# Amanda-Zheng/MR-GNAS

Hardware: AMD Instinct MI355X
Metric: million edges/sec per supernet fwd+bwd step (FB15k-237, dim=200) (higher is better)
Workload: dtype f32

## Files before the change

include/mrgnas.h:

```cpp
#ifndef MRGNAS_H
#define MRGNAS_H

#include <stdint.h>

#ifdef __cplusplus
extern "C" {
#endif

#define MRG_ABI_VERSION 19

#define MRG_OK            0
#define MRG_E_NULLPTR    -1
#define MRG_E_SHAPE      -2
#define MRG_E_ENUM       -3
#define MRG_E_WORKSPACE  -4

#define MRG_COMPOSE_MULT 0
#define MRG_COMPOSE_SUB  1
#define MRG_COMPOSE_ADD  2
#define MRG_REDUCE_SUM   0
#define MRG_REDUCE_MEAN  1
#define MRG_REDUCE_MAX   2
#define MRG_GCS_SUB      0
#define MRG_GCS_MUL      1
#define MRG_GCS_COPY     2
#define MRG_GCS_NEGS     3
#define MRG_GCS_CCORR    4
#define MRG_GCS_CCONV    5
#define MRG_ACT_NONE     0
#define MRG_ACT_RELU     1
#define MRG_ACT_SIGMOID  2

int mrg_abi_version(void);
const char *mrg_error_string(int code);
const char *mrg_target_arch(void);

int mrg_compose_fwd(int op, const float *s, const float *hr, float *out,
                    int64_t rows, int D, void *stream);
int mrg_compose_bwd(int op, const float *gout, const float *s, const float *hr,
                    float *gs, float *ghr, int64_t rows, int D, void *stream);

int mrg_gather_compose_fwd(int op, const float *ent, const float *rel,
                           const int32_t *ent_idx, const int32_t *rel_idx,
                           float *out, int64_t rows, int D, void *stream);

#define MRG_GATE_LD(D) (2 * (D) + 4)

int mrg_gate_collapse3(const float *const *W_host, const float *const *b_host, const float *const *a_host, float *uvc,
                       int D, int in_dim, int fold, void *stream);
int mrg_gate_param_grad3(const float *const *W_host, const float *const *b_host, const float *const *a_host,
                         const float *d_uvc, float *const *gW_host, float *const *gb_host, float *const *ga_host,
                         int D, int in_dim, int fold, void *stream);
int mrg_fold_halves3(const float *const *W_host, float *Wt, int D, void *stream);
int mrg_unfold_halves3(const float *const *gWt_host, float *const *gW_host, int D, void *stream);

int mrg_gate_fwd(const float *s, const float *s_in, const float *norm, const float *uvc,
                 float *out, int64_t b0, int64_t b1, int64_t M, int D, float scale, void *stream);
int64_t mrg_gate_bwd_workspace_bytes(int64_t M, int D);
int mrg_gate_bwd(const float *gout, const float *s, const float *s_in, const float *norm,
                 const float *uvc, float *gs, float *gs_in, float *d_uvc, void *ws,
                 int64_t b0, int64_t b1, int64_t M, int D, float scale, void *stream);
int mrg_gate_row_fwd(const float *s, const float *s_in, const float *norm, const float *uvc, float *fvec, float *hvec,
                     int64_t b0, int64_t b1, int64_t M, int D, float scale, void *stream);
int mrg_gate_row_bwd(const float *q, const float *hvec, const float *s, const float *s_in, const float *uvc, float *gs_in, float *d_uvc,
                     void *ws, int64_t b0, int64_t b1, int64_t M, int D, void *stream);

int64_t mrg_seg_reduce_workspace_bytes(int64_t n_slots, int D);
int mrg_seg_reduce_fwd(int mode, const float *msg, const float *self_rows,
                       const int32_t *eid,
                       const int32_t *chunk_node, const int32_t *chunk_start, const int32_t *chunk_end,
                       const int32_t *chunk_slot, int64_t n_chunks,
                       const int32_t *hub_node, const int32_t *hub_first, const int32_t *hub_count, int64_t n_hubs,
                       int64_t n_slots, const int32_t *in_degree,
                       float *out, int32_t *arg, void *ws,
                       int64_t N, int D, void *stream);
int mrg_seg_reduce_bwd(int mode, const float *gout, const int32_t *dst, const int32_t *in_degree,
                       const int32_t *arg, float *gmsg, float *gself, const float *relu_src,
                       int64_t E, int64_t N, int D, void *stream);
int mrg_seg_reduce_bwd_ordered(int mode, const float *gout, const int32_t *dst, const int32_t *in_degree, const int32_t *arg,
                               float *gmsg, float *gself, const float *relu_src, const unsigned *relu_bits, const int32_t *order,
                               int64_t E, int64_t N, int D, void *stream);
int mrg_segmax_bwd_input_ok(int D, int Kin);
int mrg_segmax_bwd_input(const float *gout, const float *mx, const int32_t *dst, const int32_t *arg, const float *W, float *gmsg,
                         float *gx, const int32_t *order, int64_t E, int64_t N, int D, int Kin, void *stream);

int64_t mrg_seg_std_workspace_bytes(int64_t n_slots, int D);
int mrg_seg_std_fwd(const float *msg, const int32_t *eid, const int32_t *chunk_node, const int32_t *chunk_start,
                    const int32_t *chunk_end, const int32_t *chunk_slot, int64_t n_chunks, const int32_t *hub_node,
                    const int32_t *hub_first, const int32_t *hub_count, int64_t n_hubs, int64_t n_slots,
                    const int32_t *in_degree, float *out, float *mean, float *coef, void *ws, int64_t N, int D, void *stream);
int mrg_seg_std_bwd(const float *gout, const float *msg, const int32_t *dst, const float *mean, const float *coef,
                    const int32_t *order, float *gmsg, int64_t E, int64_t N, int D, void *stream);

int mrg_fused_gcs(int mode, const float *X, const int32_t *xi, const float *Y, const int32_t *yi,
                  const float *scal, const int32_t *eid,
                  const int32_t *chunk_node, const int32_t *chunk_start, const int32_t *chunk_end,
                  const int32_t *chunk_slot, int64_t n_chunks,
                  const int32_t *hub_node, const int32_t *hub_first, const int32_t *hub_count, int64_t n_hubs,
                  int64_t n_slots, const int32_t *seg_len,
                  float *out, void *ws, int64_t nseg, int D, void *stream);

int mrg_span_gcs(int mode, const float *X, const float *Y, const void *meta, const float *ext_scal, int64_t E, int span,
                 const int32_t *span_slot, const int32_t *span_start, int64_t n_spans,
                 const int32_t *hub_seg, const int32_t *hub_first, const int32_t *hub_count, int64_t n_hubs,
                 int64_t n_slots, const int32_t *seg_len,
                 float *out, void *ws, int64_t nseg, int D, void *stream);

int mrg_sum_buffers(const float *const *xs_host, int K, float *out, int64_t n, int accumulate, void *stream);
int mrg_sum_rows_gather(const float *const *xs_host, int K, const float *gather_edge, const float *gather_self,
                        const int32_t *dst, int64_t E, int64_t rows, int D, float *out, void *stream);

int mrg_distmult_score(const float *ent, const float *rel, const int32_t *s_idx, const int32_t *r_idx,
                       const int32_t *o_idx, float *score, int64_t T, int D, void *stream);

int64_t mrg_mix_workspace_bytes(int K, int D);

int mrg_optim_chunk(void);
int mrg_clip_sgd_step(void *const *params, const void *const *grads, void *const *bufs, const int32_t *chunk_tensor,
                      const int64_t *chunk_off, const int32_t *chunk_len, int64_t n_chunks, double *partial, float *norm_coef,
                      float max_norm, float lr, float momentum, float weight_decay, void *stream);
typedef struct mrg_gated_branch {
  int32_t k;
  const float *s;
  const float *rowscale;
  int32_t row_k;
  const float *row_f;
  const float *row_h;
  const float *row_uvc;
  int32_t row_ld;
  int64_t b0, b1;
  float *row_dq;
  int32_t act;
  const int32_t *valid_rows;
} mrg_gated_branch;
int mrg_mix_colstats(const float *const *y_host, int K, int64_t rows, int D, double *sums, void *ws,
                     const mrg_gated_branch *gated, void *stream);
int mrg_mix_finalize_fwd(const double *sums, const float *const *gamma_host, const float *const *beta_host,
                         float *const *rmean_host, float *const *rvar_host, int K, double total_rows, int D,
                         float eps, float momentum, float *coef, void *stream);
int mrg_mix_stats_coef(const float *const *y, const float *const *gamma, const float *const *beta,
                       float *const *running_mean, float *const *running_var, int K, int64_t rows, double total_rows,
                       int D, float eps, float momentum, float *coef, void *ws, const mrg_gated_branch *gated, void *stream);
int mrg_mix_fwd(const float *const *y_host, int K, const float *coef, const float *w, const float *addend, float *out,
                int64_t rows, int D, const mrg_gated_branch *gated, void *stream);
int mrg_mix_bwd_reduce(const float *g, const float *const *y_host, int K, const float *coef, const float *w,
                       float *red, void *ws, int64_t rows, int D, const mrg_gated_branch *gated, void *stream);
int mrg_mix_finalize_bwd(const float *red, int K, double total_rows, int D, float *coef2,
                         float *const *dgamma_host, float *const *dbeta_host, float *dw, const int32_t *valid_rows, void *stream);
int mrg_mix_bwd_apply(const float *g, const float *const *y_host, float *const *gy_host, int K,
                      const float *coef, const float *coef2, const float *w, const float *const *rs, const float *rs_scale,
                      const float *rs_self, const int64_t *rs_edge_rows, const int *rs_on, const float *const *rs_full,
                      const float *const *fold_s,
                      const float *const *fold_gate, float *const *fold_gs, const int *fold_add_from, int64_t rows, int D,
                      const mrg_gated_branch *gated, void *stream);

int64_t mrg_zero_workspace_bytes(int D);
int mrg_zero_colstats(const float *ent, const float *rel, const int32_t *ent_idx, const int32_t *rel_idx, const int *ops, int K,
                      int64_t rows, int D, double *sums, void *ws, void *stream);
int mrg_zero_stats_coef(const float *ent, const float *rel, const int32_t *ent_idx, const int32_t *rel_idx, const int *ops, int K,
                        const float *const *gamma, const float *const *beta, float *const *running_mean,
                        float *const *running_var, int64_t rows, double total_rows, int D, float eps, float momentum,
                        float *coef, void *ws, const int32_t *valid_rows, void *stream);
int mrg_zero_fwd(const float *ent, const float *rel, const int32_t *ent_idx, const int32_t *rel_idx, const int *ops, int K,
                 const float *coef, const float *w, float *out, int64_t rows, int D, const int32_t *valid_rows, void *stream);
int mrg_zero_bwd_reduce(const float *g, const float *ent, const float *rel, const int32_t *ent_idx, const int32_t *rel_idx,
                        const int *ops, int K, const float *coef, const float *w, float *red, void *ws, int64_t rows, int D,
                        const int32_t *valid_rows, void *stream);
int mrg_zero_bwd_apply(const float *g, const float *ent, const float *rel, const int32_t *ent_idx, const int32_t *rel_idx,
                       const int *ops, int K, const float *coef, const float *coef2, const float *w, float *g_ent_rows,
                       float *g_rel_rows, int64_t rows, int D, const int32_t *valid_rows, void *stream);


int64_t mrg_gemm_workspace_bytes(int K, int Nout);
int mrg_gemm_set_mode(int mode);
int mrg_gemm_set_epilogue(int mode);
int mrg_gemm_set_wide8(int on);
int mrg_gemm_set_q(int on);
int mrg_gemm_set_small(int on);
int mrg_wgrad_set_variant(int variant);
int mrg_linear_fwd(const float *X, const float *W, const float *bias, float *Y, void *ws,
                   int64_t rows, int K, int Nout, int act, void *stream);
int64_t mrg_linear_relu_segmax_workspace_bytes(int64_t N, int K, int Nout);
int mrg_linear_relu_segmax_fwd(const float *X, const float *W, const float *bias, const int32_t *eid, const int32_t *dst,
                               const float *self_rows, float *out, int32_t *arg, float *mx, void *ws,
                               int64_t E, int64_t N, int K, int Nout, void *stream);
int mrg_linear_relu_segsum_fwd(const float *X, const float *W, const float *bias, const int32_t *eid, const int32_t *dst,
                               float *part, unsigned *relu_bits, void *ws, int64_t E, int K, int Nout, void *stream);
int mrg_seg_reduce_heads_fwd(int mode, const float *part, const float *self_rows, const int32_t *rowptr,
                             const int32_t *chunk_node, const int32_t *chunk_start, const int32_t *chunk_end,
                             const int32_t *chunk_slot, int64_t n_chunks, const int32_t *hub_node, const int32_t *hub_first,
                             const int32_t *hub_count, int64_t n_hubs, int64_t n_slots, const int32_t *in_degree, float *out,
                             void *ws, int64_t N, int D, void *stream);
int mrg_seg_reduce_bwd_bits(int mode, const float *gout, const int32_t *dst, const int32_t *in_degree, float *gmsg, float *gself,
                            const unsigned *relu_bits, int64_t E, int64_t N, int D, void *stream);
int64_t mrg_linear_bwd_input_workspace_bytes(int K, int Nout);
int mrg_linear_bwd_input(const float *gY, const float *W, float *gX, void *ws,
                         int64_t rows, int K, int Nout, int ldw, int accumulate, void *stream);
int64_t mrg_linear_bwd_weight_workspace_bytes(int64_t rows, int K, int Nout);
int mrg_linear_bwd_weight(const float *gY, const float *X1, const float *X2, float *gW, float *gbias, void *ws,
                          int64_t rows, int K1, int K2, int Nout, void *stream);
int mrg_linear_bwd_weight_share(const float *gY, const float *X1, const float *X2, float *gW, float *gbias, void *ws,
                                int64_t rows, int K1, int K2, int Nout, int share, void *stream);

int mrg_dense_filter_fwd(int kind, const float *s, const float *s_in, const float *W, const float *bias,
                         const float *rowscale, float scale, float *out, float *gate, void *ws,
                         int64_t rows, int D, void *stream);
int64_t mrg_dense_filter3_workspace_bytes(int D, int K);
int mrg_dense_filter_fwd3(int kind, const float *s, const float *s_in, const float *const *W, const float *const *bias,
                          const float *norm, float scale_edge, float scale_self, float *out, float *gate, void *ws,
                          int64_t b0, int64_t b1, int64_t M, int D, void *stream);
int mrg_dense_filter_dz3(int kind, const float *g, const float *s, const float *gate, const float *norm, float scale_edge,
                         float scale_self, float *dz, float *gs, int64_t b1, int64_t M, int D, void *stream);
int64_t mrg_linear_bwd_input3_workspace_bytes(int K, int Nout);
int mrg_linear_bwd_input3(const float *gY, const float *const *W, float *gX, void *ws, int64_t b0, int64_t b1, int64_t M,
                          int K, int Nout, int ldw, int accumulate, void *stream);
int64_t mrg_linear_bwd_input3_pair_workspace_bytes(int K, int Nout);
int mrg_linear_bwd_input3_pair(const float *gY1, const float *gY2, const float *const *W1, const float *const *W2, float *gX,
                               void *ws, int64_t b0, int64_t b1, int64_t M, int K, int Nout, int ldw, int accumulate,
                               void *stream);
int64_t mrg_linear_bwd_weight3_workspace_bytes(int64_t b0, int64_t b1, int64_t M, int K1, int K2, int Nout);
int mrg_linear_bwd_weight3(const float *gY, const float *X1, const float *X2, float *const *gW, float *const *gbias, void *ws,
                           int64_t b0, int64_t b1, int64_t M, int K1, int K2, int Nout, void *stream);
int mrg_dense_filter_dz(int kind, const float *g, const float *s, const float *gate, const float *rowscale,
                        float scale, float *dz, float *gs, int64_t rows, int D, void *stream);

int64_t mrg_build_graph_workspace_bytes(int64_t T);
int mrg_build_graph(const int64_t *triples, int64_t T, int64_t N, int R, int sorted,
                    const float *deg_norm_table, int64_t table_len,
                    int64_t *src, int64_t *dst, int64_t *etype, float *norm, int32_t *in_degree,
                    int32_t *src32, int32_t *dst32, int32_t *etype32, int32_t *max_degree,
                    void *ws, int64_t ws_bytes, void *stream);

int64_t mrg_plan_workspace_bytes(int64_t E, int64_t nseg, int span);
int mrg_span_plan_build(const int32_t *seg, int64_t E, int64_t nseg, int span, int snap,
                        int32_t *perm, int32_t *seg_sorted, int32_t *seg_len, int32_t *span_slot, int32_t *span_start,
                        int32_t *hub_seg, int32_t *hub_first, int32_t *hub_count, int32_t *counts,
                        void *ws, int64_t ws_bytes, void *stream);
int mrg_span_meta_pack(const int32_t *perm, const int32_t *seg_sorted, const int32_t *xi, const int32_t *yi,
                       const float *scal, int w_is_index, void *meta, int64_t E, void *stream);

int64_t mrg_chunk_plan_workspace_bytes(int64_t E, int64_t N);
int mrg_chunk_plan_build(const int32_t *dst, int64_t E, int64_t N, int chunk,
                         int32_t *eid, int32_t *rowptr, int32_t *in_degree,
                         int32_t *chunk_node, int32_t *chunk_start, int32_t *chunk_end, int32_t *chunk_slot,
                         int32_t *hub_node, int32_t *hub_first, int32_t *hub_count, int32_t *counts,
                         void *ws, int64_t ws_bytes, void *stream);

int mrg_negative_sampling(const int64_t *pos, int64_t B, int rate, const int64_t *values, const double *choices,
                          int64_t *samples, float *labels, void *stream);
int64_t mrg_sample_neighborhood_workspace_bytes(int64_t N, int64_t T);
int mrg_sample_edge_neighborhood(const int32_t *rowptr, const int32_t *adj_edge, const int32_t *adj_other, const int32_t *degrees,
                                 int64_t N, int64_t T, int64_t sample_size, const double *u_vertex, const int64_t *tries,
                                 int64_t n_tries, const double *u_edge, int32_t *edges, int64_t *status, void *ws,
                                 int64_t ws_bytes, void *stream);
int64_t mrg_relabel_workspace_bytes(int64_t num_nodes);
int mrg_relabel_nodes(const int64_t *src, const int64_t *dst, int64_t n, int64_t num_nodes, int64_t *uniq,
                      int64_t *new_src, int64_t *new_dst, int32_t *count, void *ws, int64_t ws_bytes, void *stream);
int mrg_multi_hot_labels(const int64_t *keys, const int32_t *rowptr, const int32_t *objs, const int64_t *query,
                         int64_t B, int64_t U, int64_t num_ent, float v_zero, float v_one, float *out, void *stream);

int mrg_rank_filtered(const float *pred, const float *labels, const int64_t *obj, int64_t B, int64_t N,
                      int64_t *ranks, void *stream);
int mrg_transe_score_fwd(const float *ent, const float *sub, const float *rel, float gamma, float *score,
// ... 44 lines not shown
```

mr-gnas_amd/_lib.py:

```python
import ctypes
import os
import re

import torch

_HERE = os.path.dirname(os.path.abspath(__file__))
LIB_PATH = os.environ.get("MRG_LIB_PATH") or os.path.join(_HERE, "lib", "libmrgnas_hip.so")
HEADER_PATH = os.path.join(os.path.dirname(_HERE), "include", "mrgnas.h")

ABI_VERSION = 19


class MrgnasLibraryError(RuntimeError):
    pass


class MrgnasError(RuntimeError):
    """A C-ABI call returned a non-zero code."""


_P, _I, _L, _F = ctypes.c_void_p, ctypes.c_int, ctypes.c_int64, ctypes.c_float

SIGNATURES = {
    "mrg_abi_version": (_I, []),
    "mrg_error_string": (ctypes.c_char_p, [_I]),
    "mrg_target_arch": (ctypes.c_char_p, []),
    "mrg_compose_fwd": (_I, [_I, _P, _P, _P, _L, _I, _P]),
    "mrg_compose_bwd": (_I, [_I, _P, _P, _P, _P, _P, _L, _I, _P]),
    "mrg_gather_compose_fwd": (_I, [_I, _P, _P, _P, _P, _P, _L, _I, _P]),
    "mrg_gate_collapse3": (_I, [_P, _P, _P, _P, _I, _I, _I, _P]),
    "mrg_gate_param_grad3": (_I, [_P, _P, _P, _P, _P, _P, _P, _I, _I, _I, _P]),
    "mrg_fold_halves3": (_I, [_P, _P, _I, _P]),
    "mrg_unfold_halves3": (_I, [_P, _P, _I, _P]),
    "mrg_gate_fwd": (_I, [_P, _P, _P, _P, _P, _L, _L, _L, _I, _F, _P]),
    "mrg_gate_bwd_workspace_bytes": (_L, [_L, _I]),
    "mrg_gate_bwd": (_I, [_P, _P, _P, _P, _P, _P, _P, _P, _P, _L, _L, _L, _I, _F, _P]),
    "mrg_seg_reduce_workspace_bytes": (_L, [_L, _I]),
    "mrg_seg_reduce_fwd": (_I, [_I, _P, _P, _P, _P, _P, _P, _P, _L, _P, _P, _P, _L, _L, _P, _P, _P, _P, _L, _I, _P]),
    "mrg_seg_reduce_bwd": (_I, [_I, _P, _P, _P, _P, _P, _P, _P, _L, _L, _I, _P]),
    "mrg_fused_gcs": (_I, [_I, _P, _P, _P, _P, _P, _P, _P, _P, _P, _P, _L, _P, _P, _P, _L, _L, _P, _P, _P, _L, _I, _P]),
    "mrg_span_gcs": (_I, [_I, _P, _P, _P, _P, _L, _I, _P, _P, _L, _P, _P, _P, _L, _L, _P, _P, _P, _L, _I, _P]),
    "mrg_sum_buffers": (_I, [_P, _I, _P, _L, _I, _P]),
    "mrg_sum_rows_gather": (_I, [_P, _I, _P, _P, _P, _L, _L, _I, _P, _P]),
    "mrg_distmult_score": (_I, [_P, _P, _P, _P, _P, _P, _L, _I, _P]),
    "mrg_gate_row_fwd": (_I, [_P, _P, _P, _P, _P, _P, _L, _L, _L, _I, _F, _P]),
    "mrg_gate_row_bwd": (_I, [_P, _P, _P, _P, _P, _P, _P, _P, _L, _L, _L, _I, _P]),
    "mrg_mix_workspace_bytes": (_L, [_I, _I]),
    "mrg_mix_colstats": (_I, [_P, _I, _L, _I, _P, _P, _P, _P]),
    "mrg_mix_finalize_fwd": (_I, [_P, _P, _P, _P, _P, _I, ctypes.c_double, _I, _F, _F, _P, _P]),
    "mrg_mix_stats_coef": (_I, [_P, _P, _P, _P, _P, _I, _L, ctypes.c_double, _I, _F, _F, _P, _P, _P, _P]),
    "mrg_zero_workspace_bytes": (_L, [_I]),
    "mrg_zero_colstats": (_I, [_P, _P, _P, _P, _P, _I, _L, _I, _P, _P, _P]),
    "mrg_zero_stats_coef": (_I, [_P, _P, _P, _P, _P, _I, _P, _P, _P, _P, _L, ctypes.c_double, _I, _F, _F, _P, _P, _P, _P]),
    "mrg_zero_fwd": (_I, [_P, _P, _P, _P, _P, _I, _P, _P, _P, _L, _I, _P, _P]),
    "mrg_zero_bwd_reduce": (_I, [_P, _P, _P, _P, _P, _P, _I, _P, _P, _P, _P, _L, _I, _P, _P]),
    "mrg_zero_bwd_apply": (_I, [_P, _P, _P, _P, _P, _P, _I, _P, _P, _P, _P, _P, _L, _I, _P, _P]),
    "mrg_mix_fwd": (_I, [_P, _I, _P, _P, _P, _P, _L, _I, _P, _P]),
    "mrg_mix_bwd_reduce": (_I, [_P, _P, _I, _P, _P, _P, _P, _L, _I, _P, _P]),
    "mrg_mix_finalize_bwd": (_I, [_P, _I, ctypes.c_double, _I, _P, _P, _P, _P, _P, _P]),
    "mrg_mix_bwd_apply": (_I, [_P, _P, _P, _I, _P, _P, _P, _P, _P, _P, _P, _P, _P, _P, _P, _P, _P, _L, _I, _P, _P]),
    "mrg_dense_filter_fwd": (_I, [_I, _P, _P, _P, _P, _P, _F, _P, _P, _P, _L, _I, _P]),
    "mrg_dense_filter_dz": (_I, [_I, _P, _P, _P, _P, _F, _P, _P, _L, _I, _P]),
    "mrg_gemm_workspace_bytes": (_L, [_I, _I]),
    "mrg_gemm_set_mode": (_I, [_I]),
    "mrg_gemm_set_epilogue": (_I, [_I]),
    "mrg_gemm_set_wide8": (_I, [_I]),
    "mrg_gemm_set_q": (_I, [_I]),
    "mrg_gemm_set_small": (_I, [_I]),
    "mrg_segmax_bwd_input_ok": (_I, [_I, _I]),
    "mrg_segmax_bwd_input": (_I, [_P, _P, _P, _P, _P, _P, _P, _P, _L, _L, _I, _I, _P]),
    "mrg_seg_std_workspace_bytes": (_L, [_L, _I]),
    "mrg_seg_std_fwd": (_I, [_P, _P, _P, _P, _P, _P, _L, _P, _P, _P, _L, _L, _P, _P, _P, _P, _P, _L, _I, _P]),
    "mrg_seg_std_bwd": (_I, [_P, _P, _P, _P, _P, _P, _P, _L, _L, _I, _P]),
    "mrg_optim_chunk": (_I, []),
    "mrg_clip_sgd_step": (_I, [_P, _P, _P, _P, _P, _P, _L, _P, _P, _F, _F, _F, _F, _P]),
    "mrg_act_grad_transpose": (_I, [_P, _P, _P, _L, _L, _I, _P]),
    "mrg_wgrad_set_variant": (_I, [_I]),
    "mrg_linear_fwd": (_I, [_P, _P, _P, _P, _P, _L, _I, _I, _I, _P]),
    "mrg_dense_filter3_workspace_bytes": (_L, [_I, _I]),
    "mrg_dense_filter_fwd3": (_I, [_I, _P, _P, _P, _P, _P, _F, _F, _P, _P, _P, _L, _L, _L, _I, _P]),
    "mrg_dense_filter_dz3": (_I, [_I, _P, _P, _P, _P, _F, _F, _P, _P, _L, _L, _I, _P]),
    "mrg_linear_bwd_input3_workspace_bytes": (_L, [_I, _I]),
    "mrg_linear_bwd_input3": (_I, [_P, _P, _P, _P, _L, _L, _L, _I, _I, _I, _I, _P]),
    "mrg_linear_bwd_input3_pair_workspace_bytes": (_L, [_I, _I]),
    "mrg_linear_bwd_input3_pair": (_I, [_P, _P, _P, _P, _P, _P, _L, _L, _L, _I, _I, _I, _I, _P]),
    "mrg_linear_bwd_weight3_workspace_bytes": (_L, [_L, _L, _L, _I, _I, _I]),
    "mrg_linear_bwd_weight3": (_I, [_P, _P, _P, _P, _P, _P, _L, _L, _L, _I, _I, _I, _P]),
    "mrg_linear_relu_segsum_fwd": (_I, [_P, _P, _P, _P, _P, _P, _P, _P, _L, _I, _I, _P]),
    "mrg_seg_reduce_heads_fwd": (_I, [_I, _P, _P, _P, _P, _P, _P, _P, _L, _P, _P, _P, _L, _L, _P, _P, _P, _L, _I, _P]),
    "mrg_seg_reduce_bwd_bits": (_I, [_I, _P, _P, _P, _P, _P, _P, _L, _L, _I, _P]),
    "mrg_seg_reduce_bwd_ordered": (_I, [_I, _P, _P, _P, _P, _P, _P, _P, _P, _P, _L, _L, _I, _P]),
    "mrg_linear_relu_segmax_workspace_bytes": (_L, [_L, _I, _I]),
    "mrg_linear_relu_segmax_fwd": (_I, [_P, _P, _P, _P, _P, _P, _P, _P, _P, _P, _L, _L, _I, _I, _P]),
    "mrg_linear_bwd_input_workspace_bytes": (_L, [_I, _I]),
    "mrg_linear_bwd_input": (_I, [_P, _P, _P, _P, _L, _I, _I, _I, _I, _P]),
    "mrg_linear_bwd_weight_workspace_bytes": (_L, [_L, _I, _I]),
    "mrg_linear_bwd_weight": (_I, [_P, _P, _P, _P, _P, _P, _L, _I, _I, _I, _P]),
    "mrg_linear_bwd_weight_share": (_I, [_P, _P, _P, _P, _P, _P, _L, _I, _I, _I, _I, _P]),
    "mrg_build_graph_workspace_bytes": (_L, [_L]),
    "mrg_build_graph": (_I, [_P, _L, _L, _I, _I, _P, _L, _P, _P, _P, _P, _P, _P, _P, _P, _P, _P, _L, _P]),
    "mrg_plan_workspace_bytes": (_L, [_L, _L, _I]),
    "mrg_span_plan_build": (_I, [_P, _L, _L, _I, _I, _P, _P, _P, _P, _P, _P, _P, _P, _P, _P, _L, _P]),
    "mrg_span_meta_pack": (_I, [_P, _P, _P, _P, _P, _I, _P, _L, _P]),
    "mrg_chunk_plan_workspace_bytes": (_L, [_L, _L]),
    "mrg_chunk_plan_build": (_I, [_P, _L, _L, _I, _P, _P, _P, _P, _P, _P, _P, _P, _P, _P, _P, _P, _L, _P]),
    "mrg_negative_sampling": (_I, [_P, _L, _I, _P, _P, _P, _P, _P]),
    "mrg_sample_neighborhood_workspace_bytes": (_L, [_L, _L]),
    "mrg_sample_edge_neighborhood": (_I, [_P, _P, _P, _P, _L, _L, _L, _P, _P, _L, _P, _P, _P, _P, _L, _P]),
    "mrg_relabel_workspace_bytes": (_L, [_L]),
    "mrg_relabel_nodes": (_I, [_P, _P, _L, _L, _P, _P, _P, _P, _P, _L, _P]),
    "mrg_multi_hot_labels": (_I, [_P, _P, _P, _P, _L, _L, _L, _F, _F, _P, _P]),
    "mrg_rank_filtered": (_I, [_P, _P, _P, _L, _L, _P, _P]),
    "mrg_transe_score_fwd": (_I, [_P, _P, _P, _F, _P, _L, _L, _I, _P]),
    "mrg_transe_score_bwd": (_I, [_P, _P, _P, _P, _P, _P, _P, _L, _L, _I, _P]),
    "mrg_ccorr_rows": (_I, [_I, _P, _P, _P, _L, _I, _P]),
    "mrg_ccorr_matrix": (_I, [_I, _P, _P, _I, _P]),
    "mrg_ccorr_matrix_grad": (_I, [_I, _P, _P, _I, _P]),
    "mrg_conve_fc_workspace_bytes": (_L, [_L, _L, _I]),
    "mrg_conve_bwd_workspace_bytes": (_L, [_L, _I, _I, _I]),
    "mrg_conve_bn0_fwd": (_I, [_P, _P, _L, _I, _P, _P, _I, _F, _F, _P, _P]),
    "mrg_conve_conv_fwd": (_I, [_I, _P, _P, _L, _I, _I, _I, _P, _P, _P, _P, _P, _I, _I, _P, _P]),
    "mrg_conve_bn1_fwd": (_I, [_P, _L, _I, _I, _P, _P, _P, _P, _P, _I, _F, _F, _P, _P, _P]),
    "mrg_conve_fc_fwd": (_I, [_P, _P, _P, _P, _P, _P, _L, _L, _I, _P]),
    "mrg_conve_fc_bwd": (_I, [_P, _P, _P, _P, _P, _P, _P, _P, _L, _L, _I, _P]),
    "mrg_conve_bn1_bwd": (_I, [_P, _P, _P, _P, _P, _P, _I, _L, _I, _I, _P, _P, _P]),
    "mrg_conve_conv_bwd": (_I, [_I, _P, _P, _L, _I, _I, _I, _P, _P, _P, _P, _I, _I, _P, _P, _P]),
    "mrg_conve_finish_bwd": (_I, [_I, _P, _P, _L, _I, _I, _I, _P, _P, _I, _P, _P, _P, _P, _P, _P, _P, _P]),
}

_lib = None


def declared_symbols():
# ... 7 lines not shown
    if _lib is not None:
        return _lib
    if not os.path.exists(LIB_PATH):
        raise MrgnasLibraryError(
            f"{LIB_PATH} not found: build it with `python -c 'import __graft_entry__ as g; g.build()'` "
            "(or `make -C mr-gnas_amd/csrc`). mr_gnas_amd has no CPU fallback.")
    lib = ctypes.CDLL(LIB_PATH)
    for name, (res, args) in SIGNATURES.items():
        fn = getattr(lib, name)
        fn.restype, fn.argtypes = res, args
    if lib.mrg_abi_version() != ABI_VERSION:
        raise MrgnasLibraryError(f"ABI version {lib.mrg_abi_version()} != expected {ABI_VERSION}; rebuild the library")
    _lib = lib
    return lib


class KernelMeter:

    def __init__(self):
        self.names = None
        self.records = {}

    def start(self, names=None):
        self.names = set(names) if names is not None else True
        self.records = {}

    def active(self, name):
        return self.names is not None and (self.names is True or name in self.names)

    def stop(self):
        torch.cuda.synchronize()
        out = {}
        for name, recs in self.records.items():
            ms = sum(a.elapsed_time(b) for a, b, _, _ in recs)
            out[name] = {"launches": len(recs), "ms": ms, "bytes": sum(r[2] for r in recs), "flops": sum(r[3] for r in recs)}
        self.names, self.records = None, {}
        return out


meter = KernelMeter()


_FN = {}
TRACE = os.environ.get("MRG_TRACE") == "1"


def _trace(name, args):
    import sys
    shown = [hex(a.value) if isinstance(a, ctypes.c_void_p) and a.value else ("NULL" if isinstance(a, ctypes.c_void_p) or a is None else a)
             for a in args]
    print(f"[mrg] {name} {shown}", file=sys.stderr, flush=True)


def call(name, args, nbytes=0, flops=0):
    fn = _FN.get(name)
    if fn is None:
        fn = _FN[name] = getattr(load(), name)
    if TRACE:
        _trace(name, args)
        code = fn(*args)
        torch.cuda.synchronize()
        if code != 0:
            check(code, name)
        return
    if meter.names is not None and meter.active(name):
        a, b = torch.cuda.Event(enable_timing=True), torch.cuda.Event(enable_timing=True)
        a.record()
        code = fn(*args)
        b.record()
        meter.records.setdefault(name, []).append((a, b, nbytes, flops))
    else:
        code = fn(*args)
    if code != 0:
        check(code, name)


def check(code, what=""):
    if code != 0:
        msg = load().mrg_error_string(code).decode()
        raise MrgnasError(f"{what}: {msg} (code {code})")


def ptr(t):
    return None if t is None else ctypes.c_void_p(t.data_ptr())


def ptr_array(tensors):
    arr = (ctypes.c_void_p * len(tensors))()
    for i, t in enumerate(tensors):
        arr[i] = None if t is None else t.data_ptr()
    return arr


class GatedBranch(ctypes.Structure):
    _fields_ = [("k", ctypes.c_int32), ("s", ctypes.c_void_p), ("rowscale", ctypes.c_void_p),
                ("row_k", ctypes.c_int32), ("row_f", ctypes.c_void_p), ("row_h", ctypes.c_void_p), ("row_uvc", ctypes.c_void_p),
                ("row_ld", ctypes.c_int32), ("b0", ctypes.c_int64), ("b1", ctypes.c_int64), ("row_dq", ctypes.c_void_p),
                ("act", ctypes.c_int32), ("valid_rows", ctypes.c_void_p)]


ACTS = {"relu": 0, "tanh": 1}


def gated_branch(spec, row_dq=None, act=0, valid_rows=None):
    dp = lambda t: None if t is None else t.data_ptr()
    if spec is None:
        if not act and valid_rows is None:
            return None
        return ctypes.byref(GatedBranch(-1, None, None, -1, None, None, None, 0, 0, 0, None, int(act), dp(valid_rows)))
    g = GatedBranch(int(spec.get("k", -1)), dp(spec["s"]), dp(spec.get("c")), int(spec.get("row_k", -1)), dp(spec.get("row_f")),
                    dp(spec.get("row_h")), dp(spec.get("row_uvc")), int(spec.get("row_ld", 0)), int(spec.get("b0", 0)), int(spec.get("b1", 0)),
                    dp(row_dq), int(act), dp(valid_rows))
    return ctypes.byref(g)


_RAW_STREAM = getattr(torch._C, "_cuda_getCurrentRawStream", None) if os.environ.get("MRG_RAW_STREAM", "1") == "1" else None


def stream_of(t):
    if _RAW_STREAM is not None:
        return ctypes.c_void_p(_RAW_STREAM(t.device.index if t.device.index is not None else torch.cuda.current_device()))
    return ctypes.c_void_p(torch.cuda.current_stream(t.device).cuda_stream)


def require_hip(*tensors):
    for t in tensors:
        if t is None:
            continue
        if not t.is_cuda:
            raise MrgnasError("mr_gnas_amd operators need tensors on a HIP device (no CPU fallback); got " + str(t.device))
        if not t.is_contiguous():
            raise MrgnasError("mr_gnas_amd operators need contiguous tensors")
    load()


def f32c(t):
    if t is None:
        return None
    if t.dtype != torch.float32:
        t = t.float()
    return t if t.is_contiguous() else t.contiguous()
```

mr-gnas_amd/cell_lp.py:

```python
import os

import torch
import torch.nn as nn

from . import functional as K
from . import lazy as LZ
from . import operations_lp as OPS
from .operations_lp import PRE_OPS, FIRST_OPS, MIDDLE_OPS, LAST_OPS, MIXED_OPS, MIXED_OPS_sf, SF_OPS

CALLER = os.environ.get("MRG_CALLER", "fused")

MIXED_STREAMS = int(os.environ.get("MRG_MIXED_STREAMS", "1"))


def _literal(h):
    x = h.x if isinstance(h, K.Fan) else h
    return CALLER == "reference" or not (x.table if isinstance(x, K.LazyRows) else x).is_cuda


def _tensor(y):
    return y.y if isinstance(y, K.Candidate) else y


def _plain(h):
    if isinstance(h, K.Fan):
        h = h.take()
    return h.materialize() if isinstance(h, K.LazyRows) else h


def _valid_rows(g, ys):
    counts = getattr(g, "valid_rows", None)
    y = next((y for y in ys if y is not None), None)
    return counts.get(int(_tensor(y).shape[0])) if counts and y is not None else None


def _identity_index(ops):
    ids = [k for k, op in enumerate(ops) if type(op) is OPS.f_identity_op]
    return ids[0] if len(ids) == 1 else None


def _dense_pair(ops, x):
    if not x.is_cuda:
        return None
    d = [k for k, op in enumerate(ops) if type(op) is OPS.f_dense_op_comp]
    c = [k for k, op in enumerate(ops) if type(op) is OPS.f_comp_op]
    if len(d) != 1 or len(c) != 1:
        return None
    return (d[0], c[0])


def _run(op, g, a, b, for_epilogue=False):
    if op._forward_hooks or op._forward_pre_hooks or not hasattr(op, "run"):
        return LZ.real(op(g, a, b, for_epilogue=True) if for_epilogue else op(g, a, b))
    return op.run(g, a, b, for_epilogue=for_epilogue)


def fused_candidates(ops, bns, weights, g, h, h_in, addend=None, group=None, total_rows=None, prepare_only=False):
    if isinstance(h, K.LazyRows):
        if (K.switches.CELL_ZERO_FUSED and isinstance(h_in, K.LazyRows) and addend is None and len(ops) <= 3
                and all(isinstance(op, OPS._PreOp) for op in ops)):
            return K.cell_zero_mixed([op.kind for op in ops], h, h_in, bns, weights, group, total_rows, _valid_rows(g, [h]))
        ys = [_run(op, g, h, h_in) for op in ops]
        return K.mixed_epilogue(ys, bns, weights, group, total_rows, addend, fold_row_scales=True, valid_rows=_valid_rows(g, ys))
    n = len(ops)
    fh = h if isinstance(h, K.Fan) else K.Fan(h, n)
    fi = h_in if isinstance(h_in, K.Fan) else K.Fan(h_in, n)
    pair = _dense_pair(ops, fh.x)
    paired = {}
    row_ok = pair is not None and K.switches.GATED_RECOMPUTE and K.switches.FOLD_ROW_SCALE
    dev = fh.x.device
    nstreams = min(MIXED_STREAMS, n) if fh.x.shape[0] >= K.switches.FORK_MIN_ROWS else 1
    if nstreams <= 1:
        ys = []
        for k, op in enumerate(ops):
            if isinstance(op, OPS.f_zero_op):
                ys.append(None)
            elif pair is not None and k in pair:
                if not paired:
                    paired[pair[0]], paired[pair[1]] = OPS.dense_pair_forward(ops[pair[0]], ops[pair[1]], g, fh.take(), fi.take(), for_epilogue=True)
                ys.append(paired[k])
            elif (row_ok and type(op) is OPS.f_sparse_op_comp) or type(op) in (OPS.f_dense_op_comp, OPS.f_comp_op):
                ys.append(_run(op, g, fh.take(), fi.take(), for_epilogue=True))
            else:
                ys.append(_run(op, g, fh.take(), fi.take()))
        prep = K.mixed_epilogue_prepare(ys, bns, group, total_rows, True, _identity_index(ops), valid_rows=_valid_rows(g, ys))
        return prep if prepare_only else prep(weights, addend)
    fork = K.Fork(dev, nstreams, tag="candidates")
    ys = []
    for k, op in enumerate(ops):
        if isinstance(op, OPS.f_zero_op):
            ys.append(None)
            continue
        if pair is not None and k in pair and paired:
            ys.append(paired[k])
            continue
        side = fork.stream(k)
        a, b = fh.take(), fi.take()
        if side is not fork.main:
            a.record_stream(side)
            b.record_stream(side)
        with torch.cuda.stream(side):
            if pair is not None and k in pair:
                paired[pair[0]], paired[pair[1]] = OPS.dense_pair_forward(ops[pair[0]], ops[pair[1]], g, a, b, for_epilogue=True)
                y = paired[k]
                _tensor(paired[pair[0] + pair[1] - k]).record_stream(fork.main)
            elif (row_ok and type(op) is OPS.f_sparse_op_comp) or type(op) in (OPS.f_dense_op_comp, OPS.f_comp_op):
                y = _run(op, g, a, b, for_epilogue=True)
            else:
                y = _run(op, g, a, b)
        _tensor(y).record_stream(fork.main)
        ys.append(y)
    fork.join()
    prep = K.mixed_epilogue_prepare(ys, bns, group, total_rows, True, _identity_index(ops), valid_rows=_valid_rows(g, ys))
    return prep if prepare_only else prep(weights, addend)


class MixedOp(nn.Module):

    def __init__(self, feature_dim, drop_aggr, operations, registry=None):
        super().__init__()
        registry = MIXED_OPS if registry is None else registry
        self._feature_dim, self._operations, self._drop_aggr = feature_dim, operations, drop_aggr
        self._args = {'feature_dim': feature_dim, 'drop_aggr': drop_aggr}
        self._ops = nn.ModuleList(nn.ModuleList([registry[name](self._args), nn.BatchNorm1d(feature_dim), nn.ReLU()])
                                  for name in operations)

    def op_forward(self, op, g, h, h_in):
        nh = op[0](g, h, h_in)
        for i in range(1, len(op)):
            nh = op[i](nh.float())
        return nh

    def forward(self, weights, g, h, h_in, group=None, total_rows=None, addend=None, prepare_only=False):
        if _literal(h):
            h, h_in = _plain(h), _plain(h_in)
            total = sum(w * self.op_forward(op, g, h, h_in) for w, op in zip(weights, self._ops))
            return total if addend is None else addend + total
        return fused_candidates([op for op, _, _ in self._ops], [bn for _, bn, _ in self._ops], weights, g, h, h_in, addend, group,
                                total_rows, prepare_only)

    def _identity_index(self):
        return _identity_index([op for op, _, _ in self._ops])

    def _dense_pair(self, x):
        return _dense_pair([op for op, _, _ in self._ops], x)


class MixedOp_SF(nn.Module):

    def __init__(self, gamma, operations, registry=None):
        super().__init__()
        registry = MIXED_OPS_sf if registry is None else registry
        self._operations, self.gamma = operations, gamma
        self._args = {'gamma': gamma}
        self._ops = nn.ModuleList(nn.ModuleList([registry[name](self._args)]) for name in operations)

    def op_forward(self, op, g, h, h_in):
        return op[0](g, h, h_in)

    def forward(self, weights, g, h, h_in):
        return sum(w * self.op_forward(op, g, h, h_in) for w, op in zip(weights, self._ops))


# ... 102 lines not shown
```

mr-gnas_amd/csrc/dense.hip:

```cpp
#include "gemm_dispatch.hpp"

namespace mrg {

template <int VEC, int LPR, int KMAX, int KIND>
__global__ __launch_bounds__(MRG_BLOCK) void dense_dz_k(const float* __restrict__ g, const float* __restrict__ s,
                                                        const float* __restrict__ gate, const float* __restrict__ rowscale,
                                                        float scale, float* __restrict__ dz, float* __restrict__ gs,
                                                        int64_t rows, int D, int64_t edge_rows, float scale_self) {
  constexpr int RPB = MRG_BLOCK / LPR;
  const int sl = threadIdx.x % LPR, rw = row_group_of_thread<LPR>();
  const int dv = D / VEC;
  for (int64_t r = (int64_t)blockIdx.x * RPB + rw; r < rows; r += (int64_t)gridDim.x * RPB) {
    const float c = r < edge_rows ? scale * (rowscale ? rowscale[r] : 1.0f) : scale_self;
#pragma unroll
    for (int k = 0; k < KMAX; ++k) {
      int col = sl + k * LPR;
      if (col < dv) {
        Vec<VEC> gv = Vec<VEC>::load(g + r * D + col * VEC), o;
        if (KIND == 0) {
          Vec<VEC> sv = Vec<VEC>::load(s + r * D + col * VEC), ga = Vec<VEC>::load(gate + r * D + col * VEC), o2;
#pragma unroll
          for (int j = 0; j < VEC; ++j) {
            float gc = gv[j] * c;
            o2[j] = gc * ga[j];
            o[j] = gc * sv[j] * ga[j] * (1.0f - ga[j]);
          }
          o2.store(gs + r * D + col * VEC);
        } else {
#pragma unroll
          for (int j = 0; j < VEC; ++j) o[j] = gv[j] * c;
        }
        o.store(dz + r * D + col * VEC);
      }
    }
  }
}

}

using namespace mrg;

extern "C" int mrg_dense_filter_fwd(int kind, const float* s, const float* s_in, const float* W, const float* bias,
                                    const float* rowscale, float scale, float* out, float* gate, void* ws, int64_t rows, int D,
                                    void* stream) {
  if (kind != 0 && kind != 1) return MRG_E_ENUM;
  if (rows < 0 || D <= 0) return MRG_E_SHAPE;
  if (rows == 0) return MRG_OK;
  if (!s || !W || !out) return MRG_E_NULLPTR;
  GemmArgs a{};
  a.A1 = s; a.K1 = D;
  a.A2 = s_in; a.K2 = s_in ? D : 0;
  a.B = W;
  a.bias = bias; a.C = out; a.ldc = D; a.N = D; a.rows = rows;
  a.rowscale = rowscale; a.scale = scale;
  if (kind == 0) {
    a.S = s; a.ld_s = D; a.aux = gate;
    return launch_gemm<EPI_GATE>(a, a.K1 + a.K2, 1, ws, (hipStream_t)stream);
  }
  return launch_gemm<EPI_SCALE>(a, a.K1 + a.K2, 1, ws, (hipStream_t)stream);
}

static bool dense3_shape_ok(int D, int K) { return D > 0 && (K == D || K == 2 * D) && K > 48 && D % 4 == 0; }

extern "C" int64_t mrg_dense_filter3_workspace_bytes(int D, int K) {
  if (!dense3_shape_ok(D, K) || gemm_mode() == 1) return 0;
  return 3 * (int64_t)(((int64_t)bsplit_bytes_any(D, K) + 255) / 256 * 256);
}

extern "C" int mrg_dense_filter_fwd3(int kind, const float* s, const float* s_in, const float* const* W_host, const float* const* bias_host,
                                     const float* norm, float scale_edge, float scale_self, float* out, float* gate, void* ws,
                                     int64_t b0, int64_t b1, int64_t M, int D, void* stream) {
  if (kind != 0 && kind != 1) return MRG_E_ENUM;
  if (D <= 0 || M < 0 || b0 < 0 || b1 < b0 || M < b1) return MRG_E_SHAPE;
  const int K = s_in ? 2 * D : D;
  if (!dense3_shape_ok(D, K)) return MRG_E_SHAPE;
  if (M == 0) return MRG_OK;
  if (!s || !W_host) return MRG_E_NULLPTR;
  if (kind == 0 && !gate) return MRG_E_NULLPTR;
  if (!out && kind != 0) return MRG_E_NULLPTR;
  if (!ws) return MRG_E_WORKSPACE;
  hipStream_t st = (hipStream_t)stream;
  const int64_t lo[3] = {0, b0, b1}, hi[3] = {b0, b1, M};
  const size_t each = (size_t)(((int64_t)bsplit_bytes_any(D, K) + 255) / 256 * 256);
  GemmArgs a{};
  a.A1 = s; a.K1 = D; a.A2 = s_in; a.K2 = s_in ? D : 0;
  a.C = out; a.ldc = D; a.N = D; a.rows = M; a.rowscale = norm;
  if (kind == 0) { a.S = s; a.ld_s = D; a.aux = gate; }
  if (!x3_eligible(a)) return MRG_E_SHAPE;
  const float* Bs[3]; void* outs[3];
  a.grp.n = 3;
  a.grp.bp_stride = (int64_t)each;
  for (int i = 0; i < 3; ++i) {
    const bool live = hi[i] > lo[i];
    if (live && !W_host[i]) return MRG_E_NULLPTR;
    Bs[i] = live ? W_host[i] : nullptr;
    outs[i] = (char*)ws + i * each;
    a.grp.lo[i] = lo[i]; a.grp.hi[i] = live ? hi[i] : lo[i];
    a.grp.bias[i] = bias_host ? bias_host[i] : nullptr;
    a.grp.scale[i] = i < 2 ? scale_edge : scale_self;
    a.grp.use_rowscale[i] = (i < 2 && norm) ? 1 : 0;
  }
  launch_bsplit3_any(kind == 0 ? EPI_GATE : EPI_SCALE, M, Bs, K, 1, D, K, outs, st);
  MRG_LAUNCH_CHECK();
  if (kind == 0) return launch_rowgemm_x3_mode<EPI_GATE>(a, outs[0], st);
  return launch_rowgemm_x3_mode<EPI_SCALE>(a, outs[0], st);
}

static int dense_dz_launch(int kind, const float* g, const float* s, const float* gate, const float* rowscale, float scale, float* dz,
                           float* gs, int64_t rows, int D, int64_t edge_rows, float scale_self, void* stream);

extern "C" int mrg_dense_filter_dz(int kind, const float* g, const float* s, const float* gate, const float* rowscale,
                                   float scale, float* dz, float* gs, int64_t rows, int D, void* stream) {
  return dense_dz_launch(kind, g, s, gate, rowscale, scale, dz, gs, rows, D, rows, scale, stream);
}

extern "C" int mrg_dense_filter_dz3(int kind, const float* g, const float* s, const float* gate, const float* norm, float scale_edge,
                                    float scale_self, float* dz, float* gs, int64_t b1, int64_t M, int D, void* stream) {
  if (b1 < 0 || M < b1) return MRG_E_SHAPE;
  return dense_dz_launch(kind, g, s, gate, norm, scale_edge, dz, gs, M, D, b1, scale_self, stream);
}

static int dense_dz_launch(int kind, const float* g, const float* s, const float* gate, const float* rowscale, float scale, float* dz,
                           float* gs, int64_t rows, int D, int64_t edge_rows, float scale_self, void* stream) {
  if (kind != 0 && kind != 1) return MRG_E_ENUM;
  if (rows < 0 || D <= 0) return MRG_E_SHAPE;
  if (rows == 0) return MRG_OK;
  if (!g || !dz) return MRG_E_NULLPTR;
  if (kind == 0 && (!s || !gate || !gs)) return MRG_E_NULLPTR;
  hipStream_t st = (hipStream_t)stream;
  RowGeom gm = row_geom(D, aligned16(g) && aligned16(s) && aligned16(gate) && aligned16(gs) && aligned16(dz));
  if (!gm.ok) return MRG_E_SHAPE;
#define CALL(V, L, KM)                                                                                                \
  do {                                                                                                                \
    int grid = grid_for(rows, (MRG_BLOCK / L) * 4);                                                                         \
    if (kind == 0) hipLaunchKernelGGL((dense_dz_k<V, L, KM, 0>), dim3(grid), dim3(MRG_BLOCK), 0, st, g, s, gate, rowscale, scale, dz, gs, rows, D, edge_rows, scale_self); \
    else hipLaunchKernelGGL((dense_dz_k<V, L, KM, 1>), dim3(grid), dim3(MRG_BLOCK), 0, st, g, s, gate, rowscale, scale, dz, gs, rows, D, edge_rows, scale_self); \
  } while (0)
  MRG_DISPATCH_GEOM(gm, CALL);
#undef CALL
  MRG_LAUNCH_CHECK();
  return MRG_OK;
}
```

mr-gnas_amd/csrc/gate.hip:

```cpp
#include "common.hpp"

namespace mrg {

struct SegPlan {
  int64_t lo[3], hi[3];
  int blk[4];
};

static SegPlan make_plan(int64_t b0, int64_t b1, int64_t M, int grid) {
  SegPlan p;
  p.lo[0] = 0;  p.hi[0] = b0;
  p.lo[1] = b0; p.hi[1] = b1;
  p.lo[2] = b1; p.hi[2] = M;
  int nseg = 0;
  for (int s = 0; s < 3; ++s) nseg += (p.hi[s] > p.lo[s]);
  int spare = grid - nseg;
  p.blk[0] = 0;
  for (int s = 0; s < 3; ++s) {
    int64_t rows = p.hi[s] - p.lo[s];
    int nb = rows > 0 ? 1 + (int)((double)spare * (double)rows / (double)M) : 0;
    p.blk[s + 1] = p.blk[s] + nb;
  }
  return p;
}
// ... 180 lines not shown
    if (srcidx >= 0) {
#pragma unroll
      for (int q = 0; q < RPB; ++q) acc += (double)red[q * (2 * WIDTH + 1) + srcidx];
    }
    dst[t] = (float)acc;
  }
}

template <int VEC, int LPR, int KMAX, bool HAS_IN>
__global__ __launch_bounds__(MRG_BLOCK) void gate_row_fwd_k(const float* __restrict__ s, const float* __restrict__ sin_,
                                                            const float* __restrict__ norm, const float* __restrict__ uvc,
                                                            float* __restrict__ fvec, float* __restrict__ hvec, SegPlan p, int D, float scale) {
  constexpr int RPB = MRG_BLOCK / LPR;
  const int b = blockIdx.x;
  if (b >= p.blk[3]) return;
  const int seg = (b >= p.blk[1]) + (b >= p.blk[2]);
  const int jb = b - p.blk[seg], nb = p.blk[seg + 1] - p.blk[seg];
  const int sl = threadIdx.x % LPR, rw = row_group_of_thread<LPR>();
  const int dv = D / VEC;
  const float* u = uvc + (int64_t)seg * MRG_GATE_LD(D);
  const float cc = u[HAS_IN ? 2 * D : D];
  Vec<VEC> uk[KMAX], vk[KMAX];
#pragma unroll
  for (int k = 0; k < KMAX; ++k) {
    int c = sl + k * LPR;
    uk[k] = c < dv ? Vec<VEC>::load(u + c * VEC) : Vec<VEC>::fill(0.f);
    vk[k] = (HAS_IN && c < dv) ? Vec<VEC>::load(u + D + c * VEC) : Vec<VEC>::fill(0.f);
  }
  const bool use_norm = norm != nullptr && seg < 2;
  for (int64_t r = p.lo[seg] + (int64_t)jb * RPB + rw; r < p.hi[seg]; r += (int64_t)nb * RPB) {
    float dot = 0.f;
#pragma unroll
    for (int k = 0; k < KMAX; ++k) {
      int c = sl + k * LPR;
      if (c < dv) {
        const Vec<VEC> sk = Vec<VEC>::load(s + r * D + c * VEC);
#pragma unroll
        for (int j = 0; j < VEC; ++j) dot += sk[j] * uk[k][j];
        if (HAS_IN) {
          Vec<VEC> x = Vec<VEC>::load(sin_ + r * D + c * VEC);
#pragma unroll
          for (int j = 0; j < VEC; ++j) dot += x[j] * vk[k][j];
        }
      }
    }
    const float z = group_sum<LPR>(dot) + cc;
    const float gt = sigmoidf_fast(z);
    const float nv = use_norm ? norm[r] : 1.0f;
    if (sl == 0) {
      fvec[r] = gt * scale * nv;
      const float t = scale * nv;
      hvec[r] = t * gt * (1.0f - gt);
    }
  }
}

template <int VEC, int LPR, int KMAX, bool HAS_IN>
__global__ __launch_bounds__(MRG_BLOCK) void gate_row_bwd_k(const float* __restrict__ qv, const float* __restrict__ hv, const float* __restrict__ s,
                                                            const float* __restrict__ sin_, const float* __restrict__ uvc,
                                                            float* __restrict__ gsin, float* __restrict__ ws, SegPlan p, int D) {
  constexpr int RPB = MRG_BLOCK / LPR;
  constexpr int WIDTH = LPR * KMAX * VEC;
  __shared__ float red[RPB * (2 * WIDTH + 1)];
  const int b = blockIdx.x;
  if (b >= p.blk[3]) return;
  const int seg = (b >= p.blk[1]) + (b >= p.blk[2]);
  const int jb = b - p.blk[seg], nb = p.blk[seg + 1] - p.blk[seg];
  const int sl = threadIdx.x % LPR, rw = row_group_of_thread<LPR>();
  const int dv = D / VEC;
  const int ld = MRG_GATE_LD(D);
  const int cidx = HAS_IN ? 2 * D : D;
  const float* u = uvc + (int64_t)seg * ld;
  Vec<VEC> vk[KMAX], du[KMAX], dvv[KMAX];
  double dc = 0.0;
#pragma unroll
  for (int k = 0; k < KMAX; ++k) {
    int c = sl + k * LPR;
    vk[k] = (HAS_IN && c < dv) ? Vec<VEC>::load(u + D + c * VEC) : Vec<VEC>::fill(0.f);
    du[k] = Vec<VEC>::fill(0.f);
    dvv[k] = Vec<VEC>::fill(0.f);
  }
  for (int64_t r = p.lo[seg] + (int64_t)jb * RPB + rw; r < p.hi[seg]; r += (int64_t)nb * RPB) {
    const float dz = qv[r] * hv[r];
    dc += (double)dz;
#pragma unroll
    for (int k = 0; k < KMAX; ++k) {
      int c = sl + k * LPR;
      if (c < dv) {
        const Vec<VEC> sk = Vec<VEC>::load(s + r * D + c * VEC);
#pragma unroll
        for (int j = 0; j < VEC; ++j) du[k][j] += dz * sk[j];
        if (HAS_IN) {
          const Vec<VEC> xk = Vec<VEC>::load(sin_ + r * D + c * VEC);
          Vec<VEC> o2;
#pragma unroll
          for (int j = 0; j < VEC; ++j) {
            o2[j] = dz * vk[k][j];
            dvv[k][j] += dz * xk[j];
          }
          o2.store(gsin + r * D + c * VEC);
        }
      }
    }
  }
  float* mine = red + rw * (2 * WIDTH + 1);
#pragma unroll
// ... 167 lines not shown
  if (!g.ok) return MRG_E_SHAPE;
  hipStream_t st = (hipStream_t)stream;
  int grid = 1;
#define CALL(V, L, K)                                                                                                   \
  do {                                                                                                                  \
    grid = grid_for(M, (MRG_BLOCK / L) * 4);                                                                                   \
    if (grid < 3) grid = 3;                                                                                             \
    SegPlan p = make_plan(b0, b1, M, grid);                                                                             \
    if (s_in) hipLaunchKernelGGL((gate_fwd_k<V, L, K, true, gate_rpt(L)>), dim3(p.blk[3]), dim3(MRG_BLOCK), 0, st, s, s_in, norm, uvc, out, p, D, scale); \
    else hipLaunchKernelGGL((gate_fwd_k<V, L, K, false, gate_rpt(L)>), dim3(p.blk[3]), dim3(MRG_BLOCK), 0, st, s, s_in, norm, uvc, out, p, D, scale); \
  } while (0)
  MRG_DISPATCH_GEOM(g, CALL);
#undef CALL
  MRG_LAUNCH_CHECK();
  return MRG_OK;
}

extern "C" int64_t mrg_gate_bwd_workspace_bytes(int64_t M, int D) {
  (void)M;
  return (int64_t)(MRG_MAX_GRID + 3) * MRG_GATE_LD((int64_t)D) * sizeof(float);
}

extern "C" int mrg_gate_bwd(const float* gout, const float* s, const float* s_in, const float* norm, const float* uvc,
                            float* gs, float* gs_in, float* d_uvc, void* ws, int64_t b0, int64_t b1, int64_t M, int D,
                            float scale, void* stream) {
  if (D <= 0 || M < 0 || b0 < 0 || b1 < b0 || M < b1) return MRG_E_SHAPE;
  if (!uvc || !d_uvc) return MRG_E_NULLPTR;
  if (M > 0 && (!gout || !s || !gs)) return MRG_E_NULLPTR;
  if (s_in && !gs_in) return MRG_E_NULLPTR;
  if (!ws) return MRG_E_WORKSPACE;
  hipStream_t st = (hipStream_t)stream;
  const int ld = MRG_GATE_LD(D);
  RowGeom g = row_geom(D, aligned16(gout) && aligned16(s) && aligned16(s_in) && aligned16(gs) && aligned16(gs_in) && aligned16(uvc));
  if (!g.ok) return MRG_E_SHAPE;
  SegPlan p{};
#define CALL(V, L, K)                                                                                                   \
  do {                                                                                                                  \
    int grid = grid_for(M, (MRG_BLOCK / L) * 4);                                                                               \
    if (grid < 3) grid = 3;                                                                                             \
    p = make_plan(b0, b1, M, grid);                                                                                     \
    if (M > 0) {                                                                                                        \
      if (s_in) hipLaunchKernelGGL((gate_bwd_k<V, L, K, true, gate_rpt(L)>), dim3(p.blk[3]), dim3(MRG_BLOCK), 0, st, gout, s, s_in, norm, uvc, gs, gs_in, (float*)ws, p, D, scale); \
      else hipLaunchKernelGGL((gate_bwd_k<V, L, K, false, gate_rpt(L)>), dim3(p.blk[3]), dim3(MRG_BLOCK), 0, st, gout, s, s_in, norm, uvc, gs, gs_in, (float*)ws, p, D, scale); \
    }                                                                                                                   \
  } while (0)
  MRG_DISPATCH_GEOM(g, CALL);
#undef CALL
  MRG_LAUNCH_CHECK();
  launch_ordered_reduce_ranges<float>((const float*)ws, d_uvc, p.blk, 3, ld, ld, ld, st);
  MRG_LAUNCH_CHECK();
  return MRG_OK;
}

extern "C" int mrg_gate_row_fwd(const float* s, const float* s_in, const float* norm, const float* uvc, float* fvec, float* hvec,
                                int64_t b0, int64_t b1, int64_t M, int D, float scale, void* stream) {
  if (D <= 0 || M < 0 || b0 < 0 || b1 < b0 || M < b1) return MRG_E_SHAPE;
  if (M == 0) return MRG_OK;
  if (!s || !uvc || !fvec || !hvec) return MRG_E_NULLPTR;
  RowGeom g = row_geom(D, aligned16(s) && aligned16(s_in) && aligned16(uvc));
  if (!g.ok) return MRG_E_SHAPE;
  hipStream_t st = (hipStream_t)stream;
#define CALL(V, L, K)                                                                                                   \
  do {                                                                                                                  \
    int grid = grid_for(M, (MRG_BLOCK / L) * 4);                                                                        \
    if (grid < 3) grid = 3;                                                                                             \
    SegPlan p = make_plan(b0, b1, M, grid);                                                                             \
    if (s_in) hipLaunchKernelGGL((gate_row_fwd_k<V, L, K, true>), dim3(p.blk[3]), dim3(MRG_BLOCK), 0, st, s, s_in, norm, uvc, fvec, hvec, p, D, scale); \
    else hipLaunchKernelGGL((gate_row_fwd_k<V, L, K, false>), dim3(p.blk[3]), dim3(MRG_BLOCK), 0, st, s, s_in, norm, uvc, fvec, hvec, p, D, scale); \
  } while (0)
  MRG_DISPATCH_GEOM(g, CALL);
#undef CALL
  MRG_LAUNCH_CHECK();
  return MRG_OK;
}

extern "C" int mrg_gate_row_bwd(const float* q, const float* hvec, const float* s, const float* s_in, const float* uvc, float* gs_in, float* d_uvc,
                                void* ws, int64_t b0, int64_t b1, int64_t M, int D, void* stream) {
  if (D <= 0 || M < 0 || b0 < 0 || b1 < b0 || M < b1) return MRG_E_SHAPE;
  if (!uvc || !d_uvc) return MRG_E_NULLPTR;
  if (M > 0 && (!q || !hvec || !s)) return MRG_E_NULLPTR;
  if (s_in && !gs_in) return MRG_E_NULLPTR;
  if (!ws) return MRG_E_WORKSPACE;
  hipStream_t st = (hipStream_t)stream;
  const int ld = MRG_GATE_LD(D);
  RowGeom g = row_geom(D, aligned16(s) && aligned16(s_in) && aligned16(gs_in) && aligned16(uvc));
  if (!g.ok) return MRG_E_SHAPE;
  SegPlan p{};
#define CALL(V, L, K)                                                                                                   \
  do {                                                                                                                  \
    int grid = grid_for(M, (MRG_BLOCK / L) * 4);                                                                        \
    if (grid < 3) grid = 3;                                                                                             \
    p = make_plan(b0, b1, M, grid);                                                                                     \
    if (M > 0) {                                                                                                        \
      if (s_in) hipLaunchKernelGGL((gate_row_bwd_k<V, L, K, true>), dim3(p.blk[3]), dim3(MRG_BLOCK), 0, st, q, hvec, s, s_in, uvc, gs_in, (float*)ws, p, D); \
      else hipLaunchKernelGGL((gate_row_bwd_k<V, L, K, false>), dim3(p.blk[3]), dim3(MRG_BLOCK), 0, st, q, hvec, s, s_in, uvc, gs_in, (float*)ws, p, D); \
    }                                                                                                                   \
  } while (0)
  MRG_DISPATCH_GEOM(g, CALL);
#undef CALL
  MRG_LAUNCH_CHECK();
  launch_ordered_reduce_ranges<float>((const float*)ws, d_uvc, p.blk, 3, ld, ld, ld, st);
  MRG_LAUNCH_CHECK();
  return MRG_OK;
}
```

mr-gnas_amd/csrc/gemm.hpp:

```cpp
#pragma once
#include "common.hpp"

namespace mrg {

typedef float f32x16 __attribute__((ext_vector_type(16)));
typedef float v4f __attribute__((ext_vector_type(4)));
typedef __attribute__((address_space(3))) void* lds_ptr_t;
typedef const __attribute__((address_space(1))) void* gbl_ptr_t;

constexpr int GBM_MAX = 256;

enum { EPI_BIAS_ACT = 0, EPI_GATE = 1, EPI_SCALE = 2, EPI_ACCUM = 3, EPI_SEGMAX = 4, EPI_SEGSUM = 5 };

struct GemmGroups {
  int n;
  int tile0[4];
  int64_t lo[3], hi[3];
  int64_t bp_stride;
  const float* bias[3];
  float scale[3];
  int use_rowscale[3];
};
inline int gemm_group_tiles(GemmGroups& g, int gbm) {
  g.tile0[0] = 0;
  for (int i = 0; i < 3; ++i) {
    const int64_t r = i < g.n && g.hi[i] > g.lo[i] ? g.hi[i] - g.lo[i] : 0;
    g.tile0[i + 1] = g.tile0[i] + (int)((r + gbm - 1) / gbm);
  }
  return g.tile0[3];
}

struct GemmArgs {
  const float* A1; const float* A2;
  int K1, K2;
  const float* B; int ldb;
  const float* bias;
  float* C; int ldc; int N;
  int64_t rows;
  int act;
  const float* S; int ld_s;
  const float* rowscale; float scale;
  float* aux;
  const float* Cin; int ld_cin;
  const int32_t* row_index;
  const int32_t* row_seg;
  unsigned long long* seg_out;
  float* seg_part;
  unsigned* relu_bits; int bits_ld;
  int epi_lds; int wave_lds_floats;
  GemmGroups grp;
};

template <bool DUAL>
__device__ __forceinline__ const float* gemm_a_ptr(const float* r1, const float* r2, int K1, int K2, int K, int k) {
  if (DUAL) {
    const bool first = k < K1;
    const int kk = first ? k : k - K1, ld = first ? K1 : K2;
    return (first ? r1 : r2) + (kk + 4 <= ld ? kk : ld - 4);
  }
  return r1 + (k + 4 <= K ? k : K - 4);
}

template <int NT>
__device__ __forceinline__ void gemm_epilogue_segsum(const GemmArgs& a, f32x16 (&acc)[NT], int64_t rowbase, int col0, int li, int lh) {
  if (rowbase >= a.rows) return;
  int seg[16], eidv[16];
#pragma unroll
  for (int r = 0; r < 16; ++r) {
    const int64_t row = rowbase + (r & 3) + 8 * (r >> 2) + 4 * lh;
    const bool ok = row < a.rows;
    const int64_t rc = ok ? row : a.rows - 1;
    const int e = a.row_index ? a.row_index[rc] : (int)rc;
    eidv[r] = ok ? e : -1;
    seg[r] = ok ? a.row_seg[e] : -1;
  }
#pragma unroll
  for (int n = 0; n < NT; ++n) {
    const int col = col0 + n * 32 + li;
    const bool cok = col < a.N;
    const float bv = (a.bias && cok) ? a.bias[col] : 0.f;
    int cur = -1;
    int64_t head = 0;
    float sum = 0.f;
#pragma unroll
    for (int r = 0; r < 16; ++r) {
      const float x = acc[n][r] + bv;
      const bool pos = x > 0.f;
      const unsigned long long ball = __ballot(pos);
      if (li == 0 && eidv[r] >= 0 && a.relu_bits && (col0 >> 5) + n < a.bits_ld)
        a.relu_bits[(int64_t)eidv[r] * a.bits_ld + (col0 >> 5) + n] = lh ? (unsigned)(ball >> 32) : (unsigned)ball;
      if (seg[r] != cur) {
        if (cur >= 0 && cok) a.seg_part[head * a.N + col] = sum;
        cur = seg[r];
        head = rowbase + (r & 3) + 8 * (r >> 2) + 4 * lh;
        sum = 0.f;
      }
      sum += pos ? x : 0.f;
    }
    if (cur >= 0 && cok) a.seg_part[head * a.N + col] = sum;
  }
}

template <int NT>
__device__ __forceinline__ void gemm_epilogue_segmax(const GemmArgs& a, f32x16 (&acc)[NT], int64_t rowbase, int col0, int li, int lh) {
  if (rowbase >= a.rows) return;
// ... 47 lines not shown
template <bool VEC4>
__device__ __forceinline__ float4 gemm_mask4(float4 v, int64_t row, int64_t nrows, int k, int K) {
  const bool rv = row < nrows;
  if (VEC4) {
    const bool ok = rv && k + 4 <= K;
    v.x = ok ? v.x : 0.f; v.y = ok ? v.y : 0.f; v.z = ok ? v.z : 0.f; v.w = ok ? v.w : 0.f;
  } else {
    v.x = (rv && k < K) ? v.x : 0.f; v.y = (rv && k + 1 < K) ? v.y : 0.f;
    v.z = (rv && k + 2 < K) ? v.z : 0.f; v.w = (rv && k + 3 < K) ? v.w : 0.f;
  }
  return v;
}

struct ASel { const float* base; int ld, kk; };
__device__ __forceinline__ ASel gemm_sel_a(const GemmArgs& a, int k) {
  const bool first = k < a.K1 || a.K2 == 0;
  ASel s;
  s.base = first ? a.A1 : a.A2;
  s.ld = first ? a.K1 : a.K2;
  s.kk = first ? k : k - a.K1;
  return s;
}

template <bool VEC4>
__device__ __forceinline__ float4 gemm_raw_a(const GemmArgs& a, int64_t row, int k) {
  if (VEC4) {
    const ASel sa = gemm_sel_a(a, k);
    return gemm_raw4<true>(sa.base, row, a.rows, sa.kk, sa.ld, sa.ld);
  }
  const int64_t rc = row < a.rows ? row : a.rows - 1;
  float v[4];
#pragma unroll
  for (int j = 0; j < 4; ++j) {
    const ASel sa = gemm_sel_a(a, k + j);
    const int kc = sa.kk < sa.ld ? sa.kk : sa.ld - 1;
    v[j] = sa.base[rc * sa.ld + kc];
  }
  return make_float4(v[0], v[1], v[2], v[3]);
}

template <bool VEC4>
__device__ __forceinline__ float4 gemm_mask_a(float4 v, const GemmArgs& a, int64_t row, int k) {
  if (VEC4) {
    const ASel sa = gemm_sel_a(a, k);
    return gemm_mask4<true>(v, row, a.rows, sa.kk, sa.ld);
  }
  const int K = a.K1 + a.K2;
  const bool rv = row < a.rows;
  v.x = (rv && k < K) ? v.x : 0.f; v.y = (rv && k + 1 < K) ? v.y : 0.f;
  v.z = (rv && k + 2 < K) ? v.z : 0.f; v.w = (rv && k + 3 < K) ? v.w : 0.f;
  return v;
}

template <int NT, int EPI>
__device__ __forceinline__ void gemm_epilogue(const GemmArgs& a, f32x16 (&acc)[NT], int64_t rowbase, int col0, int li, int lh,
                                              bool full) {
  if (rowbase >= a.rows) return;
  const int last = (int)((a.rows - 1 - rowbase) < 31 ? (a.rows - 1 - rowbase) : 31);
  const int colw = col0 + li < a.N ? col0 + li : a.N - 1;
  float* crow[16];
  const float* srow[16];
  float* xrow[16];
  float cs[16];
  bool rok[16];
  const bool cstore = EPI != EPI_GATE || a.C != nullptr;
#pragma unroll
  for (int r = 0; r < 16; ++r) {
    const int row = (r & 3) + 8 * (r >> 2) + 4 * lh;
    const int rc = row < last ? row : last;
    rok[r] = row <= last;
    crow[r] = a.C + (rowbase + rc) * a.ldc + colw;
    if (EPI == EPI_GATE) srow[r] = a.S + (rowbase + rc) * a.ld_s + colw;
    if (EPI == EPI_ACCUM) srow[r] = a.Cin + (rowbase + rc) * a.ld_cin + colw;
    if (EPI == EPI_GATE) xrow[r] = a.aux ? a.aux + (rowbase + rc) * a.N + colw : nullptr;
    cs[r] = 1.0f;
    if (EPI == EPI_GATE || EPI == EPI_SCALE) cs[r] = a.scale * (a.rowscale ? a.rowscale[rowbase + rc] : 1.0f);
  }
#pragma unroll
  for (int n = 0; n < NT; ++n) {
    const int col = col0 + n * 32 + li;
    const bool cok = col < a.N;
    const int off = cok ? n * 32 : 0;
    const float bv = a.bias ? a.bias[cok ? col : colw] : 0.f;
    float in[16], v[16], g[16];
#pragma unroll
    for (int r = 0; r < 16; ++r) in[r] = 0.f;
    if ((EPI == EPI_GATE && cstore) || EPI == EPI_ACCUM) {
#pragma unroll
      for (int r = 0; r < 16; ++r) in[r] = srow[r][off];
    }
#pragma unroll
    for (int r = 0; r < 16; ++r) {
      float x = acc[n][r] + bv;
      if (EPI == EPI_BIAS_ACT) {
        v[r] = (a.act == MRG_ACT_RELU) ? (x > 0.f ? x : 0.f) : (a.act == MRG_ACT_SIGMOID ? sigmoidf_fast(x) : x);
      } else if (EPI == EPI_GATE) {
        g[r] = sigmoidf_fast(x);
        v[r] = g[r] * in[r] * cs[r];
      } else if (EPI == EPI_SCALE) {
        v[r] = x * cs[r];
      } else {
        v[r] = x + in[r];
      }
    }
    if (full) {
      if (cok) {
        if (cstore) {
#pragma unroll
          for (int r = 0; r < 16; ++r) crow[r][n * 32] = v[r];
        }
        if (EPI == EPI_GATE && a.aux) {
#pragma unroll
          for (int r = 0; r < 16; ++r) xrow[r][n * 32] = g[r];
        }
      }
    } else {
#pragma unroll
      for (int r = 0; r < 16; ++r) {
        if (cok && rok[r]) {
          if (cstore) crow[r][n * 32] = v[r];
          if (EPI == EPI_GATE && a.aux) xrow[r][n * 32] = g[r];
        }
      }
    }
  }
}

template <int NT, int EPI>
__device__ __forceinline__ void gemm_epilogue_tr(const GemmArgs& a, f32x16 (&acc)[NT], int64_t rowbase, int col0, int li, int lh) {
  if (rowbase >= a.rows) return;
  const int64_t row = rowbase + li;
  const bool rok = row < a.rows;
  const int64_t rc = rok ? row : a.rows - 1;
  const int cb = col0 + 4 * lh;
  const bool cstore = EPI != EPI_GATE || a.C != nullptr;
  float* crow = cstore ? a.C + rc * a.ldc + cb : nullptr;
  const float* srow = nullptr;
  if (EPI == EPI_GATE && cstore) srow = a.S + rc * a.ld_s + cb;
  if (EPI == EPI_ACCUM) srow = a.Cin + rc * a.ld_cin + cb;
  float* xrow = (EPI == EPI_GATE && a.aux) ? a.aux + rc * a.N + cb : nullptr;
  float cs = 1.0f;
  if (EPI == EPI_GATE || EPI == EPI_SCALE) cs = a.scale * (a.rowscale ? a.rowscale[rc] : 1.0f);
  const float* brow = a.bias ? a.bias + cb : nullptr;
#pragma unroll
  for (int n = 0; n < NT; ++n) {
#pragma unroll
    for (int g = 0; g < 4; ++g) {
      const int off = n * 32 + g * 8;
      if (cb + off >= a.N) continue;
      float4 bv = make_float4(0.f, 0.f, 0.f, 0.f), in = make_float4(0.f, 0.f, 0.f, 0.f);
      if (brow) bv = *reinterpret_cast<const float4*>(brow + off);
      if (srow) in = *reinterpret_cast<const float4*>(srow + off);
      const float bb[4] = {bv.x, bv.y, bv.z, bv.w}, ii[4] = {in.x, in.y, in.z, in.w};
      float v[4], gt[4];
#pragma unroll
      for (int j = 0; j < 4; ++j) {
        const float x = acc[n][4 * g + j] + bb[j];
        if (EPI == EPI_BIAS_ACT) {
          v[j] = (a.act == MRG_ACT_RELU) ? (x > 0.f ? x : 0.f) : (a.act == MRG_ACT_SIGMOID ? sigmoidf_fast(x) : x);
        } else if (EPI == EPI_GATE) {
          gt[j] = sigmoidf_fast(x);
          v[j] = gt[j] * ii[j] * cs;
        } else if (EPI == EPI_SCALE) {
          v[j] = x * cs;
        } else {
          v[j] = x + ii[j];
        }
      }
      if (rok) {
        if (cstore) *reinterpret_cast<float4*>(crow + off) = make_float4(v[0], v[1], v[2], v[3]);
        if (EPI == EPI_GATE && xrow) *reinterpret_cast<float4*>(xrow + off) = make_float4(gt[0], gt[1], gt[2], gt[3]);
      }
    }
  }
}

template <int EPI>
// ... 395 lines not shown
```

mr-gnas_amd/csrc/gemm_dispatch.hpp:

```cpp
#pragma once
#include "gemm_x3.hpp"
#include "gemm_x3s.hpp"
#include "gemm_x3s8.hpp"
#include "gemm_x3q.hpp"

namespace mrg {

inline int gemm_mode() { return gemm_switches().mode; }

constexpr int X3Q_MIN_K = 224;
inline bool x3q_shape(int epi, int N, int K) {
  const int q = gemm_switches().q;
  return gemm_mode() == 0 && q != 0 && epi != EPI_SEGMAX && epi != EPI_SEGSUM && N > 128 && N <= X3Q_NT * 16 && K > (q == 2 ? 48 : X3Q_MIN_K);
}

constexpr int X3N_NT = 2;
inline bool x3n_shape(int epi, int64_t rows, int N, int K) {
  return gemm_mode() == 0 && rows > 0 && rows <= gemm_switches().small_rows && gemm_pick_nt(N) > X3N_NT && N <= 224 && !x3q_shape(epi, N, K);
}

inline size_t bsplit_bytes_any(int N, int K) {
  const size_t a = x3_bsplit_bytes(N, K, gemm_pick_nt(N));
  const size_t q = (N > 128 && N <= X3Q_NT * 16) ? x3q_bsplit_bytes(K) : 0;
  const size_t n = (gemm_pick_nt(N) > X3N_NT && N <= 224) ? x3_bsplit_bytes(N, K, X3N_NT) : 0;
  const size_t m = a > q ? a : q;
  return m > n ? m : n;
}

inline void launch_bsplit_any(int epi, int64_t rows, const float* B, int64_t sn, int64_t sk, int N, int K, void* Bp, hipStream_t st) {
  if (x3q_shape(epi, N, K)) {
    const float* Bs[1] = {B};
    void* outs[1] = {Bp};
    launch_bsplitq3(Bs, sn, sk, N, K, outs, 1, st);
  } else {
    launch_bsplit(B, sn, sk, N, K, x3n_shape(epi, rows, N, K) ? X3N_NT : gemm_pick_nt(N), Bp, st);
  }
}
inline void launch_bsplit3_any(int epi, int64_t rows, const float* const* B, int64_t sn, int64_t sk, int N, int K, void* const* out, hipStream_t st,
                               const float* const* B2 = nullptr, int ksplit = 0) {
  if (x3q_shape(epi, N, K)) launch_bsplitq3(B, sn, sk, N, K, out, 3, st, B2, ksplit);
  else launch_bsplit3(B, sn, sk, N, K, x3n_shape(epi, rows, N, K) ? X3N_NT : gemm_pick_nt(N), out, st, B2, ksplit);
}

template <int EPI>
inline int launch_rowgemm_x3_mode(GemmArgs a, const void* Bp, hipStream_t st) {
  if (x3q_shape(EPI, a.N, a.K1 + a.K2)) {
    if (!x3q_eligible(a)) return MRG_E_SHAPE;
    return launch_rowgemm_x3q<EPI>(a, Bp, st);
  }
  if (x3n_shape(EPI, a.rows, a.N, a.K1 + a.K2)) {
    if (!x3_eligible(a)) return MRG_E_SHAPE;
    return launch_rowgemm_x3<EPI>(a, Bp, st, X3N_NT);
  }
  if (gemm_mode() != 2 && x3s_eligible(a)) {
    if constexpr (EPI != EPI_GATE) {
      if (x3s8_eligible<EPI>(a)) return launch_rowgemm_x3s8<EPI>(a, Bp, st);
    }
    return launch_rowgemm_x3s<EPI>(a, Bp, st);
  }
  return launch_rowgemm_x3<EPI>(a, Bp, st);
}

inline size_t gemm_workspace_bytes(int K, int N) {
  const size_t split = bsplit_bytes_any(N, K);
  const size_t transp = (size_t)K * N * sizeof(float);
  return split > transp ? split : transp;
}

template <int EPI>
inline int launch_gemm(GemmArgs a, int64_t b_sn, int64_t b_sk, void* ws, hipStream_t st) {
  if (a.rows <= 0) return MRG_OK;
  if (!a.A2 || a.K2 == 0) { a.A2 = a.A1; a.K2 = 0; }
  const int K = a.K1 + a.K2;
  if (ws && gemm_mode() != 1 && x3_eligible(a)) {
    launch_bsplit_any(EPI, a.rows, a.B, b_sn, b_sk, a.N, K, ws, st);
    return launch_rowgemm_x3_mode<EPI>(a, ws, st);
  }
  if (b_sk != 1) {
    if (!ws) return MRG_E_WORKSPACE;
    launch_transpose(a.B, (float*)ws, (int)(K), a.N, (int)b_sk, st);
    a.B = (const float*)ws;
    a.ldb = K;
  } else {
    a.ldb = (int)b_sn;
  }
  return launch_rowgemm<EPI>(a, st);
}

}
```

mr-gnas_amd/csrc/gemm_x3q.hpp:

```cpp
#pragma once
#include "gemm_x3.hpp"

namespace mrg {

constexpr int X3Q_CHUNK = X3Q_HT * 3 * 1024;
constexpr int X3Q_ROWS = 64;

inline size_t x3q_bsplit_bytes(int K) { return (size_t)x3q_slabs(K) * 2 * X3Q_CHUNK; }

template <int EPI>
__device__ __forceinline__ void gemm_epilogue_q(const GemmArgs& a, f32x4v (&acc)[X3Q_NT], int64_t rowbase, int li, int lh, bool full) {
  if (rowbase >= a.rows) return;
  const int last = (int)((a.rows - 1 - rowbase) < 15 ? (a.rows - 1 - rowbase) : 15);
  const int colw = li < a.N ? li : a.N - 1;
  float* crow[8];
  const float* srow[8];
  float* xrow[8];
  float cs[8];
  bool rok[8];
  const bool cstore = EPI != EPI_GATE || a.C != nullptr;
#pragma unroll
  for (int i = 0; i < 8; ++i) {
    const int row = i + 8 * lh;
    const int rc = row < last ? row : last;
    rok[i] = row <= last;
    crow[i] = a.C + (rowbase + rc) * a.ldc + colw;
    if (EPI == EPI_GATE) srow[i] = a.S + (rowbase + rc) * a.ld_s + colw;
    if (EPI == EPI_ACCUM) srow[i] = a.Cin + (rowbase + rc) * a.ld_cin + colw;
    if (EPI == EPI_GATE) xrow[i] = a.aux ? a.aux + (rowbase + rc) * a.N + colw : nullptr;
    cs[i] = 1.0f;
    if (EPI == EPI_GATE || EPI == EPI_SCALE) cs[i] = a.scale * (a.rowscale ? a.rowscale[rowbase + rc] : 1.0f);
  }
  const int lc = li & 15;
#pragma unroll
  for (int j = 0; j < X3Q_HT; ++j) {
    const int ca = (2 * j) * 16 + lc, cb = (2 * j + 1) * 16 + lc;
    const float bva = a.bias ? a.bias[ca < a.N ? ca : a.N - 1] : 0.f;
    const float bvb = a.bias ? a.bias[cb < a.N ? cb : a.N - 1] : 0.f;
    float acc8[8];
#pragma unroll
    for (int r = 0; r < 4; ++r) {
      float xa = acc[2 * j][r] + bva, xb = acc[2 * j + 1][r] + bvb;
      asm volatile("s_nop 1\n\tv_permlane16_swap_b32 %0, %1" : "+v"(xa), "+v"(xb));
      acc8[r] = xa;
      acc8[4 + r] = xb;
    }
    const int col = j * 32 + li;
    const bool cok = col < a.N;
    const int off = cok ? j * 32 : 0;
    float in[8], v[8], g[8];
#pragma unroll
    for (int i = 0; i < 8; ++i) in[i] = 0.f;
    if ((EPI == EPI_GATE && cstore) || EPI == EPI_ACCUM) {
#pragma unroll
      for (int i = 0; i < 8; ++i) in[i] = srow[i][off];
    }
#pragma unroll
    for (int i = 0; i < 8; ++i) {
      const float x = acc8[i];
      if (EPI == EPI_BIAS_ACT) {
        v[i] = (a.act == MRG_ACT_RELU) ? (x > 0.f ? x : 0.f) : (a.act == MRG_ACT_SIGMOID ? sigmoidf_fast(x) : x);
      } else if (EPI == EPI_GATE) {
        g[i] = sigmoidf_fast(x);
        v[i] = g[i] * in[i] * cs[i];
      } else if (EPI == EPI_SCALE) {
        v[i] = x * cs[i];
      } else {
        v[i] = x + in[i];
      }
    }
    if (full) {
      if (cok) {
        if (cstore) {
#pragma unroll
          for (int i = 0; i < 8; ++i) crow[i][j * 32] = v[i];
        }
        if (EPI == EPI_GATE && a.aux) {
#pragma unroll
          for (int i = 0; i < 8; ++i) xrow[i][j * 32] = g[i];
        }
      }
    } else {
#pragma unroll
      for (int i = 0; i < 8; ++i) {
        if (cok && rok[i]) {
          if (cstore) crow[i][j * 32] = v[i];
          if (EPI == EPI_GATE && a.aux) xrow[i][j * 32] = g[i];
        }
      }
    }
  }
}

constexpr int X3Q_WPS = 3;

template <int EPI, bool DUAL>
__global__ __launch_bounds__(256, X3Q_WPS) void rowgemm_x3q_k(GemmArgs a, const char* __restrict__ Bp) {
  constexpr int NCH = X3Q_HT * 3;
  constexpr int NBW = (NCH + 3) / 4;
  extern __shared__ __align__(16) char smem_q[];
  const int tid = threadIdx.x, wave = __builtin_amdgcn_readfirstlane(tid >> 6), lane = tid & 63;
  const int lr = lane & 15, lg = lane >> 4;
  MRG_GROUP_SELECT(X3Q_ROWS)
  const int64_t roww = row0 + wave * 16;
  const int K = a.K1 + a.K2;
  const int nslab = (K + 31) >> 5;

  f32x4v acc[X3Q_NT];
#pragma unroll
  for (int n = 0; n < X3Q_NT; ++n)
#pragma unroll
    for (int r = 0; r < 4; ++r) acc[n][r] = 0.f;

  const float* ar1; const float* ar2;
  x3_a_row(a, roww + lr, ar1, ar2);
  v4f xr[2][2];
  auto load_a = [&](int slab, v4f (&x)[2]) { x3_load_a<32, DUAL>(x, slab, nslab, lg, ar1, ar2, a.K1, a.K2, K); };
  auto fetch_b = [&](int c) { x3_fetch_b<NCH>(Bq + (int64_t)c * X3Q_CHUNK, smem_q + (c & 1) * X3Q_CHUNK, wave, lane); };
  const unsigned lds0 = (unsigned)(size_t)(lds_ptr_t)smem_q + (unsigned)lane * 16u;
  u32x4 bq[2][3];
  auto read_b = [&](int t, int buf, u32x4 (&q)[3]) { x3_read_b(lds0 + (unsigned)(buf * X3Q_CHUNK + t * 3072), q); };
  u32x4 ch, cm, cl, nh, nm, nl;
// ... 11 lines not shown
    constexpr int HF = decltype(half_c)::value;
    constexpr bool SPLIT = decltype(split_c)::value;
    read_b(0, HF, bq[0]);
#pragma unroll
    for (int t = 0; t < X3Q_HT; ++t) {
      if (t + 1 < X3Q_HT) {
        read_b(t + 1, HF, bq[(t + 1) & 1]);
        asm volatile("s_waitcnt lgkmcnt(3)" ::: "memory");
      } else {
        asm volatile("s_waitcnt lgkmcnt(0)" ::: "memory");
      }
      __builtin_amdgcn_sched_barrier(0);
      if (SPLIT && t < 4) split_pair_of(xn, t, nh, nm, nl);
      const bf16x8 Ah = __builtin_bit_cast(bf16x8, ch), Am = __builtin_bit_cast(bf16x8, cm), Al = __builtin_bit_cast(bf16x8, cl);
      const bf16x8 Bh = __builtin_bit_cast(bf16x8, bq[t & 1][0]), Bm = __builtin_bit_cast(bf16x8, bq[t & 1][1]), Bl = __builtin_bit_cast(bf16x8, bq[t & 1][2]);
      x3_chain(acc[HF * X3Q_HT + t], Ah, Am, Al, Bh, Bm, Bl);
      if (SPLIT) {
#pragma unroll
        for (int i = 0; i < 6; ++i) {
          __builtin_amdgcn_sched_group_barrier(0x008, 1, 0);
          __builtin_amdgcn_sched_group_barrier(0x002, 2, 0);
        }
      }
      __builtin_amdgcn_sched_barrier(0);
    }
  };

  auto slab = [&](auto r_c, int s) {
    constexpr int R = decltype(r_c)::value;
    const bool has_next = s + 1 < nslab;
    if (s > 0) fetch_b(2 * s + 1);
    half_slab(std::integral_constant<int, 0>{}, std::false_type{}, xr[0]);
    asm volatile("s_waitcnt vmcnt(0)" ::: "memory");
    __builtin_amdgcn_s_barrier();
    if (has_next) fetch_b(2 * s + 2);
    load_a(s + 2, xr[R]);
    half_slab(std::integral_constant<int, 1>{}, std::true_type{}, xr[R ^ 1]);
    ch = nh; cm = nm; cl = nl;
    if (has_next) {
      asm volatile("s_waitcnt vmcnt(2)" ::: "memory");
      __builtin_amdgcn_s_barrier();
    }
  };
  int s = 0;
  for (; s + 1 < nslab; s += 2) {
    slab(std::integral_constant<int, 0>{}, s);
    slab(std::integral_constant<int, 1>{}, s + 1);
  }
  if (s < nslab) slab(std::integral_constant<int, 0>{}, s);
  asm volatile("s_waitcnt vmcnt(0)" ::: "memory");
  asm volatile("" :: "v"(xr[0][0]), "v"(xr[0][1]), "v"(xr[1][0]), "v"(xr[1][1]));

  const int li = lane & 31, lh = lane >> 5;
  gemm_epilogue_q<EPI>(a, acc, roww, li, lh, row0 + X3Q_ROWS <= a.rows);
}

inline bool x3q_eligible(const GemmArgs& a) { return x3_eligible(a) && a.rows > 0 && a.N <= X3Q_NT * 16 && !a.row_seg; }

template <int EPI>
inline int launch_rowgemm_x3q(GemmArgs a, const void* Bp, hipStream_t st) {
  if (a.rows <= 0) return MRG_OK;
  if (!a.A2 || a.K2 == 0) { a.A2 = a.A1; a.K2 = 0; }
  const int gbm = X3Q_ROWS;
  if (a.grp.n > 0 && gemm_group_tiles(a.grp, gbm) == 0) return MRG_OK;
  dim3 grid((unsigned)(a.grp.n > 0 ? a.grp.tile0[3] : (a.rows + gbm - 1) / gbm));
  const size_t lds = (size_t)2 * X3Q_CHUNK;
  if constexpr (EPI == EPI_SEGMAX || EPI == EPI_SEGSUM) {
    return MRG_E_SHAPE;
  } else {
    if (a.K2 > 0) return launch_kernel(rowgemm_x3q_k<EPI, true>, grid, dim3(256), lds, st, a, Bp);
    return launch_kernel(rowgemm_x3q_k<EPI, false>, grid, dim3(256), lds, st, a, Bp);
  }
}

}
```

mr-gnas_amd/csrc/gemm_x3s.hpp:

```cpp
#pragma once
#include "gemm_x3.hpp"


namespace mrg {

template <int NT, int EPI, bool DUAL, bool TR>
__global__ __launch_bounds__(256, 2) void rowgemm_x3s_k(GemmArgs a, const char* __restrict__ Bp, int ntile) {
  constexpr int GBM = 128;
  constexpr int NCH = NT * 3;
  constexpr int BSLAB = NCH * 1024;
  constexpr int NBW = (NCH + 3) / 4;
  extern __shared__ __align__(16) char smem_b[];
  const int tid = threadIdx.x, wave = __builtin_amdgcn_readfirstlane(tid >> 6), lane = tid & 63, li = lane & 31, lh = lane >> 5;
  MRG_GROUP_SELECT(GBM)
  const int64_t roww = row0 + wave * 32;
  const int col0 = blockIdx.y * (NT * 32);
  const int K = a.K1 + a.K2;
  const int nslab = (K + 15) >> 4;

  f32x16 acc[NT];
#pragma unroll
  for (int n = 0; n < NT; ++n)
#pragma unroll
    for (int r = 0; r < 16; ++r) acc[n][r] = 0.f;
// ... 38 lines not shown
        read_b(n0 + 2, R, bq2[(pp + 1) & 1][0]);
        if (n1 + 2 < NT) {
          read_b(n1 + 2, R, bq2[(pp + 1) & 1][1]);
          asm volatile("s_waitcnt lgkmcnt(6)" ::: "memory");
        } else {
          asm volatile("s_waitcnt lgkmcnt(3)" ::: "memory");
        }
      } else {
        asm volatile("s_waitcnt lgkmcnt(0)" ::: "memory");
      }
      __builtin_amdgcn_sched_barrier(0);
      if (has_next) {
#pragma unroll
        for (int q = pp * SPP; q < (pp + 1) * SPP && q < 4; ++q) split_pair_of(xr[(R + 1) % 3], q, nh, nm, nl);
      }
      const bf16x8 Ah = __builtin_bit_cast(bf16x8, ch), Am = __builtin_bit_cast(bf16x8, cm), Al = __builtin_bit_cast(bf16x8, cl);
      const bf16x8 Bh0 = __builtin_bit_cast(bf16x8, bq2[pp & 1][0][0]), Bm0 = __builtin_bit_cast(bf16x8, bq2[pp & 1][0][1]),
                   Bl0 = __builtin_bit_cast(bf16x8, bq2[pp & 1][0][2]);
      if (n1 < NT) {
        const bf16x8 Bh1 = __builtin_bit_cast(bf16x8, bq2[pp & 1][1][0]), Bm1 = __builtin_bit_cast(bf16x8, bq2[pp & 1][1][1]),
                     Bl1 = __builtin_bit_cast(bf16x8, bq2[pp & 1][1][2]);
        x3_chain2<TR>(acc[n0], acc[n1], Ah, Am, Al, Bh0, Bm0, Bl0, Ah, Am, Al, Bh1, Bm1, Bl1);
      } else {
        x3_chain<TR>(acc[n0], Ah, Am, Al, Bh0, Bm0, Bl0);
      }
#pragma unroll
      for (int i = 0; i < 12; ++i) {
        __builtin_amdgcn_sched_group_barrier(0x008, 1, 0);
        __builtin_amdgcn_sched_group_barrier(0x002, 3, 0);
      }
      __builtin_amdgcn_sched_barrier(0);
    }
    if (NT < 4 && has_next) {
#pragma unroll
      for (int q = NT; q < 4; ++q) split_pair_of(xr[(R + 1) % 3], q, nh, nm, nl);
    }
    if (has_next) {
      ch = nh; cm = nm; cl = nl;
      wait_vmcnt(2 + nb_issued(s) + 2);
      __builtin_amdgcn_s_barrier();
    }
  };
  int s = 0;
  for (; s + 2 < nslab; s += 3) {
    slab(std::integral_constant<int, 0>{}, s);
    slab(std::integral_constant<int, 1>{}, s + 1);
    slab(std::integral_constant<int, 2>{}, s + 2);
  }
  if (s < nslab) { slab(std::integral_constant<int, 0>{}, s); ++s; }
  if (s < nslab) { slab(std::integral_constant<int, 1>{}, s); ++s; }
  asm volatile("s_waitcnt vmcnt(0)" ::: "memory");
  asm volatile("" :: "v"(xr[0][0]), "v"(xr[0][1]), "v"(xr[1][0]), "v"(xr[1][1]), "v"(xr[2][0]), "v"(xr[2][1]));

  if constexpr (EPI == EPI_SEGMAX) gemm_epilogue_segmax<NT>(a, acc, roww, col0, li, lh);
  else if constexpr (EPI == EPI_SEGSUM) gemm_epilogue_segsum<NT>(a, acc, roww, col0, li, lh);
  else if constexpr (TR) gemm_epilogue_tr<NT, EPI>(a, acc, roww, col0, li, lh);
  else gemm_epilogue<NT, EPI>(a, acc, roww, col0, li, lh, row0 + GBM <= a.rows);
}

inline bool x3s_eligible(const GemmArgs& a) { return x3_eligible(a) && a.rows > 0; }

template <int EPI>
inline int launch_rowgemm_x3s(GemmArgs a, const void* Bp, hipStream_t st) {
  if (a.rows <= 0) return MRG_OK;
  if (!a.A2 || a.K2 == 0) { a.A2 = a.A1; a.K2 = 0; }
  const int nt = gemm_pick_nt(a.N);
  const int ntile = x3_tiles(a.N, nt);
  const int gbm = 128;
  if (a.grp.n > 0 && gemm_group_tiles(a.grp, gbm) == 0) return MRG_OK;
  dim3 grid((unsigned)(a.grp.n > 0 ? a.grp.tile0[3] : (a.rows + gbm - 1) / gbm), (unsigned)(ntile / nt));
  size_t lds = (size_t)3 * nt * 3 * 1024;
  bool tr = false;
  if constexpr (EPI != EPI_SEGMAX && EPI != EPI_SEGSUM) tr = gemm_switches().epilogue == 2 && gemm_epilogue_tr_ok<EPI>(a);
#define MRG_GOS3(NTV, DV, TV) return launch_kernel(rowgemm_x3s_k<NTV, EPI, DV, TV>, grid, dim3(256), lds, st, a, Bp, ntile)
#define MRG_GOS2(NTV, DV)                                                                                             \
  do {                                                                                                                \
    if constexpr (EPI == EPI_SEGMAX || EPI == EPI_SEGSUM) MRG_GOS3(NTV, DV, false);                                   \
    else { if (tr) MRG_GOS3(NTV, DV, true); else MRG_GOS3(NTV, DV, false); }                                          \
  } while (0)
#define MRG_GOS(NTV) do { if (a.K2 > 0) MRG_GOS2(NTV, true); else MRG_GOS2(NTV, false); } while (0)
  switch (nt) {
    case 1: MRG_GOS(1); break;
    case 2: MRG_GOS(2); break;
    case 4: MRG_GOS(4); break;
    default: MRG_GOS(7); break;
  }
#undef MRG_GOS
#undef MRG_GOS2
#undef MRG_GOS3
}

}
```

mr-gnas_amd/csrc/mixedop.hip:

```cpp
#include "common.hpp"

#define MRG_MIX_MAXK 8

namespace mrg {

struct PtrPack { const float* p[MRG_MIX_MAXK]; };
struct MutPack { float* p[MRG_MIX_MAXK]; };
struct RowScalePack { const float* rs[MRG_MIX_MAXK]; float scale[MRG_MIX_MAXK]; float self_scale[MRG_MIX_MAXK]; int64_t edge_rows[MRG_MIX_MAXK]; int on[MRG_MIX_MAXK];
                      const float* full[MRG_MIX_MAXK];
                      const float* s[MRG_MIX_MAXK]; const float* gate[MRG_MIX_MAXK]; float* gs_out[MRG_MIX_MAXK]; int add_from[MRG_MIX_MAXK]; };

struct GatedPack { int k; const float* s; const float* c;
                   int pair_k;
                   int rk; const float* rf;
                   const float* rh; const float* uvc; int uld; int64_t b0, b1; float* rdq;
                   const int32_t* vrows;
                   int act; };

__device__ __forceinline__ int64_t valid_rows(const int32_t* vrows, int64_t rows) {
  if (vrows == nullptr) return rows;
  const int64_t v = (int64_t)*vrows;
  return v < rows ? (v < 0 ? 0 : v) : rows;
}

__device__ __forceinline__ float gated_rowscale(const GatedPack& gp, int64_t r) { return gp.c[r]; }

template <int VEC, int LPR, int KMAX>
__device__ __forceinline__ void colstats_flush(const double (&s1)[KMAX][VEC], const double (&s2)[KMAX][VEC], double* red, double* __restrict__ dst,
                                               int D, int sl, int rw) {
  constexpr int RPB = MRG_BLOCK / LPR;
  constexpr int WIDTH = LPR * KMAX * VEC;
  __syncthreads();
#pragma unroll
  for (int q = 0; q < KMAX; ++q) {
    int c = sl + q * LPR;
#pragma unroll
    for (int j = 0; j < VEC; ++j) {
      red[(rw * 2 + 0) * WIDTH + c * VEC + j] = s1[q][j];
      red[(rw * 2 + 1) * WIDTH + c * VEC + j] = s2[q][j];
    }
  }
  __syncthreads();
  for (int t = threadIdx.x; t < 2 * D; t += MRG_BLOCK) {
    int which = t / D, c = t - which * D;
    double acc = 0.0;
#pragma unroll
    for (int q = 0; q < RPB; ++q) acc += red[(q * 2 + which) * WIDTH + c];
    dst[t] = acc;
  }
}

template <int VEC, int LPR, int KMAX, bool GATED>
__global__ __launch_bounds__(MRG_BLOCK) void mix_colstats_k(PtrPack ys, int K, int64_t rows, int D, double* __restrict__ ws, GatedPack gp) {
  rows = valid_rows(gp.vrows, rows);
  constexpr int RPB = MRG_BLOCK / LPR;
// ... 47 lines not shown
        }
      }
      for (; r < rows; r += step) {
        const float ck = gated_rowscale(gp, r), rf = gp.rf[r];
#pragma unroll
        for (int q = 0; q < KMAX; ++q) {
          int c = sl + q * LPR;
          if (c < dv) {
            const Vec<VEC> sv = Vec<VEC>::load(gp.s + r * D + c * VEC), ga = Vec<VEC>::load(gate + r * D + c * VEC);
#pragma unroll
            for (int j = 0; j < VEC; ++j) {
              double d = (double)sv[j]; s1[q][j] += d; s2[q][j] += d * d;
              d = (double)(ga[j] * sv[j] * ck); t1[q][j] += d; t2[q][j] += d * d;
              d = (double)(sv[j] * rf); u1[q][j] += d; u2[q][j] += d * d;
            }
          }
        }
      }
      if (gp.k >= 0) colstats_flush<VEC, LPR, KMAX>(t1, t2, red, ws + ((int64_t)blockIdx.x * K + gp.k) * 2 * D, D, sl, rw);
      if (gp.pair_k >= 0) colstats_flush<VEC, LPR, KMAX>(s1, s2, red, ws + ((int64_t)blockIdx.x * K + gp.pair_k) * 2 * D, D, sl, rw);
      if (gp.rk >= 0) colstats_flush<VEC, LPR, KMAX>(u1, u2, red, ws + ((int64_t)blockIdx.x * K + gp.rk) * 2 * D, D, sl, rw);
      continue;
    }
    if (y != nullptr) {
      int64_t r = (int64_t)blockIdx.x * RPB + rw;
      for (; r + 3 * step < rows; r += 4 * step) {
#pragma unroll
        for (int q = 0; q < KMAX; ++q) {
          int c = sl + q * LPR;
          if (c < dv) {
            Vec<VEC> v[4];
#pragma unroll
            for (int u = 0; u < 4; ++u) v[u] = Vec<VEC>::load(y + (r + u * step) * D + c * VEC);
#pragma unroll
            for (int u = 0; u < 4; ++u)
#pragma unroll
              for (int j = 0; j < VEC; ++j) { double d = (double)v[u][j]; s1[q][j] += d; s2[q][j] += d * d; }
          }
        }
      }
      for (; r < rows; r += step) {
#pragma unroll
        for (int q = 0; q < KMAX; ++q) {
          int c = sl + q * LPR;
          if (c < dv) {
            Vec<VEC> v = Vec<VEC>::load(y + r * D + c * VEC);
#pragma unroll
            for (int j = 0; j < VEC; ++j) { double d = (double)v[j]; s1[q][j] += d; s2[q][j] += d * d; }
          }
        }
      }
    }
    colstats_flush<VEC, LPR, KMAX>(s1, s2, red, ws + ((int64_t)blockIdx.x * K + k) * 2 * D, D, sl, rw);
  }
}

template <typename T>
__global__ void mix_reduce_k(const T* __restrict__ ws, T* __restrict__ out, int nblocks, int len) {
  int t = blockIdx.x * blockDim.x + threadIdx.x;
  if (t >= len) return;
  T acc = 0;
  for (int b = 0; b < nblocks; ++b) acc += ws[(int64_t)b * len + t];
  out[t] = acc;
}

__global__ void mix_finalize_fwd_k(const double* __restrict__ sums, PtrPack gamma, PtrPack beta, MutPack rmean, MutPack rvar,
                                   int K, double total_rows, int D, float eps, float momentum, float* __restrict__ coef,
                                   const int32_t* __restrict__ vrows) {
  if (vrows) total_rows = *vrows > 0 ? (double)*vrows : 1.0;
  int k = blockIdx.y;
  int c = blockIdx.x * blockDim.x + threadIdx.x;
  if (c >= D || k >= K) return;
  double mean = sums[(k * 2 + 0) * D + c] / total_rows;
  double var = sums[(k * 2 + 1) * D + c] / total_rows - mean * mean;
  if (var < 0) var = 0;
  double invstd = 1.0 / sqrt(var + (double)eps);
  float g = gamma.p[k] ? gamma.p[k][c] : 1.f, b = beta.p[k] ? beta.p[k][c] : 0.f;
  float* o = coef + (int64_t)k * 4 * D;
  o[c] = (float)(g * invstd);
  o[D + c] = (float)(b - mean * g * invstd);
  o[2 * D + c] = (float)invstd;
  o[3 * D + c] = (float)(mean * invstd);
  if (rmean.p[k]) {
    double unbiased = total_rows > 1 ? var * (total_rows / (total_rows - 1.0)) : var;
    rmean.p[k][c] = (1.f - momentum) * rmean.p[k][c] + momentum * (float)mean;
    rvar.p[k][c] = (1.f - momentum) * rvar.p[k][c] + momentum * (float)unbiased;
  }
}

__global__ void mix_reduce_finalize_fwd_k(const double* __restrict__ ws, int nb, PtrPack gamma, PtrPack beta, MutPack rmean, MutPack rvar,
                                          int K, double total_rows, int D, float eps, float momentum, float* __restrict__ coef,
                                          const int32_t* __restrict__ vrows) {
  if (vrows) total_rows = *vrows > 0 ? (double)*vrows : 1.0;
  __shared__ double part[2][16][64];
  const int tx = threadIdx.x & 63, ty = threadIdx.x >> 6;
  const int c = blockIdx.x * 64 + tx, k = blockIdx.y;
  const int ld = K * 2 * D;
#pragma unroll
  for (int j = 0; j < 2; ++j) part[j][ty][tx] = c < D ? ordered_partial<double>(ws, 0, nb, ld, (k * 2 + j) * D + c, ty) : 0.0;
  __syncthreads();
  if (ty != 0 || c >= D) return;
  double tot[2];
#pragma unroll
  for (int j = 0; j < 2; ++j) {
    double t = part[j][0][tx];
#pragma unroll
// ... 654 lines not shown
  gp->vrows = gb ? gb->valid_rows : nullptr;
  if (gb && gb->act != 0 && gb->act != 1) return MRG_E_ENUM;
  gp->act = gb ? gb->act : 0;
  if (gp->act == 1 && (K > 5 || gb->k >= 0 || gb->row_k >= 0)) return MRG_E_SHAPE;
  if (!gb || (gb->k < 0 && gb->row_k < 0)) return MRG_OK;
  if (gb->k >= K || gb->row_k >= K || (gb->k >= 0 && gb->k == gb->row_k)) return MRG_E_SHAPE;
  if (!gb->s) return MRG_E_NULLPTR;
  gp->s = gb->s;
  if (gb->k >= 0) {
    if (!gb->rowscale || !y_host[gb->k]) return MRG_E_NULLPTR;
    gp->k = gb->k; gp->c = gb->rowscale;
  }
  if (gb->row_k >= 0) {
    if (!gb->row_f) return MRG_E_NULLPTR;
    if (y_host[gb->row_k] != gb->s) return MRG_E_SHAPE;
    gp->rk = gb->row_k; gp->rf = gb->row_f;
    if (apply) {
      if (!gb->row_h || !gb->row_uvc || !gb->row_dq) return MRG_E_NULLPTR;
      if (gb->b0 < 0 || gb->b1 < gb->b0 || gb->row_ld <= 0) return MRG_E_SHAPE;
      gp->rh = gb->row_h; gp->uvc = gb->row_uvc; gp->uld = gb->row_ld; gp->b0 = gb->b0; gp->b1 = gb->b1; gp->rdq = gb->row_dq;
      *al = *al && aligned16(gb->row_uvc) && gb->row_ld % 4 == 0;
    }
  }
  if (!gp->c) gp->c = gp->rf;
  if (!gp->rf) gp->rf = gp->c;
  if (!gp->rh) { gp->rh = gp->rf; gp->uvc = gp->s; gp->uld = 0; gp->b0 = gp->b1 = 0; }
  for (int q = 0; q < K; ++q)
    if (q != gb->k && q != gb->row_k && y_host[q] == gb->s) { gp->pair_k = q; break; }
  *al = *al && aligned16(gb->s);
  return MRG_OK;
}

}

using namespace mrg;

extern "C" int64_t mrg_mix_workspace_bytes(int K, int D) {
  if (K < 1 || K > MRG_MIX_MAXK || D <= 0) return 0;
  return (int64_t)1024 * K * 3 * D * sizeof(double);
}

static int mix_colstats_blocks(const float* const* y_host, int K, int64_t rows, int D, void* ws, hipStream_t st, int* grid_out,
                               const mrg_gated_branch* gated);

extern "C" int mrg_mix_stats_coef(const float* const* y_host, const float* const* gamma_host, const float* const* beta_host,
                                  float* const* rmean_host, float* const* rvar_host, int K, int64_t rows, double total_rows, int D, float eps,
                                  float momentum, float* coef, void* ws, const mrg_gated_branch* gated, void* stream) {
  const int32_t* valid_rows = gated ? gated->valid_rows : nullptr;
  if (K < 1 || K > MRG_MIX_MAXK || D <= 0 || total_rows < 0) return MRG_E_SHAPE;
  if (valid_rows && total_rows != (double)rows) return MRG_E_SHAPE;
  if (!coef || !gamma_host || !beta_host) return MRG_E_NULLPTR;
  hipStream_t st = (hipStream_t)stream;
  int grid = 1;
  const int rc = mix_colstats_blocks(y_host, K, rows, D, ws, st, &grid, gated);
  if (rc != MRG_OK) return rc;
  PtrPack ga{}, be{};
  MutPack rm{}, rv{};
  for (int k = 0; k < K; ++k) {
    ga.p[k] = gamma_host[k]; be.p[k] = beta_host[k];
    rm.p[k] = rmean_host ? rmean_host[k] : nullptr;
    rv.p[k] = rvar_host ? rvar_host[k] : nullptr;
    if ((rm.p[k] == nullptr) != (rv.p[k] == nullptr)) return MRG_E_NULLPTR;
  }
  hipLaunchKernelGGL(mix_reduce_finalize_fwd_k, dim3((D + 63) / 64, K), dim3(1024), 0, st, (const double*)ws, grid, ga, be, rm, rv, K,
                     total_rows > 0 ? total_rows : 1.0, D, eps, momentum, coef, valid_rows);
  MRG_LAUNCH_CHECK();
  return MRG_OK;
}

extern "C" int mrg_mix_colstats(const float* const* y_host, int K, int64_t rows, int D, double* sums, void* ws,
                                const mrg_gated_branch* gated, void* stream) {
  if (!sums) return MRG_E_NULLPTR;
  if (gated && gated->valid_rows) return MRG_E_SHAPE;
  hipStream_t st = (hipStream_t)stream;
  int grid = 1;
  const int rc = mix_colstats_blocks(y_host, K, rows, D, ws, st, &grid, gated);
  if (rc != MRG_OK) return rc;
  int len = K * 2 * D;
  launch_ordered_reduce<double>((const double*)ws, sums, 0, grid, len, len, st);
  MRG_LAUNCH_CHECK();
  return MRG_OK;
}

static int mix_colstats_blocks(const float* const* y_host, int K, int64_t rows, int D, void* ws, hipStream_t st, int* grid_out,
                               const mrg_gated_branch* gated) {
  if (!pack_ok((const void* const*)y_host, K)) return MRG_E_SHAPE;
  if (rows < 0 || D <= 0) return MRG_E_SHAPE;
  if (!ws) return MRG_E_WORKSPACE;
  PtrPack ys{};
  bool al = true;
  for (int k = 0; k < K; ++k) { ys.p[k] = y_host[k]; al = al && aligned16(y_host[k]); }
  GatedPack gp;
  const int grc = gated_pack(gated, y_host, K, &gp, &al);
  if (grc != MRG_OK) return grc;
  RowGeom g = row_geom(D, al);
  if (!g.ok) return MRG_E_SHAPE;
  int grid = 1;
#define CALL(V, L, KM)                                                                                    \
  do {                                                                                                    \
    grid = mix_grid(rows, L);                                                                             \
    if (gp.k >= 0 || gp.rk >= 0) hipLaunchKernelGGL((mix_colstats_k<V, L, KM, true>), dim3(grid), dim3(MRG_BLOCK), 0, st, ys, K, rows, D, (double*)ws, gp); \
    else hipLaunchKernelGGL((mix_colstats_k<V, L, KM, false>), dim3(grid), dim3(MRG_BLOCK), 0, st, ys, K, rows, D, (double*)ws, gp); \
  } while (0)
  MRG_DISPATCH_GEOM(g, CALL);
#undef CALL
  MRG_LAUNCH_CHECK();
  *grid_out = grid;
  return MRG_OK;
}

extern "C" int mrg_mix_finalize_fwd(const double* sums, const float* const* gamma_host, const float* const* beta_host,
                                    float* const* rmean_host, float* const* rvar_host, int K, double total_rows, int D,
                                    float eps, float momentum, float* coef, void* stream) {
  if (K < 1 || K > MRG_MIX_MAXK || D <= 0 || total_rows < 0) return MRG_E_SHAPE;
  if (!sums || !coef || !gamma_host || !beta_host) return MRG_E_NULLPTR;
  PtrPack ga{}, be{};
  MutPack rm{}, rv{};
  for (int k = 0; k < K; ++k) {
    ga.p[k] = gamma_host[k]; be.p[k] = beta_host[k];
    rm.p[k] = rmean_host ? rmean_host[k] : nullptr;
    rv.p[k] = rvar_host ? rvar_host[k] : nullptr;
    if ((rm.p[k] == nullptr) != (rv.p[k] == nullptr)) return MRG_E_NULLPTR;
  }
  hipLaunchKernelGGL(mix_finalize_fwd_k, dim3((D + 127) / 128, K), dim3(128), 0, (hipStream_t)stream, sums, ga, be, rm, rv, K,
                     total_rows > 0 ? total_rows : 1.0, D, eps, momentum, coef, (const int32_t*)nullptr);
  MRG_LAUNCH_CHECK();
// ... 323 lines not shown
```

mr-gnas_amd/functional/__init__.py:

```python
from . import switches
from ._base import (
    bump_counters, deferred_counters,
    COMPOSE, REDUCE, ACT, gate_ld, same_rows, _same_memory, _cnt, _ws, _WS_BYTES, _ws_bytes, _SIDE_STREAMS, Fork,
)
from .candidates import (
    Link, Candidate,
)
from .gcs import (
    GCS, fused_gcs, span_gcs, ComposePlan, _ComposeAggregate, compose_aggregate,
)
from .reducers import (
    _seg_fwd, _seg_bwd, _SegReduce, seg_reduce, _AggRows, aggregate_rows, _fused_agg_ws, _LinReluAgg, linear_relu_aggregate,
    _LinReluPartial, linear_relu_partial, _SumPartial, sum_partial,
)
from .fanin import (
    sum_buffers, _Fanout, _FanBox, Fan,
)
from .compose_gather import (
    _Compose, compose, gather_rows, GatherPlan, _Gather, gather, LazyRows, _pair_meta, _GatherCompose,
)
from .gates import (
    _Gate, gate_comp, gate_last, _GateRow, gate_comp_row_factor,
)
from .row_linear import (
    _Linear, linear, module_linear,
)
from .dense import (
    _DenseFilter, _FoldHalves, dense_filter_comp, _DensePair, dense_pair_available, _GATED_C, _gated_rowscale, dense_filter_pair,
    dense_filter_single,
)
from .mixed import (
    _MixCfg, _row_candidate_as_s, _MixedEpilogue, mixed_epilogue, PreparedEpilogue, _all_reduce_sum, StatChain,
    mixed_epilogue_prepare,
)
from .cell_zero import (
    _CellZeroMixed, cell_zero_mixed,
)
from .scoring import (
    ScorePlan, _DistMult, distmult_score, distmult_scores_all, _TransE, transe_scores_all,
)
from .ccorr import (
    _CCorrRows, _Circulant, ccorr,
)
from .conve import (
    _ConvEFeatures, conve_features, conve_scores, drop_masks, hip_path_ok,
)
from .nc import (
    _SegStd, aggregate_std, inv_in_degree, aggregate_nc, linear_relu_aggregate_nc,
)
from .._lib import ptr_array, call, f32c, ptr, require_hip, stream_of
```

mr-gnas_amd/functional/candidates.py:

```python
import torch

from .. import _lib


class Link:

    __slots__ = ("folded", "written", "gs_direct", "s", "gate", "row_h", "row_uvc", "row_written")

    def __init__(self, slots=1):
        self.folded = [False] * slots
        self.written = [None] * slots
        self.gs_direct = None
        self.s = self.gate = None
        self.row_h = self.row_uvc = None
        self.row_written = None

    def claim(self, slot):
        if self.folded[slot]:
            return False
        self.folded[slot] = True
        return True

    def arrived(self, slot, g, what):
        if not self.folded[slot] or self.written[slot] is None:
            return False
        if self.written[slot] != g.data_ptr():
            raise _lib.MrgnasError(f"{what}: the folded epilogue gradient was combined with another consumer's gradient; "
                                   "call mixed_epilogue(fold_row_scales=False) when a candidate's output is read elsewhere")
        return True


class Candidate:

    __slots__ = ("kind", "y", "s", "c", "rowscale", "link", "slot", "b0", "b1")

    def __init__(self, kind, y, link=None, slot=0, s=None, c=None, rowscale=None, b0=0, b1=0):
        self.kind, self.y, self.link, self.slot, self.s, self.c, self.rowscale, self.b0, self.b1 = kind, y, link, slot, s, c, rowscale, b0, b1

    def materialize(self):
        if self.kind == "stored":
            return self.y
        if self.kind == "rowfactor":
            return self.s * self.y.unsqueeze(1)
        return self.y * self.s * self.c.unsqueeze(1)
```

mr-gnas_amd/functional/dense.py:

```python
import weakref

import torch

from .. import _lib
from .._lib import ptr_array, call, f32c, ptr, require_hip, stream_of
from . import switches as SW
from ._base import Fork, _ws, _ws_bytes, same_rows
from .candidates import Candidate, Link


class _DenseFilter(torch.autograd.Function):

    @staticmethod
    def forward(ctx, link, kind, s, s_in, norm, b0, b1, scale_edge, scale_self, *params):
        s, s_in, norm = f32c(s), f32c(s_in), f32c(norm)
        params = tuple(f32c(p) for p in params)
        require_hip(s, s_in, norm, *params)
        M, D = s.shape
        st = stream_of(s)
        out = torch.empty_like(s)
        gate = torch.empty_like(s) if kind == 0 else None
        ctx.link = link
        if link is not None:
            link.s, link.gate = s, (gate.detach() if gate is not None else None)
        K_ = 2 * D if s_in is not None else D
        ws3 = int(_lib.load().mrg_dense_filter3_workspace_bytes(D, K_)) if (SW.GROUPED_SEGMENTS and all(params[2 * i] is not None for i in range(3))) else 0
        if ws3 > 0:
            call("mrg_dense_filter_fwd3", (kind, ptr(s), ptr(s_in), ptr_array([params[0], params[2], params[4]]),
                                           ptr_array([params[1], params[3], params[5]]), ptr(norm), scale_edge, scale_self, ptr(out), ptr(gate),
                                           ptr(_ws(ws3, s)), b0, b1, M, D, st),
                 nbytes=4 * M * (K_ + D * (2 if kind == 0 else 1)), flops=2 * M * K_ * D)
            ctx.cfg = (kind, b0, b1, scale_edge, scale_self)
            ctx.save_for_backward(s, s_in, norm, gate, *params)
            return out
        segs = [(i, lo, hi, scale, edge) for i, (lo, hi, scale, edge) in
                enumerate(((0, b0, scale_edge, True), (b0, b1, scale_edge, True), (b1, M, scale_self, False))) if hi > lo]
        gws = [_ws(_ws_bytes("mrg_gemm_workspace_bytes", K_, D), s) for _ in segs]
        fork = Fork(s.device, len(segs) if M >= SW.FORK_MIN_ROWS else 1)
        for j, (i, lo, hi, scale, edge) in enumerate(segs):
            W, b = params[2 * i], params[2 * i + 1]
            rs = norm[lo:hi] if (edge and norm is not None) else None
            with fork.on(j):
                call("mrg_dense_filter_fwd", (kind, ptr(s[lo:hi]), ptr(s_in[lo:hi]) if s_in is not None else None, ptr(W), ptr(b),
                                              ptr(rs), scale, ptr(out[lo:hi]), ptr(gate[lo:hi]) if gate is not None else None,
                                              ptr(gws[j]), hi - lo, D, stream_of(s)),
                     nbytes=4 * (hi - lo) * (K_ + D * (2 if kind == 0 else 1)), flops=2 * (hi - lo) * K_ * D)
        fork.join()
        ctx.cfg = (kind, b0, b1, scale_edge, scale_self)
        ctx.save_for_backward(s, s_in, norm, gate, *params)
        return out

    @staticmethod
    def backward(ctx, g):
        s, s_in, norm, gate, *params = ctx.saved_tensors
        kind, b0, b1, scale_edge, scale_self = ctx.cfg
        g = f32c(g)
        M, D = s.shape
        st = stream_of(s)
        prescaled = ctx.link is not None and ctx.link.arrived(0, g, "dense filter")
        if prescaled and kind == 0:
            gs = ctx.link.gs_direct
# ... 57 lines not shown
                call("mrg_linear_bwd_input", (ptr(w["dz"]), ptr(W), ptr(gs[sl]), ptr(w["wt"]), rows, D, D, K_, int(kind == 0), st), **gwork)
                if s_in is not None:
                    call("mrg_linear_bwd_input", (ptr(w["dz"]), ptr(W[:, D:]), ptr(gs_in[sl]), ptr(w["wt2"]), rows, D, D, K_, 0, st), **gwork)
                call("mrg_linear_bwd_weight_share", (ptr(w["dz"]), ptr(s[sl]), ptr(s_in[sl]) if s_in is not None else None, ptr(w["gW"]),
                                                     ptr(w["gb"]), ptr(w["ws"]), rows, D, D if s_in is not None else 0, D, share, st),
                     nbytes=4 * rows * (D + K_), flops=2 * rows * K_ * D)
        fork.join()
        return (None, None, gs, gs_in, None, None, None, None, None, *grads)


class _FoldHalves(torch.autograd.Function):

    @staticmethod
    def forward(ctx, *Ws):
        Ws = tuple(f32c(W) for W in Ws)
        Ws3 = (Ws + (None, None, None))[:3]
        ref = next(W for W in Ws3 if W is not None)
        require_hip(*Ws3)
        D = ref.shape[0]
        buf = torch.empty(3, D, D, dtype=torch.float32, device=ref.device)
        call("mrg_fold_halves3", (ptr_array(Ws3), ptr(buf), D, stream_of(ref)), nbytes=12 * D * D * sum(W is not None for W in Ws3))
        ctx.meta = (D, [W is not None for W in Ws3], len(Ws), ref.device)
        return tuple(buf[i] if Ws3[i] is not None else None for i in range(len(Ws)))

    @staticmethod
    def backward(ctx, *gs):
        D, present, n, dev = ctx.meta
        src = [f32c(gs[i]) if (i < n and present[i] and gs[i] is not None) else None for i in range(3)]
        gWs = [torch.empty(D, 2 * D, dtype=torch.float32, device=dev) if (i < n and present[i]) else None for i in range(3)]
        ref = next(t for t in gWs if t is not None)
        call("mrg_unfold_halves3", (ptr_array(src), ptr_array(gWs), D, stream_of(ref)), nbytes=12 * D * D * sum(present))
        return tuple(gWs[:n])


def dense_filter_comp(kind, s, s_in, norm, b0, b1, W_in, b_in, W_out, b_out, W_self, b_self, self_scale, for_epilogue=False):
    if s_in is not None and same_rows(s, s_in):
        W_in, W_out, W_self = _FoldHalves.apply(W_in, W_out, W_self)
        s_in = None
    norm = f32c(norm)
    if norm is not None and norm.numel() < int(b1):
        raise _lib.MrgnasError(f"dense filter: edge norm has {norm.numel()} entries, the edge rows need {int(b1)}")
    fold = for_epilogue and SW.FOLD_ROW_SCALE and f32c(s).is_cuda and torch.is_grad_enabled()
    link = Link() if fold else None
    y = _DenseFilter.apply(link, kind, s, s_in, norm, int(b0), int(b1), 1.0 / 3.0, float(self_scale),
                           W_in, b_in, W_out, b_out, W_self, b_self)
    if fold and y.requires_grad:
        return Candidate("stored", y, link=link, slot=0, rowscale=(norm, int(b1), 1.0 / 3.0, float(self_scale), kind == 0))
    return y


class _DensePair(torch.autograd.Function):

    @staticmethod
    def forward(ctx, link, s, s_in, norm, b0, b1, gate_only, *params):
        s, s_in, norm = f32c(s), f32c(s_in), f32c(norm)
        params = tuple(f32c(p) for p in params)
        require_hip(s, s_in, norm, *params)
        M, D = s.shape
        st = stream_of(s)
        K_ = 2 * D if s_in is not None else D
        ws3 = int(_lib.load().mrg_dense_filter3_workspace_bytes(D, K_))
        out_c, gate = torch.empty_like(s), torch.empty_like(s)
        out_d = gate if gate_only else torch.empty_like(s)
        dW, dB, cW = [params[0], params[2], params[4]], [params[1], params[3], params[5]], list(params[6:9])
        work = dict(flops=2 * M * K_ * D)
        call("mrg_dense_filter_fwd3", (0, ptr(s), ptr(s_in), ptr_array(dW), ptr_array(dB), ptr(norm), 1.0 / 3.0, 1.0 / 3.0,
                                       None if gate_only else ptr(out_d), ptr(gate), ptr(_ws(ws3, s)), b0, b1, M, D, st),
             nbytes=4 * M * (K_ + (1 if gate_only else 2) * D), **work)
        call("mrg_dense_filter_fwd3", (1, ptr(s), ptr(s_in), ptr_array(cW), ptr_array([None, None, None]), ptr(norm), 1.0 / 3.0, 1.0, ptr(out_c), None,
                                       ptr(_ws(ws3, s)), b0, b1, M, D, st), nbytes=4 * M * (K_ + D), **work)
        ctx.cfg = (b0, b1)
        ctx.save_for_backward(s, s_in, norm, gate, *params)
        ctx.link = link
        if link is not None:
            link.s, link.gate = s, gate.detach()
        return out_d, out_c

    @staticmethod
    def backward(ctx, g_d, g_c):
        s, s_in, norm, gate, *params = ctx.saved_tensors
        b0, b1 = ctx.cfg
        M, D = s.shape
        st = stream_of(s)
        g_d, g_c = f32c(g_d), f32c(g_c)
        pres = [ctx.link is not None and ctx.link.arrived(i, g, "dense filter pair") for i, g in enumerate((g_d, g_c))]
        K_ = 2 * D if s_in is not None else D
        dW, cW = [params[0], params[2], params[4]], list(params[6:9])
        if pres[0]:
            dz_d, gs = g_d, ctx.link.gs_direct
            gs.record_stream(torch.cuda.current_stream())
        else:
            dz_d, gs = torch.empty_like(s), torch.empty_like(s)
            call("mrg_dense_filter_dz3", (0, ptr(g_d), ptr(s), ptr(gate), ptr(norm), 1.0 / 3.0, 1.0 / 3.0, ptr(dz_d), ptr(gs), b1, M, D, st),
                 nbytes=4 * M * D * 5)
        if pres[1]:
            dz_c = g_c
        else:
            dz_c = torch.empty_like(s)
            call("mrg_dense_filter_dz3", (1, ptr(g_c), ptr(s), None, ptr(norm), 1.0 / 3.0, 1.0, ptr(dz_c), None, b1, M, D, st), nbytes=4 * M * D * 2)
        lib = _lib.load()
        wsp = int(lib.mrg_linear_bwd_input3_pair_workspace_bytes(D, D))
        gwork = dict(nbytes=4 * M * 3 * D + 24 * D * D, flops=4 * M * D * D)
        call("mrg_linear_bwd_input3_pair", (ptr(dz_d), ptr(dz_c), ptr_array(dW), ptr_array(cW), ptr(gs), ptr(_ws(wsp, s)), b0, b1, M, D, D, K_, 1, st),
             nbytes=4 * M * 4 * D + 24 * D * D, flops=4 * M * D * D)
        gs_in = None
        if s_in is not None:
            gs_in = torch.empty_like(s)
            call("mrg_linear_bwd_input3_pair", (ptr(dz_d), ptr(dz_c), ptr_array([W[:, D:] for W in dW]), ptr_array([W[:, D:] for W in cW]), ptr(gs_in),
                                                ptr(_ws(wsp, s)), b0, b1, M, D, D, K_, 0, st), **gwork)
        wsw = int(lib.mrg_linear_bwd_weight3_workspace_bytes(b0, b1, M, D, K_ - D, D))
        g_dW = [torch.empty_like(W) for W in dW]
        g_dB = [torch.empty_like(params[2 * i + 1]) for i in range(3)]
        g_cW = [torch.empty_like(W) for W in cW]
        wwork = dict(nbytes=4 * M * (D + K_), flops=2 * M * K_ * D)
        call("mrg_linear_bwd_weight3", (ptr(dz_d), ptr(s), ptr(s_in), ptr_array(g_dW), ptr_array(g_dB), ptr(_ws(wsw, s)), b0, b1, M, D, K_ - D, D, st), **wwork)
        call("mrg_linear_bwd_weight3", (ptr(dz_c), ptr(s), ptr(s_in), ptr_array(g_cW), ptr_array([None, None, None]), ptr(_ws(wsw, s)), b0, b1, M, D, K_ - D, D, st),
             **wwork)
        grads_d = [t for pair in zip(g_dW, g_dB) for t in pair]
        return (None, gs, gs_in, None, None, None, None, *grads_d, *g_cW)


def dense_pair_available(D, tied):
    if not (SW.DENSE_PAIR and SW.GROUPED_SEGMENTS):
        return False
    lib = _lib.load()
    K_ = D if tied else 2 * D
    return (int(lib.mrg_dense_filter3_workspace_bytes(D, K_)) > 0 and int(lib.mrg_linear_bwd_input3_pair_workspace_bytes(D, D)) > 0
            and int(lib.mrg_linear_bwd_weight3_workspace_bytes(1, 2, 3, D, K_ - D, D)) > 0)
_GATED_C = {}


def _gated_rowscale(norm, b1, M, scale_edge, scale_self, device):
    base = None if norm is None else (norm._base if norm._base is not None else norm)
    key = (None if norm is None else (norm.data_ptr(), norm._version), b1, M, scale_edge, scale_self, str(device))
    hit = _GATED_C.get(key)
    if hit is not None and (norm is None or hit[0]() is base):
        return hit[1]
    c = torch.empty(M, dtype=torch.float32, device=device)
    if norm is None:
        c[:b1] = scale_edge
    else:
        torch.mul(norm[:b1], scale_edge, out=c[:b1])
    c[b1:] = scale_self
    if len(_GATED_C) > 64:
        _GATED_C.clear()
    import weakref
    _GATED_C[key] = (weakref.ref(base) if base is not None else None, c)
    return c


def dense_filter_pair(s, s_in, norm, b0, b1, dense_params, comp_weights, gate_only=False, for_epilogue=False):
    dW, dB = list(dense_params[0::2]), list(dense_params[1::2])
    cW = list(comp_weights)
    if s_in is not None and same_rows(s, s_in):
        dW = list(_FoldHalves.apply(*dW))
        cW = list(_FoldHalves.apply(*cW))
        s_in = None
    norm = f32c(norm)
    if norm is not None and norm.numel() < int(b1):
        raise _lib.MrgnasError(f"dense filter: edge norm has {norm.numel()} entries, the edge rows need {int(b1)}")
    s = f32c(s)
    gate_only = bool(gate_only and for_epilogue and s.is_cuda)
    fold = for_epilogue and SW.FOLD_ROW_SCALE and s.is_cuda and torch.is_grad_enabled()
    link = Link(2) if fold else None
    y_d, y_c = _DensePair.apply(link, s, s_in, norm, int(b0), int(b1), gate_only, dW[0], dB[0], dW[1], dB[1], dW[2], dB[2], *cW)
    if not for_epilogue:
        return y_d, y_c
    fold = fold and y_d.requires_grad
    rs_d = (norm, int(b1), 1.0 / 3.0, 1.0 / 3.0, True) if fold else None
    rs_c = (norm, int(b1), 1.0 / 3.0, 1.0, False) if fold else None
    if gate_only:
        c_d = Candidate("gate", y_d, link=link, slot=0, s=s, c=_gated_rowscale(norm, int(b1), s.shape[0], 1.0 / 3.0, 1.0 / 3.0, s.device), rowscale=rs_d)
    else:
        c_d = Candidate("stored", y_d, link=link, slot=0, rowscale=rs_d)
    return c_d, Candidate("stored", y_c, link=link, slot=1, rowscale=rs_c)


def dense_filter_single(s, s_in, W, b):
    if s_in is not None and same_rows(s, s_in):
        (W,) = _FoldHalves.apply(W)
        s_in = None
    return _DenseFilter.apply(None, 0, s, s_in, None, 0, 0, 1.0, 1.0, None, None, None, None, W, b)
```

mr-gnas_amd/functional/gates.py:

```python
import torch

from .. import _lib
from .._lib import ptr_array, call, f32c, ptr, require_hip, stream_of
from ._base import _ws, _ws_bytes, gate_ld, same_rows
from .candidates import Candidate, Link


class _Gate(torch.autograd.Function):

    @staticmethod
    def forward(ctx, s, s_in, norm, b0, b1, scale, *params):
        tied = s_in is not None and same_rows(s, s_in)
        s, s_in, norm = f32c(s), (None if tied else f32c(s_in)), f32c(norm)
        params = tuple(f32c(p) for p in params)
        require_hip(s, s_in, norm, *params)
        M, D = s.shape
        st = stream_of(s)
        in_dim = 2 * D if (s_in is not None or tied) else D
        Ws, bs, as_ = params[0::3], params[1::3], params[2::3]
        uvc = torch.empty(3, gate_ld(D), dtype=torch.float32, device=s.device)
        call("mrg_gate_collapse3", (ptr_array(Ws), ptr_array(bs), ptr_array(as_), ptr(uvc), D, in_dim, int(tied), st),
             nbytes=4 * D * in_dim * sum(W is not None for W in Ws))
        out = torch.empty_like(s)
        nb = 4 * D * M * (3 if s_in is not None else 2) + (4 * b1 if norm is not None else 0)
        call("mrg_gate_fwd", (ptr(s), ptr(s_in), ptr(norm), ptr(uvc), ptr(out), b0, b1, M, D, scale, st), nbytes=nb)
        ctx.save_for_backward(s, s_in, norm, uvc, *params)
        ctx.cfg = (b0, b1, scale, in_dim, tied)
        return out

    @staticmethod
    def backward(ctx, g):
        s, s_in, norm, uvc, *params = ctx.saved_tensors
        b0, b1, scale, in_dim, tied = ctx.cfg
        g = f32c(g)
        M, D = s.shape
        st = stream_of(s)
        gs = torch.empty_like(s)
        gs_in = torch.empty_like(s) if s_in is not None else None
        d_uvc = torch.empty(3, gate_ld(D), dtype=torch.float32, device=s.device)
        ws = _ws(_ws_bytes("mrg_gate_bwd_workspace_bytes", M, D), s)
        nb = 4 * D * M * (5 if s_in is not None else 3) + (4 * b1 if norm is not None else 0)
        call("mrg_gate_bwd", (ptr(g), ptr(s), ptr(s_in), ptr(norm), ptr(uvc), ptr(gs), ptr(gs_in), ptr(d_uvc), ptr(ws),
                              b0, b1, M, D, scale, st), nbytes=nb)
        Ws, bs, as_ = params[0::3], params[1::3], params[2::3]
        gWs = [None if W is None else torch.empty_like(W) for W in Ws]
        gbs = [None if b is None else torch.empty_like(b) for b in bs]
        gas = [None if a is None else torch.empty_like(a) for a in as_]
        call("mrg_gate_param_grad3", (ptr_array(Ws), ptr_array(bs), ptr_array(as_), ptr(d_uvc), ptr_array(gWs), ptr_array(gbs), ptr_array(gas),
                                      D, in_dim, int(tied), st), nbytes=8 * D * in_dim * sum(W is not None for W in Ws))
        gparams = []
        for gW, gb, ga in zip(gWs, gbs, gas):
            gparams += [gW, gb, ga]
        return (gs, gs_in, None, None, None, None, *gparams)


def gate_comp(s, s_in, norm, b0, b1, W_in, b_in, a_in, W_out, b_out, a_out, W_self, b_self, a_self):
    return _Gate.apply(s, s_in, norm, int(b0), int(b1), 1.0 / 3.0, W_in, b_in, a_in, W_out, b_out, a_out, W_self, b_self, a_self)


def gate_last(s, W, b, a):
    return _Gate.apply(s, None, None, 0, 0, 1.0, None, None, None, None, None, None, W, b, a)


class _GateRow(torch.autograd.Function):

    @staticmethod
    def forward(ctx, link, s, s_in, norm, b0, b1, scale, *params):
        tied = s_in is not None and same_rows(s, s_in)
        s, s_in, norm = f32c(s), (None if tied else f32c(s_in)), f32c(norm)
        params = tuple(f32c(p) for p in params)
        require_hip(s, s_in, norm, *params)
        M, D = s.shape
        st = stream_of(s)
        in_dim = 2 * D if (s_in is not None or tied) else D
        Ws, bs, as_ = params[0::3], params[1::3], params[2::3]
        uvc = torch.empty(3, gate_ld(D), dtype=torch.float32, device=s.device)
        call("mrg_gate_collapse3", (ptr_array(Ws), ptr_array(bs), ptr_array(as_), ptr(uvc), D, in_dim, int(tied), st),
             nbytes=4 * D * in_dim * sum(W is not None for W in Ws))
        fvec = torch.empty(M, dtype=torch.float32, device=s.device)
        hvec = torch.empty(M, dtype=torch.float32, device=s.device)
        nb = 4 * D * M * (2 if s_in is not None else 1) + (4 * b1 if norm is not None else 0) + 8 * M
        call("mrg_gate_row_fwd", (ptr(s), ptr(s_in), ptr(norm), ptr(uvc), ptr(fvec), ptr(hvec), b0, b1, M, D, scale, st), nbytes=nb)
        ctx.save_for_backward(s, s_in, norm, uvc, hvec, *params)
        ctx.cfg = (b0, b1, scale, in_dim, tied)
        ctx.link = link
        if link is not None:
            link.row_h, link.row_uvc = hvec, uvc
        return fvec

    @staticmethod
    def backward(ctx, gq):
        s, s_in, norm, uvc, hvec, *params = ctx.saved_tensors
        b0, b1, scale, in_dim, tied = ctx.cfg
        gq = f32c(gq)
        M, D = s.shape
        st = stream_of(s)
        gs_in = torch.empty_like(s) if s_in is not None else None
        d_uvc = torch.empty(3, gate_ld(D), dtype=torch.float32, device=s.device)
        ws = _ws(_ws_bytes("mrg_gate_bwd_workspace_bytes", M, D), s)
        nb = 4 * D * M * (3 if s_in is not None else 1) + 8 * M
        call("mrg_gate_row_bwd", (ptr(gq), ptr(hvec), ptr(s), ptr(s_in), ptr(uvc), ptr(gs_in), ptr(d_uvc), ptr(ws), b0, b1, M, D, st), nbytes=nb)
        Ws, bs, as_ = params[0::3], params[1::3], params[2::3]
        gWs = [None if W is None else torch.empty_like(W) for W in Ws]
        gbs = [None if b is None else torch.empty_like(b) for b in bs]
        gas = [None if a is None else torch.empty_like(a) for a in as_]
        call("mrg_gate_param_grad3", (ptr_array(Ws), ptr_array(bs), ptr_array(as_), ptr(d_uvc), ptr_array(gWs), ptr_array(gbs), ptr_array(gas),
                                      D, in_dim, int(tied), st), nbytes=8 * D * in_dim * sum(W is not None for W in Ws))
        gparams = []
        for gW, gb, ga in zip(gWs, gbs, gas):
            gparams += [gW, gb, ga]
        gs = None
        folded = ctx.link.row_written if ctx.link is not None else None
        if ctx.link is not None:
            ctx.link.row_written = None
        if folded is not None and folded != gq.data_ptr():
            raise _lib.MrgnasError("f_sparse_comp (row factor): the MixedOp epilogue folded the gradient w.r.t. s, but a different gradient "
                                   "tensor reached the factor's node -- the factor has a second consumer, which the folded form does not support")
        if folded is None:
            dz = gq * hvec
            gs = torch.empty_like(s)
            for seg, (lo, hi) in enumerate(((0, b0), (b0, b1), (b1, M))):
                if hi > lo:
                    torch.mul(dz[lo:hi, None], uvc[seg, :D][None, :], out=gs[lo:hi])
        return (None, gs, gs_in, None, None, None, None, *gparams)


def gate_comp_row_factor(s, s_in, norm, b0, b1, W_in, b_in, a_in, W_out, b_out, a_out, W_self, b_self, a_self):
    s = f32c(s)
    link = Link()
    fvec = _GateRow.apply(link, s, s_in, norm, int(b0), int(b1), 1.0 / 3.0, W_in, b_in, a_in, W_out, b_out, a_out, W_self, b_self, a_self)
    return Candidate("rowfactor", fvec, link=link, s=s, b0=int(b0), b1=int(b1))
```

mr-gnas_amd/functional/mixed.py:

```python
import torch

from .. import _lib
from .._lib import ptr_array, call, f32c, ptr, require_hip, stream_of
from . import switches as SW
from ._base import _same_memory, _ws, _ws_bytes, bump_counters
from .candidates import Candidate
from .dense import _gated_rowscale


class _MixCfg:

    def __init__(self, bns, present, group=None, total_rows=None, has_addend=False, rowscale=None, identity=None, gated=None, act=0,
                 valid_rows=None):
        self.bns, self.present, self.group, self.total_rows, self.has_addend = bns, present, group, total_rows, has_addend
        self.act = act
        self.valid_rows = valid_rows
        self.gated = gated
        self.chain = None
        self.identity = identity
        self.rowscale = rowscale


def _row_candidate_as_s(cfg, ys):
    if cfg.gated is not None and cfg.gated.get("row_k") is not None:
        ys = list(ys)
        ys[cfg.gated["row_k"]] = cfg.gated["s"]
    return ys


class _MixedEpilogue(torch.autograd.Function):
    @staticmethod
    def forward(ctx, cfg, w, *tensors):
        from .._lib import ptr_array
        K_ = len(cfg.bns)
        nz = sum(cfg.present)
        ys_nz = [f32c(t) for t in tensors[:nz]]
        gam, bet = list(tensors[nz:nz + K_]), list(tensors[nz + K_:nz + 2 * K_])
        addend = f32c(tensors[nz + 2 * K_]) if cfg.has_addend else None
        it = iter(ys_nz)
        ys = [next(it) if p else None for p in cfg.present]
        ys = _row_candidate_as_s(cfg, ys)
        ref = next((y for y in ys if y is not None), None)
        if ref is None:
            raise _lib.MrgnasError("mixed epilogue needs at least one non-zero branch to know the row count")
        require_hip(w, addend, *ys_nz, *gam, *bet)
        rows, D = ref.shape
        dev, st = ref.device, stream_of(ref)
        w = f32c(w)
        total = float(cfg.total_rows if cfg.total_rows is not None else rows)
        coef = torch.empty(K_, 4, D, dtype=torch.float32, device=dev)
        ypa = ptr_array(ys)
        gb = _lib.gated_branch(cfg.gated, act=cfg.act, valid_rows=cfg.valid_rows)
        nz_rd = len({y.data_ptr() for y in ys if y is not None} | ({cfg.gated["s"].data_ptr()} if cfg.gated is not None else set()))
        bn0 = cfg.bns[0]
        training = bn0.training or not bn0.track_running_stats
        if training:
            ws = _ws(_ws_bytes("mrg_mix_workspace_bytes", K_, D), ref)
            track = bn0.track_running_stats
            rm = ptr_array([b.running_mean if track else None for b in cfg.bns])
            rv = ptr_array([b.running_var if track else None for b in cfg.bns])
            mom = bn0.momentum if bn0.momentum is not None else 0.1
            if cfg.group is None:
                call("mrg_mix_stats_coef", (ypa, ptr_array(gam), ptr_array(bet), rm, rv, K_, rows, total, D, bn0.eps, mom, ptr(coef), ptr(ws), gb, st),
                     nbytes=4 * D * rows * nz_rd)
            else:
                import torch.distributed as dist
                if cfg.chain is not None and cfg.chain[0].sums is not None:
                    sums = cfg.chain[0].sums[cfg.chain[1]]
                else:
                    sums = torch.empty(K_, 2, D, dtype=torch.float64, device=dev)
                    call("mrg_mix_colstats", (ypa, K_, rows, D, ptr(sums), ptr(ws), gb, st), nbytes=4 * D * rows * nz_rd)
                    _all_reduce_sum(sums, cfg.group)
                call("mrg_mix_finalize_fwd", (ptr(sums), ptr_array(gam), ptr_array(bet), rm, rv, K_, total, D, bn0.eps, mom, ptr(coef), st))
            if track:
                bump_counters(cfg.bns)
        else:
            for k, b in enumerate(cfg.bns):
                invstd = torch.rsqrt(b.running_var + b.eps)
                coef[k, 0] = gam[k] * invstd
                coef[k, 1] = bet[k] - b.running_mean * gam[k] * invstd
                coef[k, 2] = invstd
                coef[k, 3] = b.running_mean * invstd
        out = torch.empty(rows, D, dtype=torch.float32, device=dev)
        call("mrg_mix_fwd", (ypa, K_, ptr(coef), ptr(w), ptr(addend), ptr(out), rows, D, gb, st), nbytes=4 * D * rows * (nz_rd + 1 + (addend is not None)))
        if SW.MASK_TAP is not None:
            masks = []
            for k in range(K_):
                one = torch.zeros(K_, dtype=torch.float32, device=dev)
                one[k] = 1.0
                o = torch.empty(rows, D, dtype=torch.float32, device=dev)
                call("mrg_mix_fwd", (ypa, K_, ptr(coef), ptr(one), None, ptr(o), rows, D, gb, st))
                masks.append(o > 0)
            SW.MASK_TAP(cfg.bns, masks)
        ctx.cfg, ctx.training, ctx.total, ctx.nz, ctx.nz_rd = cfg, training, total, nz, nz_rd
        ctx.save_for_backward(w, coef, *ys_nz)
        if cfg.chain is not None:
            cfg.chain[0].register(cfg.chain[1], ctx)
        return out

    @staticmethod
    def _launch_bwd_reduce(ctx, g, red):
        from .._lib import ptr_array
        w, coef, *ys_nz = ctx.saved_tensors
        cfg, K_ = ctx.cfg, len(ctx.cfg.bns)
        it = iter(ys_nz)
        ys = _row_candidate_as_s(cfg, [next(it) if p else None for p in cfg.present])
        rows, D = g.shape
        ws = _ws(_ws_bytes("mrg_mix_workspace_bytes", K_, D), g)
        call("mrg_mix_bwd_reduce", (ptr(g), ptr_array(ys), K_, ptr(coef), ptr(w), ptr(red), ptr(ws), rows, D,
                                    _lib.gated_branch(cfg.gated, act=cfg.act, valid_rows=cfg.valid_rows), stream_of(g)),
             nbytes=4 * D * rows * (ctx.nz_rd + 1))

    @staticmethod
    def backward(ctx, g):
        from .._lib import ptr_array
        w, coef, *ys_nz = ctx.saved_tensors
        cfg, K_, nz = ctx.cfg, len(ctx.cfg.bns), ctx.nz
# ... 178 lines not shown
            D = g.shape[1]
            red = torch.empty(sum(ks), 3, D, dtype=torch.float32, device=g.device)
            off, loc = 0, []
            for i, c in enumerate(self.ctx):
                launch(c, g, red[off:off + ks[i]])
                loc.append(red[off:off + ks[i]])
                off += ks[i]
            glob = red.clone()
            _all_reduce_sum(glob, self.group)
            off, gl = 0, []
            for k_ in ks:
                gl.append(glob[off:off + k_])
                off += k_
            self.bwd = (g.data_ptr(), loc, gl, g)
        return self.bwd[1][j], self.bwd[2][j]


def mixed_epilogue_prepare(ys, bns, group=None, total_rows=None, fold_row_scales=False, identity=None, act="relu", valid_rows=None):
    from ..lazy import real as _real_tensor
    if valid_rows is not None and group is not None:
        raise _lib.MrgnasError("mixed epilogue: a device row count (valid_rows) counts the launch's own rows, not sharded ones")
    ys = [_real_tensor(y) for y in ys]
    cands = [y if isinstance(y, Candidate) else None for y in ys]
    ys = [c.y if c is not None else y for c, y in zip(cands, ys)]
    present = [y is not None for y in ys]
    rowscale = [None] * len(ys)
    if fold_row_scales:
        for k, c in enumerate(cands):
            if c is not None and c.rowscale is not None and c.link is not None and c.link.claim(c.slot):
                rowscale[k] = c.rowscale[:4] + (c.link if c.rowscale[4] else None, c.link, c.slot)
    gated = None
    for k, c in enumerate(cands):
        if c is not None and c.kind == "gate":
            if gated is not None:
                raise _lib.MrgnasError("mixed epilogue: one recomputed (gate-only) candidate at most")
            gated = dict(k=k, s=c.s, c=c.c)
    ys = list(ys)
    for k, c in enumerate(cands):
        if c is None or c.kind != "rowfactor":
            continue
        y, s_r, rb0, rb1 = c.y, c.s, c.b0, c.b1
        D_ = s_r.shape[1]
        wants_grad = torch.is_grad_enabled() and (y.requires_grad or s_r.requires_grad)
        aligned = all(t.data_ptr() % 16 == 0 for t in [s_r] + [t for t in ys if t is not None and t.dim() == 2])
        ok = (gated is not None and "row_k" not in gated and _same_memory(gated["s"], s_r)
              and ((D_ % 4 == 0 and D_ <= 256 and aligned) or D_ <= 64))
        if ok and wants_grad:
            rs_g = rowscale[gated["k"]]
            ok = rs_g is not None and rs_g[4] is not None and y.requires_grad and c.link is not None
        if ok:
            gated.update(row_k=k, row_f=y, b0=rb0, b1=rb1, row_link=c.link if wants_grad else None)
        else:
            ys[k] = c.materialize()
    cfg = _MixCfg(list(bns), present, group, total_rows, False, rowscale, identity, gated, _lib.ACTS[act], valid_rows)
    return PreparedEpilogue(cfg, [y for y in ys if y is not None], list(bns))
```

mr-gnas_amd/functional/switches.py:

```python
import os

ROW_FACTOR = os.environ.get("MRG_ROW_FACTOR", "1") == "1"
LAZY_ASUM = os.environ.get("MRG_LAZY_ASUM", "1") == "1"
FUSED_AMAX = os.environ.get("MRG_FUSED_AMAX", "1") == "1"
FUSED_AMAX_MIN_ROWS = int(os.environ.get("MRG_FUSED_AMAX_MIN_ROWS", "100000"))
FUSED_AMEAN = os.environ.get("MRG_FUSED_AMEAN", "1") == "1"
WIDE_BWD_INPUT = os.environ.get("MRG_WIDE_BWD_INPUT", "1") == "1"
NODE_LINEAR = os.environ.get("MRG_NODE_LINEAR", "1") == "1"
MASK_TAP = None
FOLD_IDENTITY = os.environ.get("MRG_FOLD_IDENTITY", "1") == "1"
CELL_ZERO_FUSED = os.environ.get("MRG_CELL_ZERO_FUSED", "1") == "1"
FORK_MIN_ROWS = int(os.environ.get("MRG_FORK_MIN_ROWS", str(1 << 17)))
SEGMENT_STREAMS = int(os.environ.get("MRG_SEGMENT_STREAMS", "3"))
FOLD_ROW_SCALE = os.environ.get("MRG_FOLD_ROW_SCALE", "1") == "1"
GROUPED_SEGMENTS = os.environ.get("MRG_GROUPED_SEGMENTS", "1") == "1"
DENSE_PAIR = os.environ.get("MRG_DENSE_PAIR", "1") == "1"
GATED_RECOMPUTE = os.environ.get("MRG_GATED_RECOMPUTE", "1") == "1"
COMPGCN_TAIL = os.environ.get("MRG_COMPGCN_TAIL", "1") == "1"
SPARSE_AMAX_BWD = os.environ.get("MRG_SPARSE_AMAX_BWD", "1") == "1"
CCORR_PATH = None
```

mr-gnas_amd/operations_lp.py:

```python
import torch
import torch.nn as nn
import torch.nn.functional as F

from . import functional as K
from . import lazy as LZ

LZ.install_indexing()

PRE_OPS = ['pre_mult', 'pre_sub', 'pre_add']
FIRST_OPS = ['f_zero', 'f_identity', 'f_dense_comp', 'f_sparse_comp', 'f_comp']
MIDDLE_OPS = ['a_max', 'a_sum', 'a_mean']
LAST_OPS = ['f_zero', 'f_identity', 'f_dense_last', 'f_sparse_last']
SF_OPS = ['sf_TransE', 'sf_DisMult']


def _bounds(g):
    if hasattr(g, "bounds"):
        return g.bounds()
    E = g.num_edges()
    return E // 2, E


class _Operator(nn.Module):

# ... 26 lines not shown
class pre_add_op(_PreOp):
    kind = "add"


def _rows_now(x):
    return x.materialize() if isinstance(x, K.LazyRows) else LZ.real(x)


ccorr = K.ccorr


class pre_corr_op(_Operator):

    def __init__(self):
        super().__init__()

    def forward(self, g, src_emb, hr):
        if LZ.wanted(src_emb):
            return LZ.defer(self, g, src_emb, hr, self.out_shape(g, src_emb))
        return self.run(g, src_emb, hr)

    def run(self, g, src_emb, hr, for_epilogue=False):
        src_emb, hr = _rows_now(src_emb), _rows_now(hr)
        return K.ccorr(src_emb, hr.expand_as(src_emb))


class f_identity_op(_Operator):
    def run(self, g, src_emb, src_emb_in, for_epilogue=False):
        return LZ.real(src_emb)


class f_zero_op(_Operator):
    def run(self, g, src_emb, src_emb_in, for_epilogue=False):
        return 0 * LZ.real(src_emb)


class f_sparse_op_comp(_Operator):

    def __init__(self, args):
        super().__init__()
        D = self._feature_dim = args.get('feature_dim', 100)
        for x in ("in", "out", "self"):
            setattr(self, "W_" + x, nn.Linear(2 * D, D, bias=True))
            setattr(self, "a_" + x, nn.Linear(D, 1, bias=False))

    def run(self, g, src_emb, src_emb_in, for_epilogue=False):
        src_emb, src_emb_in = LZ.real(src_emb), LZ.real(src_emb_in)
        b0, b1 = _bounds(g)
        p = []
        for x in ("in", "out", "self"):
            W, a = getattr(self, "W_" + x), getattr(self, "a_" + x)
            p += [W.weight, W.bias, a.weight]
        if for_epilogue and K.switches.ROW_FACTOR and src_emb.is_cuda:
            return K.gate_comp_row_factor(src_emb, src_emb_in, g.norm_flat(), b0, b1, *p)
        return K.gate_comp(src_emb, src_emb_in, g.norm_flat(), b0, b1, *p)


class f_sparse_op_last(_Operator):
    def __init__(self, args):
        super().__init__()
        D = self._feature_dim = args.get('feature_dim', 100)
        self.W = nn.Linear(D, D, bias=True)
        self.a = nn.Linear(D, 1, bias=False)

    def run(self, g, src_emb, src_emb_in, for_epilogue=False):
        return K.gate_last(LZ.real(src_emb), self.W.weight, self.W.bias, self.a.weight)


class f_sparse_op(_Operator):

    def __init__(self, args):
        super().__init__()
        D = self._feature_dim = args.get('feature_dim', 100)
        self.W = nn.Linear(2 * D, D, bias=True)
        self.a = nn.Linear(D, 1, bias=False)

    def run(self, g, src_emb, src_emb_in, for_epilogue=False):
        src_emb, src_emb_in = LZ.real(src_emb), LZ.real(src_emb_in)
        none3 = [None, None, None]
        return K._Gate.apply(src_emb, src_emb_in, None, 0, 0, 1.0, *none3, *none3, self.W.weight, self.W.bias, self.a.weight)


class f_dense_op_comp(_Operator):
    def __init__(self, args):
        super().__init__()
        D = self._feature_dim = args.get('feature_dim', 100)
        self.W_in = nn.Linear(2 * D, D, bias=True)
        self.W_out = nn.Linear(2 * D, D, bias=True)
        self.W_self = nn.Linear(2 * D, D, bias=True)

    def run(self, g, src_emb, src_emb_in, for_epilogue=False):
        src_emb, src_emb_in = LZ.real(src_emb), LZ.real(src_emb_in)
        b0, b1 = _bounds(g)
        return K.dense_filter_comp(0, src_emb, src_emb_in, g.norm_flat(), b0, b1, self.W_in.weight, self.W_in.bias,
                                   self.W_out.weight, self.W_out.bias, self.W_self.weight, self.W_self.bias, 1.0 / 3.0,
                                   for_epilogue=for_epilogue and src_emb.is_cuda)


class f_comp_op(_Operator):
    def __init__(self, args):
        super().__init__()
        D = self._feature_dim = args.get('feature_dim', 100)
        self.W_in = nn.Linear(2 * D, D, bias=False)
        self.W_out = nn.Linear(2 * D, D, bias=False)
        self.W_self = nn.Linear(2 * D, D, bias=False)

    def run(self, g, src_emb, src_emb_in, for_epilogue=False):
# ... 150 lines not shown
```

Baseline: 11.18.

## Compute batch-norm column statistics inside producer kernels for mixed epilogue

Gate-row and dense-filter forward kernels gain colsum variants that accumulate per-block double-precision column sums and sums of squares while writing their outputs. These partials are passed through the gated-branch struct as given statistics, so the mixed epilogue's stats pass can skip re-reading those candidate tensors. The goal is to remove a full read of large edge-row activations per candidate, at the cost of shared-memory reductions, extra partial buffers and more complex plumbing across streams.

Result: faster. 11.34 (median of 6 runs) (+1.5%).

```diff
diff --git a/include/mrgnas.h b/include/mrgnas.h
--- a/include/mrgnas.h
+++ b/include/mrgnas.h
@@ -7,7 +7,7 @@
 extern "C" {
 #endif
 
-#define MRG_ABI_VERSION 19
+#define MRG_ABI_VERSION 20
 
 #define MRG_OK            0
 #define MRG_E_NULLPTR    -1
@@ -62,6 +62,9 @@
                  int64_t b0, int64_t b1, int64_t M, int D, float scale, void *stream);
 int mrg_gate_row_fwd(const float *s, const float *s_in, const float *norm, const float *uvc, float *fvec, float *hvec,
                      int64_t b0, int64_t b1, int64_t M, int D, float scale, void *stream);
+int64_t mrg_gate_row_colsum_blocks(int64_t b0, int64_t b1, int64_t M, int D, int vec4);
+int mrg_gate_row_fwd_colsum(const float *s, const float *s_in, const float *norm, const float *uvc, float *fvec, float *hvec,
+                            int64_t b0, int64_t b1, int64_t M, int D, float scale, void *stream, double *colsum, int64_t colsum_blocks);
 int mrg_gate_row_bwd(const float *q, const float *hvec, const float *s, const float *s_in, const float *uvc, float *gs_in, float *d_uvc,
                      void *ws, int64_t b0, int64_t b1, int64_t M, int D, void *stream);
 
@@ -119,6 +122,7 @@
 int mrg_clip_sgd_step(void *const *params, const void *const *grads, void *const *bufs, const int32_t *chunk_tensor,
                       const int64_t *chunk_off, const int32_t *chunk_len, int64_t n_chunks, double *partial, float *norm_coef,
                       float max_norm, float lr, float momentum, float weight_decay, void *stream);
+#define MRG_MIX_MAX_CANDIDATES 8
 typedef struct mrg_gated_branch {
   int32_t k;
   const float *s;
@@ -132,6 +136,9 @@
   float *row_dq;
   int32_t act;
   const int32_t *valid_rows;
+  const double *given[MRG_MIX_MAX_CANDIDATES];
+  int32_t given_n[MRG_MIX_MAX_CANDIDATES];
+  int64_t given_stride[MRG_MIX_MAX_CANDIDATES];
 } mrg_gated_branch;
 int mrg_mix_colstats(const float *const *y_host, int K, int64_t rows, int D, double *sums, void *ws,
                      const mrg_gated_branch *gated, void *stream);
@@ -209,6 +216,10 @@
 int mrg_dense_filter_fwd3(int kind, const float *s, const float *s_in, const float *const *W, const float *const *bias,
                           const float *norm, float scale_edge, float scale_self, float *out, float *gate, void *ws,
                           int64_t b0, int64_t b1, int64_t M, int D, void *stream);
+int64_t mrg_dense_filter3_colsum_blocks(int kind, int64_t b0, int64_t b1, int64_t M, int D, int K);
+int mrg_dense_filter_fwd3_colsum(int kind, const float *s, const float *s_in, const float *const *W, const float *const *bias,
+                                 const float *norm, float scale_edge, float scale_self, float *out, float *gate, void *ws,
+                                 int64_t b0, int64_t b1, int64_t M, int D, void *stream, double *colsum, int64_t colsum_blocks);
 int mrg_dense_filter_dz3(int kind, const float *g, const float *s, const float *gate, const float *norm, float scale_edge,
                          float scale_self, float *dz, float *gs, int64_t b1, int64_t M, int D, void *stream);
 int64_t mrg_linear_bwd_input3_workspace_bytes(int K, int Nout);
diff --git a/mr-gnas_amd/_lib.py b/mr-gnas_amd/_lib.py
--- a/mr-gnas_amd/_lib.py
+++ b/mr-gnas_amd/_lib.py
@@ -8,7 +8,7 @@
 LIB_PATH = os.environ.get("MRG_LIB_PATH") or os.path.join(_HERE, "lib", "libmrgnas_hip.so")
 HEADER_PATH = os.path.join(os.path.dirname(_HERE), "include", "mrgnas.h")
 
-ABI_VERSION = 19
+ABI_VERSION = 20
 
 
 class MrgnasLibraryError(RuntimeError):
@@ -44,6 +44,8 @@
     "mrg_sum_rows_gather": (_I, [_P, _I, _P, _P, _P, _L, _L, _I, _P, _P]),
     "mrg_distmult_score": (_I, [_P, _P, _P, _P, _P, _P, _L, _I, _P]),
     "mrg_gate_row_fwd": (_I, [_P, _P, _P, _P, _P, _P, _L, _L, _L, _I, _F, _P]),
+    "mrg_gate_row_colsum_blocks": (_L, [_L, _L, _L, _I, _I]),
+    "mrg_gate_row_fwd_colsum": (_I, [_P, _P, _P, _P, _P, _P, _L, _L, _L, _I, _F, _P, _P, _L]),
     "mrg_gate_row_bwd": (_I, [_P, _P, _P, _P, _P, _P, _P, _P, _L, _L, _L, _I, _P]),
     "mrg_mix_workspace_bytes": (_L, [_I, _I]),
     "mrg_mix_colstats": (_I, [_P, _I, _L, _I, _P, _P, _P, _P]),
@@ -79,6 +81,8 @@
     "mrg_linear_fwd": (_I, [_P, _P, _P, _P, _P, _L, _I, _I, _I, _P]),
     "mrg_dense_filter3_workspace_bytes": (_L, [_I, _I]),
     "mrg_dense_filter_fwd3": (_I, [_I, _P, _P, _P, _P, _P, _F, _F, _P, _P, _P, _L, _L, _L, _I, _P]),
+    "mrg_dense_filter3_colsum_blocks": (_L, [_I, _L, _L, _L, _I, _I]),
+    "mrg_dense_filter_fwd3_colsum": (_I, [_I, _P, _P, _P, _P, _P, _F, _F, _P, _P, _P, _L, _L, _L, _I, _P, _P, _L]),
     "mrg_dense_filter_dz3": (_I, [_I, _P, _P, _P, _P, _F, _F, _P, _P, _L, _L, _I, _P]),
     "mrg_linear_bwd_input3_workspace_bytes": (_L, [_I, _I]),
     "mrg_linear_bwd_input3": (_I, [_P, _P, _P, _P, _L, _L, _L, _I, _I, _I, _I, _P]),
@@ -192,10 +196,11 @@
     print(f"[mrg] {name} {shown}", file=sys.stderr, flush=True)
 
 
-def call(name, args, nbytes=0, flops=0):
-    fn = _FN.get(name)
+def call(name, args, nbytes=0, flops=0, symbol=None):
+    sym = symbol or name
+    fn = _FN.get(sym)
     if fn is None:
-        fn = _FN[name] = getattr(load(), name)
+        fn = _FN[sym] = getattr(load(), sym)
     if TRACE:
         _trace(name, args)
         code = fn(*args)
@@ -236,21 +241,36 @@
     _fields_ = [("k", ctypes.c_int32), ("s", ctypes.c_void_p), ("rowscale", ctypes.c_void_p),
                 ("row_k", ctypes.c_int32), ("row_f", ctypes.c_void_p), ("row_h", ctypes.c_void_p), ("row_uvc", ctypes.c_void_p),
                 ("row_ld", ctypes.c_int32), ("b0", ctypes.c_int64), ("b1", ctypes.c_int64), ("row_dq", ctypes.c_void_p),
-                ("act", ctypes.c_int32), ("valid_rows", ctypes.c_void_p)]
+                ("act", ctypes.c_int32), ("valid_rows", ctypes.c_void_p),
+                ("given", ctypes.c_void_p * 8), ("given_n", ctypes.c_int32 * 8), ("given_stride", ctypes.c_int64 * 8)]
+
+
+class ColSums:
+
+    __slots__ = ("buf", "offset", "n", "stride", "rows")
+
+    def __init__(self, buf, offset, n, stride, rows):
+        self.buf, self.offset, self.n, self.stride, self.rows = buf, int(offset), int(n), int(stride), int(rows)
 
 
 ACTS = {"relu": 0, "tanh": 1}
 
 
-def gated_branch(spec, row_dq=None, act=0, valid_rows=None):
+def gated_branch(spec, row_dq=None, act=0, valid_rows=None, given=None):
     dp = lambda t: None if t is None else t.data_ptr()
+    if given is not None and not any(c is not None for c in given):
+        given = None
     if spec is None:
-        if not act and valid_rows is None:
+        if not act and valid_rows is None and given is None:
             return None
-        return ctypes.byref(GatedBranch(-1, None, None, -1, None, None, None, 0, 0, 0, None, int(act), dp(valid_rows)))
-    g = GatedBranch(int(spec.get("k", -1)), dp(spec["s"]), dp(spec.get("c")), int(spec.get("row_k", -1)), dp(spec.get("row_f")),
-                    dp(spec.get("row_h")), dp(spec.get("row_uvc")), int(spec.get("row_ld", 0)), int(spec.get("b0", 0)), int(spec.get("b1", 0)),
-                    dp(row_dq), int(act), dp(valid_rows))
+        g = GatedBranch(-1, None, None, -1, None, None, None, 0, 0, 0, None, int(act), dp(valid_rows))
+    else:
+        g = GatedBranch(int(spec.get("k", -1)), dp(spec["s"]), dp(spec.get("c")), int(spec.get("row_k", -1)), dp(spec.get("row_f")),
+                        dp(spec.get("row_h")), dp(spec.get("row_uvc")), int(spec.get("row_ld", 0)), int(spec.get("b0", 0)), int(spec.get("b1", 0)),
+                        dp(row_dq), int(act), dp(valid_rows))
+    for k, c in enumerate(given or ()):
+        if c is not None:
+            g.given[k], g.given_n[k], g.given_stride[k] = c.buf.data_ptr() + c.offset, c.n, c.stride
     return ctypes.byref(g)
 
 
diff --git a/mr-gnas_amd/cell_lp.py b/mr-gnas_amd/cell_lp.py
--- a/mr-gnas_amd/cell_lp.py
+++ b/mr-gnas_amd/cell_lp.py
@@ -20,6 +20,13 @@
 
 def _tensor(y):
     return y.y if isinstance(y, K.Candidate) else y
+
+
+def _record_stream(y, stream):
+    _tensor(y).record_stream(stream)
+    for c in (getattr(y, "sums", None), getattr(y, "s_sums", None)):
+        if c is not None:
+            c.buf.record_stream(stream)
 
 
 def _plain(h):
@@ -68,6 +75,9 @@
     pair = _dense_pair(ops, fh.x)
     paired = {}
     row_ok = pair is not None and K.switches.GATED_RECOMPUTE and K.switches.FOLD_ROW_SCALE
+    bn0 = bns[0]
+    want = K.ForEpilogue(stats=K.switches.PRODUCER_STATS and group is None and (bn0.training or not bn0.track_running_stats)
+                         and _valid_rows(g, [fh.x]) is None)
     dev = fh.x.device
     nstreams = min(MIXED_STREAMS, n) if fh.x.shape[0] >= K.switches.FORK_MIN_ROWS else 1
     if nstreams <= 1:
@@ -77,10 +87,10 @@
                 ys.append(None)
             elif pair is not None and k in pair:
                 if not paired:
-                    paired[pair[0]], paired[pair[1]] = OPS.dense_pair_forward(ops[pair[0]], ops[pair[1]], g, fh.take(), fi.take(), for_epilogue=True)
+                    paired[pair[0]], paired[pair[1]] = OPS.dense_pair_forward(ops[pair[0]], ops[pair[1]], g, fh.take(), fi.take(), for_epilogue=want)
                 ys.append(paired[k])
             elif (row_ok and type(op) is OPS.f_sparse_op_comp) or type(op) in (OPS.f_dense_op_comp, OPS.f_comp_op):
-                ys.append(_run(op, g, fh.take(), fi.take(), for_epilogue=True))
+                ys.append(_run(op, g, fh.take(), fi.take(), for_epilogue=want))
             else:
                 ys.append(_run(op, g, fh.take(), fi.take()))
         prep = K.mixed_epilogue_prepare(ys, bns, group, total_rows, True, _identity_index(ops), valid_rows=_valid_rows(g, ys))
@@ -101,14 +111,14 @@
             b.record_stream(side)
         with torch.cuda.stream(side):
             if pair is not None and k in pair:
-                paired[pair[0]], paired[pair[1]] = OPS.dense_pair_forward(ops[pair[0]], ops[pair[1]], g, a, b, for_epilogue=True)
+                paired[pair[0]], paired[pair[1]] = OPS.dense_pair_forward(ops[pair[0]], ops[pair[1]], g, a, b, for_epilogue=want)
                 y = paired[k]
-                _tensor(paired[pair[0] + pair[1] - k]).record_stream(fork.main)
+                _record_stream(paired[pair[0] + pair[1] - k], fork.main)
             elif (row_ok and type(op) is OPS.f_sparse_op_comp) or type(op) in (OPS.f_dense_op_comp, OPS.f_comp_op):
-                y = _run(op, g, a, b, for_epilogue=True)
+                y = _run(op, g, a, b, for_epilogue=want)
             else:
                 y = _run(op, g, a, b)
-        _tensor(y).record_stream(fork.main)
+        _record_stream(y, fork.main)
         ys.append(y)
     fork.join()
     prep = K.mixed_epilogue_prepare(ys, bns, group, total_rows, True, _identity_index(ops), valid_rows=_valid_rows(g, ys))
diff --git a/mr-gnas_amd/csrc/dense.hip b/mr-gnas_amd/csrc/dense.hip
--- a/mr-gnas_amd/csrc/dense.hip
+++ b/mr-gnas_amd/csrc/dense.hip
@@ -67,9 +67,22 @@
   return 3 * (int64_t)(((int64_t)bsplit_bytes_any(D, K) + 255) / 256 * 256);
 }
 
-extern "C" int mrg_dense_filter_fwd3(int kind, const float* s, const float* s_in, const float* const* W_host, const float* const* bias_host,
-                                     const float* norm, float scale_edge, float scale_self, float* out, float* gate, void* ws,
-                                     int64_t b0, int64_t b1, int64_t M, int D, void* stream) {
+static void dense3_groups(GemmArgs& a, int64_t b0, int64_t b1, int64_t M, const float* const* bias_host, const float* norm, float scale_edge,
+                          float scale_self, size_t each) {
+  const int64_t lo[3] = {0, b0, b1}, hi[3] = {b0, b1, M};
+  a.grp.n = 3;
+  a.grp.bp_stride = (int64_t)each;
+  for (int i = 0; i < 3; ++i) {
+    a.grp.lo[i] = lo[i]; a.grp.hi[i] = hi[i] > lo[i] ? hi[i] : lo[i];
+    a.grp.bias[i] = bias_host ? bias_host[i] : nullptr;
+    a.grp.scale[i] = i < 2 ? scale_edge : scale_self;
+    a.grp.use_rowscale[i] = (i < 2 && norm) ? 1 : 0;
+  }
+}
+
+static int dense_filter_fwd3(int kind, const float* s, const float* s_in, const float* const* W_host, const float* const* bias_host,
+                             const float* norm, float scale_edge, float scale_self, float* out, float* gate, void* ws,
+                             int64_t b0, int64_t b1, int64_t M, int D, void* stream, double* colsum, int64_t colsum_blocks) {
   if (kind != 0 && kind != 1) return MRG_E_ENUM;
   if (D <= 0 || M < 0 || b0 < 0 || b1 < b0 || M < b1) return MRG_E_SHAPE;
   const int K = s_in ? 2 * D : D;
@@ -88,22 +101,44 @@
   if (kind == 0) { a.S = s; a.ld_s = D; a.aux = gate; }
   if (!x3_eligible(a)) return MRG_E_SHAPE;
   const float* Bs[3]; void* outs[3];
-  a.grp.n = 3;
-  a.grp.bp_stride = (int64_t)each;
+  dense3_groups(a, b0, b1, M, bias_host, norm, scale_edge, scale_self, each);
   for (int i = 0; i < 3; ++i) {
     const bool live = hi[i] > lo[i];
     if (live && !W_host[i]) return MRG_E_NULLPTR;
     Bs[i] = live ? W_host[i] : nullptr;
     outs[i] = (char*)ws + i * each;
-    a.grp.lo[i] = lo[i]; a.grp.hi[i] = live ? hi[i] : lo[i];
-    a.grp.bias[i] = bias_host ? bias_host[i] : nullptr;
-    a.grp.scale[i] = i < 2 ? scale_edge : scale_self;
-    a.grp.use_rowscale[i] = (i < 2 && norm) ? 1 : 0;
   }
   launch_bsplit3_any(kind == 0 ? EPI_GATE : EPI_SCALE, M, Bs, K, 1, D, K, outs, st);
   MRG_LAUNCH_CHECK();
+  if (colsum) {
+    if (gemm_colsum_blocks(kind == 0 ? EPI_GATE : EPI_SCALE, a) != colsum_blocks) return MRG_E_SHAPE;
+    gemm_set_colsum(a, colsum);
+    if (kind == 0) return launch_rowgemm_x3_mode_colsum<EPI_GATE_SUMS>(a, outs[0], st);
+    return launch_rowgemm_x3_mode_colsum<EPI_SCALE_SUMS>(a, outs[0], st);
+  }
   if (kind == 0) return launch_rowgemm_x3_mode<EPI_GATE>(a, outs[0], st);
   return launch_rowgemm_x3_mode<EPI_SCALE>(a, outs[0], st);
+}
+
+extern "C" int mrg_dense_filter_fwd3(int kind, const float* s, const float* s_in, const float* const* W_host, const float* const* bias_host,
+                                     const float* norm, float scale_edge, float scale_self, float* out, float* gate, void* ws,
+                                     int64_t b0, int64_t b1, int64_t M, int D, void* stream) {
+  return dense_filter_fwd3(kind, s, s_in, W_host, bias_host, norm, scale_edge, scale_self, out, gate, ws, b0, b1, M, D, stream, nullptr, 0);
+}
+
+extern "C" int64_t mrg_dense_filter3_colsum_blocks(int kind, int64_t b0, int64_t b1, int64_t M, int D, int K) {
+  if ((kind != 0 && kind != 1) || !dense3_shape_ok(D, K) || b0 < 0 || b1 < b0 || M < b1 || M <= 0) return 0;
+  GemmArgs a{};
+  a.K1 = D; a.K2 = K - D; a.N = D; a.rows = M;
+  dense3_groups(a, b0, b1, M, nullptr, nullptr, 1.f, 1.f, 0);
+  return gemm_colsum_blocks(kind == 0 ? EPI_GATE : EPI_SCALE, a);
+}
+
+extern "C" int mrg_dense_filter_fwd3_colsum(int kind, const float* s, const float* s_in, const float* const* W_host, const float* const* bias_host,
+                                            const float* norm, float scale_edge, float scale_self, float* out, float* gate, void* ws,
+                                            int64_t b0, int64_t b1, int64_t M, int D, void* stream, double* colsum, int64_t colsum_blocks) {
+  if (!colsum) return MRG_E_NULLPTR;
+  return dense_filter_fwd3(kind, s, s_in, W_host, bias_host, norm, scale_edge, scale_self, out, gate, ws, b0, b1, M, D, stream, colsum, colsum_blocks);
 }
 
 static int dense_dz_launch(int kind, const float* g, const float* s, const float* gate, const float* rowscale, float scale, float* dz,
diff --git a/mr-gnas_amd/csrc/gate.hip b/mr-gnas_amd/csrc/gate.hip
--- a/mr-gnas_amd/csrc/gate.hip
+++ b/mr-gnas_amd/csrc/gate.hip
@@ -256,6 +256,75 @@
       const float t = scale * nv;
       hvec[r] = t * gt * (1.0f - gt);
     }
+  }
+}
+
+template <int VEC, int LPR, bool HAS_IN>
+__global__ __launch_bounds__(MRG_BLOCK) void gate_row_fwd_colsum_k(const float* __restrict__ s, const float* __restrict__ sin_,
+                                                                   const float* __restrict__ norm, const float* __restrict__ uvc,
+                                                                   float* __restrict__ fvec, float* __restrict__ hvec, SegPlan p, int D, float scale,
+                                                                   double* __restrict__ colsum) {
+  constexpr int RPB = MRG_BLOCK / LPR;
+  constexpr int WIDTH = LPR * VEC;
+  __shared__ double red[RPB * WIDTH];
+  const int b = blockIdx.x;
+  if (b >= p.blk[3]) return;
+  const int seg = (b >= p.blk[1]) + (b >= p.blk[2]);
+  const int jb = b - p.blk[seg], nb = p.blk[seg + 1] - p.blk[seg];
+  const int sl = threadIdx.x % LPR, rw = row_group_of_thread<LPR>();
+  const int dv = D / VEC;
+  const float* u = uvc + (int64_t)seg * MRG_GATE_LD(D);
+  const float cc = u[HAS_IN ? 2 * D : D];
+  const bool mine = sl < dv;
+  const Vec<VEC> uk = mine ? Vec<VEC>::load(u + sl * VEC) : Vec<VEC>::fill(0.f);
+  const Vec<VEC> vk = (HAS_IN && mine) ? Vec<VEC>::load(u + D + sl * VEC) : Vec<VEC>::fill(0.f);
+  const bool use_norm = norm != nullptr && seg < 2;
+  double st[4][VEC];
+#pragma unroll
+  for (int q = 0; q < 4; ++q)
+#pragma unroll
+    for (int j = 0; j < VEC; ++j) st[q][j] = 0.0;
+  for (int64_t r = p.lo[seg] + (int64_t)jb * RPB + rw; r < p.hi[seg]; r += (int64_t)nb * RPB) {
+    float dot = 0.f;
+    Vec<VEC> sk = Vec<VEC>::fill(0.f);
+    if (mine) {
+      sk = Vec<VEC>::load(s + r * D + sl * VEC);
+#pragma unroll
+      for (int j = 0; j < VEC; ++j) dot += sk[j] * uk[j];
+      if (HAS_IN) {
+        Vec<VEC> x = Vec<VEC>::load(sin_ + r * D + sl * VEC);
+#pragma unroll
+        for (int j = 0; j < VEC; ++j) dot += x[j] * vk[j];
+      }
+    }
+    const float z = group_sum<LPR>(dot) + cc;
+    const float gt = sigmoidf_fast(z);
+    const float nv = use_norm ? norm[r] : 1.0f;
+    const float rf = gt * scale * nv;
+    if (sl == 0) {
+      fvec[r] = rf;
+      const float t = scale * nv;
+      hvec[r] = t * gt * (1.0f - gt);
+    }
+#pragma unroll
+    for (int j = 0; j < VEC; ++j) {
+      double d = (double)sk[j]; st[0][j] += d; st[1][j] += d * d;
+      d = (double)(sk[j] * rf); st[2][j] += d; st[3][j] += d * d;
+    }
+  }
+  double* __restrict__ dst = colsum + (int64_t)b * 4 * D;
+#pragma unroll
+  for (int q = 0; q < 4; ++q) {
+#pragma unroll
+    for (int j = 0; j < VEC; ++j) red[rw * WIDTH + sl * VEC + j] = st[q][j];
+    __syncthreads();
+    for (int c = threadIdx.x; c < D; c += MRG_BLOCK) {
+      double acc = 0.0;
+#pragma unroll
+      for (int g = 0; g < RPB; ++g) acc += red[g * WIDTH + c];
+      dst[q * D + c] = acc;
+    }
+    __syncthreads();
   }
 }
 
@@ -529,26 +598,56 @@
   return MRG_OK;
 }
 
-extern "C" int mrg_gate_row_fwd(const float* s, const float* s_in, const float* norm, const float* uvc, float* fvec, float* hvec,
-                                int64_t b0, int64_t b1, int64_t M, int D, float scale, void* stream) {
+static int gate_row_plan(int64_t b0, int64_t b1, int64_t M, int lpr, SegPlan* p) {
+  int grid = grid_for(M, (MRG_BLOCK / lpr) * 4);
+  if (grid < 3) grid = 3;
+  *p = make_plan(b0, b1, M, grid);
+  return p->blk[3];
+}
+
+static int gate_row_fwd(const float* s, const float* s_in, const float* norm, const float* uvc, float* fvec, float* hvec,
+                        int64_t b0, int64_t b1, int64_t M, int D, float scale, void* stream, double* colsum, int64_t colsum_blocks) {
   if (D <= 0 || M < 0 || b0 < 0 || b1 < b0 || M < b1) return MRG_E_SHAPE;
   if (M == 0) return MRG_OK;
   if (!s || !uvc || !fvec || !hvec) return MRG_E_NULLPTR;
   RowGeom g = row_geom(D, aligned16(s) && aligned16(s_in) && aligned16(uvc));
   if (!g.ok) return MRG_E_SHAPE;
+  if (colsum && g.kmax != 1) return MRG_E_SHAPE;
   hipStream_t st = (hipStream_t)stream;
 #define CALL(V, L, K)                                                                                                   \
   do {                                                                                                                  \
-    int grid = grid_for(M, (MRG_BLOCK / L) * 4);                                                                        \
-    if (grid < 3) grid = 3;                                                                                             \
-    SegPlan p = make_plan(b0, b1, M, grid);                                                                             \
-    if (s_in) hipLaunchKernelGGL((gate_row_fwd_k<V, L, K, true>), dim3(p.blk[3]), dim3(MRG_BLOCK), 0, st, s, s_in, norm, uvc, fvec, hvec, p, D, scale); \
+    SegPlan p;                                                                                                          \
+    gate_row_plan(b0, b1, M, L, &p);                                                                                    \
+    if (colsum && p.blk[3] != colsum_blocks) return MRG_E_SHAPE;     \
+    if (colsum) {                                                                                                       \
+      if (s_in) hipLaunchKernelGGL((gate_row_fwd_colsum_k<V, L, true>), dim3(p.blk[3]), dim3(MRG_BLOCK), 0, st, s, s_in, norm, uvc, fvec, hvec, p, D, scale, colsum); \
+      else hipLaunchKernelGGL((gate_row_fwd_colsum_k<V, L, false>), dim3(p.blk[3]), dim3(MRG_BLOCK), 0, st, s, s_in, norm, uvc, fvec, hvec, p, D, scale, colsum); \
+    } else if (s_in) hipLaunchKernelGGL((gate_row_fwd_k<V, L, K, true>), dim3(p.blk[3]), dim3(MRG_BLOCK), 0, st, s, s_in, norm, uvc, fvec, hvec, p, D, scale); \
     else hipLaunchKernelGGL((gate_row_fwd_k<V, L, K, false>), dim3(p.blk[3]), dim3(MRG_BLOCK), 0, st, s, s_in, norm, uvc, fvec, hvec, p, D, scale); \
   } while (0)
   MRG_DISPATCH_GEOM(g, CALL);
 #undef CALL
   MRG_LAUNCH_CHECK();
   return MRG_OK;
+}
+
+extern "C" int mrg_gate_row_fwd(const float* s, const float* s_in, const float* norm, const float* uvc, float* fvec, float* hvec,
+                                int64_t b0, int64_t b1, int64_t M, int D, float scale, void* stream) {
+  return gate_row_fwd(s, s_in, norm, uvc, fvec, hvec, b0, b1, M, D, scale, stream, nullptr, 0);
+}
+
+extern "C" int64_t mrg_gate_row_colsum_blocks(int64_t b0, int64_t b1, int64_t M, int D, int vec4) {
+  if (D <= 0 || M <= 0 || b0 < 0 || b1 < b0 || M < b1) return 0;
+  RowGeom g = row_geom(D, vec4 != 0);
+  if (!g.ok || g.kmax != 1 || (vec4 && g.vec != 4)) return 0;
+  SegPlan p;
+  return gate_row_plan(b0, b1, M, g.lpr, &p);
+}
+
+extern "C" int mrg_gate_row_fwd_colsum(const float* s, const float* s_in, const float* norm, const float* uvc, float* fvec, float* hvec,
+                                       int64_t b0, int64_t b1, int64_t M, int D, float scale, void* stream, double* colsum, int64_t colsum_blocks) {
+  if (!colsum) return MRG_E_NULLPTR;
+  return gate_row_fwd(s, s_in, norm, uvc, fvec, hvec, b0, b1, M, D, scale, stream, colsum, colsum_blocks);
 }
 
 extern "C" int mrg_gate_row_bwd(const float* q, const float* hvec, const float* s, const float* s_in, const float* uvc, float* gs_in, float* d_uvc,
diff --git a/mr-gnas_amd/csrc/gemm.hpp b/mr-gnas_amd/csrc/gemm.hpp
--- a/mr-gnas_amd/csrc/gemm.hpp
+++ b/mr-gnas_amd/csrc/gemm.hpp
@@ -11,6 +11,9 @@
 constexpr int GBM_MAX = 256;
 
 enum { EPI_BIAS_ACT = 0, EPI_GATE = 1, EPI_SCALE = 2, EPI_ACCUM = 3, EPI_SEGMAX = 4, EPI_SEGSUM = 5 };
+enum { EPI_GATE_SUMS = 6, EPI_SCALE_SUMS = 7 };
+constexpr bool epi_sums(int epi) { return epi == EPI_GATE_SUMS || epi == EPI_SCALE_SUMS; }
+constexpr int epi_base(int epi) { return epi == EPI_GATE_SUMS ? EPI_GATE : (epi == EPI_SCALE_SUMS ? EPI_SCALE : epi); }
 
 struct GemmGroups {
   int n;
@@ -51,6 +54,9 @@
   GemmGroups grp;
 };
 
+inline void gemm_set_colsum(GemmArgs& a, double* colsum) { a.seg_part = reinterpret_cast<float*>(colsum); }
+__host__ __device__ __forceinline__ double* gemm_colsum(const GemmArgs& a) { return reinterpret_cast<double*>(a.seg_part); }
+
 template <bool DUAL>
 __device__ __forceinline__ const float* gemm_a_ptr(const float* r1, const float* r2, int K1, int K2, int K, int k) {
   if (DUAL) {
@@ -204,10 +210,17 @@
   return v;
 }
 
-template <int NT, int EPI>
+template <int NT, int EPI, bool SUMS = false>
 __device__ __forceinline__ void gemm_epilogue(const GemmArgs& a, f32x16 (&acc)[NT], int64_t rowbase, int col0, int li, int lh,
-                                              bool full) {
-  if (rowbase >= a.rows) return;
+                                              bool full, double* __restrict__ sums = nullptr) {
+  static_assert(!SUMS || EPI == EPI_GATE || EPI == EPI_SCALE, "column sums: gate and scale epilogues only");
+  if (rowbase >= a.rows) {
+    if constexpr (SUMS) {
+#pragma unroll
+      for (int n = 0; n < NT; ++n) { sums[(lh * 2 + 0) * NT * 32 + n * 32 + li] = 0.0; sums[(lh * 2 + 1) * NT * 32 + n * 32 + li] = 0.0; }
+    }
+    return;
+  }
   const int last = (int)((a.rows - 1 - rowbase) < 31 ? (a.rows - 1 - rowbase) : 31);
   const int colw = col0 + li < a.N ? col0 + li : a.N - 1;
   float* crow[16];
@@ -237,7 +250,7 @@
     float in[16], v[16], g[16];
 #pragma unroll
     for (int r = 0; r < 16; ++r) in[r] = 0.f;
-    if ((EPI == EPI_GATE && cstore) || EPI == EPI_ACCUM) {
+    if ((EPI == EPI_GATE && (cstore || SUMS)) || EPI == EPI_ACCUM) {
 #pragma unroll
       for (int r = 0; r < 16; ++r) in[r] = srow[r][off];
     }
@@ -255,6 +268,16 @@
         v[r] = x + in[r];
       }
     }
+    if constexpr (SUMS) {
+      double s1 = 0.0, s2 = 0.0;
+#pragma unroll
+      for (int r = 0; r < 16; ++r) {
+        const double d = (full || rok[r]) ? (double)v[r] : 0.0;
+        s1 += d; s2 += d * d;
+      }
+      sums[(lh * 2 + 0) * NT * 32 + n * 32 + li] = cok ? s1 : 0.0;
+      sums[(lh * 2 + 1) * NT * 32 + n * 32 + li] = cok ? s2 : 0.0;
+    }
     if (full) {
       if (cok) {
         if (cstore) {
@@ -275,6 +298,19 @@
         }
       }
     }
+  }
+}
+
+template <int W, int NSLOT>
+__device__ __forceinline__ void gemm_colsum_flush(const double* __restrict__ lds, double* __restrict__ colsum, int N, int col0) {
+  double* __restrict__ dst = colsum + (int64_t)blockIdx.x * 2 * N;
+  for (int t = threadIdx.x; t < 2 * W; t += blockDim.x) {
+    const int which = t / W, c = t - which * W;
+    if (col0 + c >= N) continue;
+    double acc = 0.0;
+#pragma unroll
+    for (int q = 0; q < NSLOT; ++q) acc += lds[(q * 2 + which) * W + c];
+    dst[which * N + col0 + c] = acc;
   }
 }
 
diff --git a/mr-gnas_amd/csrc/gemm_dispatch.hpp b/mr-gnas_amd/csrc/gemm_dispatch.hpp
--- a/mr-gnas_amd/csrc/gemm_dispatch.hpp
+++ b/mr-gnas_amd/csrc/gemm_dispatch.hpp
@@ -61,6 +61,27 @@
   return launch_rowgemm_x3<EPI>(a, Bp, st);
 }
 
+inline int64_t gemm_colsum_blocks(int epi, GemmArgs a) {
+  const int K = a.K1 + a.K2;
+  if ((epi != EPI_GATE && epi != EPI_SCALE) || gemm_mode() != 0 || gemm_switches().epilogue != 0) return 0;
+  if (a.N % 4 != 0 || a.N <= 128 || a.N > 224 || a.rows <= 0 || !x3_eligible(a)) return 0;
+  int gbm = 128;
+  if (x3q_shape(epi, a.N, K)) {
+    if (!x3q_eligible(a)) return 0;
+    gbm = X3Q_ROWS;
+  } else if (x3n_shape(epi, a.rows, a.N, K)) {
+    return 0;
+  }
+  return a.grp.n > 0 ? gemm_group_tiles(a.grp, gbm) : (a.rows + gbm - 1) / gbm;
+}
+
+template <int EPI>
+inline int launch_rowgemm_x3_mode_colsum(GemmArgs a, const void* Bp, hipStream_t st) {
+  if (!gemm_colsum(a) || gemm_colsum_blocks(epi_base(EPI), a) <= 0) return MRG_E_SHAPE;
+  if (x3q_shape(epi_base(EPI), a.N, a.K1 + a.K2)) return launch_rowgemm_x3q<EPI>(a, Bp, st);
+  return launch_rowgemm_x3s_colsum<EPI>(a, Bp, st);
+}
+
 inline size_t gemm_workspace_bytes(int K, int N) {
   const size_t split = bsplit_bytes_any(N, K);
   const size_t transp = (size_t)K * N * sizeof(float);
diff --git a/mr-gnas_amd/csrc/gemm_x3q.hpp b/mr-gnas_amd/csrc/gemm_x3q.hpp
--- a/mr-gnas_amd/csrc/gemm_x3q.hpp
+++ b/mr-gnas_amd/csrc/gemm_x3q.hpp
@@ -8,9 +8,18 @@
 
 inline size_t x3q_bsplit_bytes(int K) { return (size_t)x3q_slabs(K) * 2 * X3Q_CHUNK; }
 
-template <int EPI>
-__device__ __forceinline__ void gemm_epilogue_q(const GemmArgs& a, f32x4v (&acc)[X3Q_NT], int64_t rowbase, int li, int lh, bool full) {
-  if (rowbase >= a.rows) return;
+template <int EPI, bool SUMS = false>
+__device__ __forceinline__ void gemm_epilogue_q(const GemmArgs& a, f32x4v (&acc)[X3Q_NT], int64_t rowbase, int li, int lh, bool full,
+                                                double* __restrict__ sums = nullptr) {
+  static_assert(!SUMS || EPI == EPI_GATE || EPI == EPI_SCALE, "column sums: gate and scale epilogues only");
+  constexpr int W = X3Q_HT * 32;
+  if (rowbase >= a.rows) {
+    if constexpr (SUMS) {
+#pragma unroll
+      for (int j = 0; j < X3Q_HT; ++j) { sums[(lh * 2 + 0) * W + j * 32 + li] = 0.0; sums[(lh * 2 + 1) * W + j * 32 + li] = 0.0; }
+    }
+    return;
+  }
   const int last = (int)((a.rows - 1 - rowbase) < 15 ? (a.rows - 1 - rowbase) : 15);
   const int colw = li < a.N ? li : a.N - 1;
   float* crow[8];
@@ -51,7 +60,7 @@
     float in[8], v[8], g[8];
 #pragma unroll
     for (int i = 0; i < 8; ++i) in[i] = 0.f;
-    if ((EPI == EPI_GATE && cstore) || EPI == EPI_ACCUM) {
+    if ((EPI == EPI_GATE && (cstore || SUMS)) || EPI == EPI_ACCUM) {
 #pragma unroll
       for (int i = 0; i < 8; ++i) in[i] = srow[i][off];
     }
@@ -68,6 +77,16 @@
       } else {
         v[i] = x + in[i];
       }
+    }
+    if constexpr (SUMS) {
+      double s1 = 0.0, s2 = 0.0;
+#pragma unroll
+      for (int i = 0; i < 8; ++i) {
+        const double d = (full || rok[i]) ? (double)v[i] : 0.0;
+        s1 += d; s2 += d * d;
+      }
+      sums[(lh * 2 + 0) * W + j * 32 + li] = cok ? s1 : 0.0;
+      sums[(lh * 2 + 1) * W + j * 32 + li] = cok ? s2 : 0.0;
     }
     if (full) {
       if (cok) {
@@ -185,7 +204,15 @@
   asm volatile("" :: "v"(xr[0][0]), "v"(xr[0][1]), "v"(xr[1][0]), "v"(xr[1][1]));
 
   const int li = lane & 31, lh = lane >> 5;
-  gemm_epilogue_q<EPI>(a, acc, roww, li, lh, row0 + X3Q_ROWS <= a.rows);
+  if constexpr (epi_sums(EPI)) {
+    double* sums = reinterpret_cast<double*>(smem_q);
+    __syncthreads();
+    gemm_epilogue_q<epi_base(EPI), true>(a, acc, roww, li, lh, row0 + X3Q_ROWS <= a.rows, sums + wave * (4 * X3Q_HT * 32));
+    __syncthreads();
+    gemm_colsum_flush<X3Q_HT * 32, 8>(sums, gemm_colsum(a), a.N, 0);
+  } else {
+    gemm_epilogue_q<EPI>(a, acc, roww, li, lh, row0 + X3Q_ROWS <= a.rows);
+  }
 }
 
 inline bool x3q_eligible(const GemmArgs& a) { return x3_eligible(a) && a.rows > 0 && a.N <= X3Q_NT * 16 && !a.row_seg; }
diff --git a/mr-gnas_amd/csrc/gemm_x3s.hpp b/mr-gnas_amd/csrc/gemm_x3s.hpp
--- a/mr-gnas_amd/csrc/gemm_x3s.hpp
+++ b/mr-gnas_amd/csrc/gemm_x3s.hpp
@@ -114,7 +114,14 @@
   asm volatile("s_waitcnt vmcnt(0)" ::: "memory");
   asm volatile("" :: "v"(xr[0][0]), "v"(xr[0][1]), "v"(xr[1][0]), "v"(xr[1][1]), "v"(xr[2][0]), "v"(xr[2][1]));
 
-  if constexpr (EPI == EPI_SEGMAX) gemm_epilogue_segmax<NT>(a, acc, roww, col0, li, lh);
+  if constexpr (epi_sums(EPI)) {
+    double* sums = reinterpret_cast<double*>(smem_b);
+    __syncthreads();
+    gemm_epilogue<NT, epi_base(EPI), true>(a, acc, roww, col0, li, lh, row0 + GBM <= a.rows, sums + wave * (4 * NT * 32));
+    __syncthreads();
+    gemm_colsum_flush<NT * 32, 8>(sums, gemm_colsum(a), a.N, col0);
+  }
+  else if constexpr (EPI == EPI_SEGMAX) gemm_epilogue_segmax<NT>(a, acc, roww, col0, li, lh);
   else if constexpr (EPI == EPI_SEGSUM) gemm_epilogue_segsum<NT>(a, acc, roww, col0, li, lh);
   else if constexpr (TR) gemm_epilogue_tr<NT, EPI>(a, acc, roww, col0, li, lh);
   else gemm_epilogue<NT, EPI>(a, acc, roww, col0, li, lh, row0 + GBM <= a.rows);
@@ -152,4 +159,19 @@
 #undef MRG_GOS3
 }
 
+template <int EPI>
+inline int launch_rowgemm_x3s_colsum(GemmArgs a, const void* Bp, hipStream_t st) {
+  static_assert(epi_sums(EPI), "the column-sum epilogues");
+  if (a.rows <= 0) return MRG_OK;
+  if (!a.A2 || a.K2 == 0) { a.A2 = a.A1; a.K2 = 0; }
+  const int nt = gemm_pick_nt(a.N);
+  if (nt != 7 || a.N > 7 * 32 || !gemm_colsum(a)) return MRG_E_SHAPE;
+  const int ntile = x3_tiles(a.N, nt);
+  if (a.grp.n > 0 && gemm_group_tiles(a.grp, 128) == 0) return MRG_OK;
+  dim3 grid((unsigned)(a.grp.n > 0 ? a.grp.tile0[3] : (a.rows + 127) / 128), 1);
+  const size_t lds = (size_t)3 * nt * 3 * 1024;
+  if (a.K2 > 0) return launch_kernel(rowgemm_x3s_k<7, EPI, true, false>, grid, dim3(256), lds, st, a, Bp, ntile);
+  return launch_kernel(rowgemm_x3s_k<7, EPI, false, false>, grid, dim3(256), lds, st, a, Bp, ntile);
 }
+
+}
diff --git a/mr-gnas_amd/csrc/mixedop.hip b/mr-gnas_amd/csrc/mixedop.hip
--- a/mr-gnas_amd/csrc/mixedop.hip
+++ b/mr-gnas_amd/csrc/mixedop.hip
@@ -1,6 +1,7 @@
 #include "common.hpp"
 
 #define MRG_MIX_MAXK 8
+static_assert(MRG_MIX_MAXK == MRG_MIX_MAX_CANDIDATES, "mrg_gated_branch.given is sized by the header's constant");
 
 namespace mrg {
 
@@ -154,6 +155,31 @@
       }
     }
     colstats_flush<VEC, LPR, KMAX>(s1, s2, red, ws + ((int64_t)blockIdx.x * K + k) * 2 * D, D, sl, rw);
+  }
+}
+
+struct GivenPack { const double* p[MRG_MIX_MAXK]; int n[MRG_MIX_MAXK]; int64_t stride[MRG_MIX_MAXK]; };
+
+__global__ __launch_bounds__(MRG_BLOCK) void mix_given_reduce_k(GivenPack gv, int K, int D, double* __restrict__ ws, int zero_absent) {
+  const int b = blockIdx.x, k = blockIdx.y, G = gridDim.x;
+  double* __restrict__ dst = ws + ((int64_t)b * K + k) * 2 * D;
+  const double* __restrict__ src = gv.p[k];
+  if (src == nullptr) {
+    if (zero_absent)
+      for (int t = threadIdx.x; t < 2 * D; t += MRG_BLOCK) dst[t] = 0.0;
+    return;
+  }
+  const int64_t n = gv.n[k], stride = gv.stride[k];
+  const int64_t lo = n * b / G, hi = n * (b + 1) / G;
+  for (int t = threadIdx.x; t < 2 * D; t += MRG_BLOCK) {
+    double a0 = 0.0, a1 = 0.0, a2 = 0.0, a3 = 0.0;
+    int64_t i = lo;
+    for (; i + 3 < hi; i += 4) {
+      const double v0 = src[i * stride + t], v1 = src[(i + 1) * stride + t], v2 = src[(i + 2) * stride + t], v3 = src[(i + 3) * stride + t];
+      a0 += v0; a1 += v1; a2 += v2; a3 += v3;
+    }
+    for (; i < hi; ++i) a0 += src[i * stride + t];
+    dst[t] = (a0 + a1) + (a2 + a3);
   }
 }
 
@@ -914,8 +940,40 @@
   if (!coef || !gamma_host || !beta_host) return MRG_E_NULLPTR;
   hipStream_t st = (hipStream_t)stream;
   int grid = 1;
-  const int rc = mix_colstats_blocks(y_host, K, rows, D, ws, st, &grid, gated);
-  if (rc != MRG_OK) return rc;
+  bool any_given = false;
+  for (int k = 0; gated && k < K; ++k) any_given = any_given || gated->given[k] != nullptr;
+  if (!any_given) {
+    const int rc = mix_colstats_blocks(y_host, K, rows, D, ws, st, &grid, gated);
+    if (rc != MRG_OK) return rc;
+  } else {
+    if (valid_rows) return MRG_E_SHAPE;
+    if (!pack_ok((const void* const*)y_host, K) || rows < 0) return MRG_E_SHAPE;
+    if (!ws) return MRG_E_WORKSPACE;
+    const float* y2[MRG_MIX_MAXK];
+    mrg_gated_branch g2 = *gated;
+    GivenPack gv{};
+    bool any_read = false;
+    int64_t n_max = 1;
+    for (int k = 0; k < K; ++k) {
+      y2[k] = y_host[k];
+      if (!gated->given[k]) { any_read = any_read || y_host[k] != nullptr; continue; }
+      if (gated->given_n[k] < 1 || gated->given_stride[k] < 2 * (int64_t)D) return MRG_E_SHAPE;
+      gv.p[k] = gated->given[k]; gv.n[k] = gated->given_n[k]; gv.stride[k] = gated->given_stride[k];
+      if (gv.n[k] > n_max) n_max = gv.n[k];
+      y2[k] = nullptr;
+      if (g2.k == k) g2.k = -1;
+      if (g2.row_k == k) g2.row_k = -1;
+    }
+    if (any_read) {
+      const int rc = mix_colstats_blocks(y2, K, rows, D, ws, st, &grid, &g2);
+      if (rc != MRG_OK) return rc;
+    } else {
+      const int64_t g = (n_max + 15) / 16;
+      grid = (int)(g < 256 ? g : 256);
+    }
+    hipLaunchKernelGGL(mix_given_reduce_k, dim3(grid, K), dim3(MRG_BLOCK), 0, st, gv, K, D, (double*)ws, any_read ? 0 : 1);
+    MRG_LAUNCH_CHECK();
+  }
   PtrPack ga{}, be{};
   MutPack rm{}, rv{};
   for (int k = 0; k < K; ++k) {
@@ -934,6 +992,8 @@
                                 const mrg_gated_branch* gated, void* stream) {
   if (!sums) return MRG_E_NULLPTR;
   if (gated && gated->valid_rows) return MRG_E_SHAPE;
+  for (int k = 0; gated && k < MRG_MIX_MAXK; ++k)
+    if (gated->given[k]) return MRG_E_SHAPE;
   hipStream_t st = (hipStream_t)stream;
   int grid = 1;
   const int rc = mix_colstats_blocks(y_host, K, rows, D, ws, st, &grid, gated);
diff --git a/mr-gnas_amd/functional/__init__.py b/mr-gnas_amd/functional/__init__.py
--- a/mr-gnas_amd/functional/__init__.py
+++ b/mr-gnas_amd/functional/__init__.py
@@ -4,7 +4,7 @@
     COMPOSE, REDUCE, ACT, gate_ld, same_rows, _same_memory, _cnt, _ws, _WS_BYTES, _ws_bytes, _SIDE_STREAMS, Fork,
 )
 from .candidates import (
-    Link, Candidate,
+    Link, Candidate, ForEpilogue, wants_stats,
 )
 from .gcs import (
     GCS, fused_gcs, span_gcs, ComposePlan, _ComposeAggregate, compose_aggregate,
diff --git a/mr-gnas_amd/functional/candidates.py b/mr-gnas_amd/functional/candidates.py
--- a/mr-gnas_amd/functional/candidates.py
+++ b/mr-gnas_amd/functional/candidates.py
@@ -30,12 +30,28 @@
         return True
 
 
+class ForEpilogue:
+
+    __slots__ = ("stats",)
+
+    def __init__(self, stats=False):
+        self.stats = bool(stats)
+
+    def __bool__(self):
+        return True
+
+
+def wants_stats(for_epilogue):
+    return bool(getattr(for_epilogue, "stats", False))
+
+
 class Candidate:
 
-    __slots__ = ("kind", "y", "s", "c", "rowscale", "link", "slot", "b0", "b1")
+    __slots__ = ("kind", "y", "s", "c", "rowscale", "link", "slot", "b0", "b1", "sums", "s_sums")
 
-    def __init__(self, kind, y, link=None, slot=0, s=None, c=None, rowscale=None, b0=0, b1=0):
+    def __init__(self, kind, y, link=None, slot=0, s=None, c=None, rowscale=None, b0=0, b1=0, sums=None, s_sums=None):
         self.kind, self.y, self.link, self.slot, self.s, self.c, self.rowscale, self.b0, self.b1 = kind, y, link, slot, s, c, rowscale, b0, b1
+        self.sums, self.s_sums = sums, s_sums
 
     def materialize(self):
         if self.kind == "stored":
diff --git a/mr-gnas_amd/functional/dense.py b/mr-gnas_amd/functional/dense.py
--- a/mr-gnas_amd/functional/dense.py
+++ b/mr-gnas_amd/functional/dense.py
@@ -6,7 +6,7 @@
 from .._lib import ptr_array, call, f32c, ptr, require_hip, stream_of
 from . import switches as SW
 from ._base import Fork, _ws, _ws_bytes, same_rows
-from .candidates import Candidate, Link
+from .candidates import Candidate, Link, wants_stats
 
 
 class _DenseFilter(torch.autograd.Function):
@@ -170,7 +170,7 @@
 class _DensePair(torch.autograd.Function):
 
     @staticmethod
-    def forward(ctx, link, s, s_in, norm, b0, b1, gate_only, *params):
+    def forward(ctx, link, sums, s, s_in, norm, b0, b1, gate_only, *params):
         s, s_in, norm = f32c(s), f32c(s_in), f32c(norm)
         params = tuple(f32c(p) for p in params)
         require_hip(s, s_in, norm, *params)
@@ -182,11 +182,23 @@
         out_d = gate if gate_only else torch.empty_like(s)
         dW, dB, cW = [params[0], params[2], params[4]], [params[1], params[3], params[5]], list(params[6:9])
         work = dict(flops=2 * M * K_ * D)
-        call("mrg_dense_filter_fwd3", (0, ptr(s), ptr(s_in), ptr_array(dW), ptr_array(dB), ptr(norm), 1.0 / 3.0, 1.0 / 3.0,
-                                       None if gate_only else ptr(out_d), ptr(gate), ptr(_ws(ws3, s)), b0, b1, M, D, st),
-             nbytes=4 * M * (K_ + (1 if gate_only else 2) * D), **work)
-        call("mrg_dense_filter_fwd3", (1, ptr(s), ptr(s_in), ptr_array(cW), ptr_array([None, None, None]), ptr(norm), 1.0 / 3.0, 1.0, ptr(out_c), None,
-                                       ptr(_ws(ws3, s)), b0, b1, M, D, st), nbytes=4 * M * (K_ + D), **work)
+        wsp = _ws(ws3, s)
+        args_d = (0, ptr(s), ptr(s_in), ptr_array(dW), ptr_array(dB), ptr(norm), 1.0 / 3.0, 1.0 / 3.0,
+                  None if gate_only else ptr(out_d), ptr(gate), ptr(wsp), b0, b1, M, D, st)
+        args_c = (1, ptr(s), ptr(s_in), ptr_array(cW), ptr_array([None, None, None]), ptr(norm), 1.0 / 3.0, 1.0, ptr(out_c), None,
+                  ptr(wsp), b0, b1, M, D, st)
+        for kind, args, nb in ((0, args_d, 4 * M * (K_ + (1 if gate_only else 2) * D)), (1, args_c, 4 * M * (K_ + D))):
+            blocks = int(_lib.load().mrg_dense_filter3_colsum_blocks(kind, b0, b1, M, D, K_)) if sums is not None else 0
+            if blocks > 0:
+                part = _ws(blocks * 2 * D * 8, s)
+                call("mrg_dense_filter_fwd3", args + (ptr(part), blocks), nbytes=nb + part.numel() + (4 * M * D if kind == 0 and gate_only else 0),
+                     symbol="mrg_dense_filter_fwd3_colsum", **work)
+                sums.append(_lib.ColSums(part, 0, blocks, 2 * D, M))
+            else:
+                call("mrg_dense_filter_fwd3", args, nbytes=nb, **work)
+                if sums is not None:
+                    sums.append(None)
+        del wsp
         ctx.cfg = (b0, b1)
         ctx.save_for_backward(s, s_in, norm, gate, *params)
         ctx.link = link
@@ -235,7 +247,7 @@
         call("mrg_linear_bwd_weight3", (ptr(dz_c), ptr(s), ptr(s_in), ptr_array(g_cW), ptr_array([None, None, None]), ptr(_ws(wsw, s)), b0, b1, M, D, K_ - D, D, st),
              **wwork)
         grads_d = [t for pair in zip(g_dW, g_dB) for t in pair]
-        return (None, gs, gs_in, None, None, None, None, *grads_d, *g_cW)
+        return (None, None, gs, gs_in, None, None, None, None, *grads_d, *g_cW)
 
 
 def dense_pair_available(D, tied):
@@ -281,17 +293,20 @@
     gate_only = bool(gate_only and for_epilogue and s.is_cuda)
     fold = for_epilogue and SW.FOLD_ROW_SCALE and s.is_cuda and torch.is_grad_enabled()
     link = Link(2) if fold else None
-    y_d, y_c = _DensePair.apply(link, s, s_in, norm, int(b0), int(b1), gate_only, dW[0], dB[0], dW[1], dB[1], dW[2], dB[2], *cW)
+    sums = [] if (wants_stats(for_epilogue) and s.is_cuda) else None
+    y_d, y_c = _DensePair.apply(link, sums, s, s_in, norm, int(b0), int(b1), gate_only, dW[0], dB[0], dW[1], dB[1], dW[2], dB[2], *cW)
     if not for_epilogue:
         return y_d, y_c
     fold = fold and y_d.requires_grad
     rs_d = (norm, int(b1), 1.0 / 3.0, 1.0 / 3.0, True) if fold else None
     rs_c = (norm, int(b1), 1.0 / 3.0, 1.0, False) if fold else None
+    sums_d, sums_c = sums if sums else (None, None)
     if gate_only:
-        c_d = Candidate("gate", y_d, link=link, slot=0, s=s, c=_gated_rowscale(norm, int(b1), s.shape[0], 1.0 / 3.0, 1.0 / 3.0, s.device), rowscale=rs_d)
+        c_d = Candidate("gate", y_d, link=link, slot=0, s=s, c=_gated_rowscale(norm, int(b1), s.shape[0], 1.0 / 3.0, 1.0 / 3.0, s.device), rowscale=rs_d,
+                        sums=sums_d)
     else:
-        c_d = Candidate("stored", y_d, link=link, slot=0, rowscale=rs_d)
-    return c_d, Candidate("stored", y_c, link=link, slot=1, rowscale=rs_c)
+        c_d = Candidate("stored", y_d, link=link, slot=0, rowscale=rs_d, sums=sums_d)
+    return c_d, Candidate("stored", y_c, link=link, slot=1, rowscale=rs_c, sums=sums_c)
 
 
 def dense_filter_single(s, s_in, W, b):
diff --git a/mr-gnas_amd/functional/gates.py b/mr-gnas_amd/functional/gates.py
--- a/mr-gnas_amd/functional/gates.py
+++ b/mr-gnas_amd/functional/gates.py
@@ -3,7 +3,7 @@
 from .. import _lib
 from .._lib import ptr_array, call, f32c, ptr, require_hip, stream_of
 from ._base import _ws, _ws_bytes, gate_ld, same_rows
-from .candidates import Candidate, Link
+from .candidates import Candidate, Link, wants_stats
 
 
 class _Gate(torch.autograd.Function):
@@ -65,7 +65,7 @@
 class _GateRow(torch.autograd.Function):
 
     @staticmethod
-    def forward(ctx, link, s, s_in, norm, b0, b1, scale, *params):
+    def forward(ctx, link, sums, s, s_in, norm, b0, b1, scale, *params):
         tied = s_in is not None and same_rows(s, s_in)
         s, s_in, norm = f32c(s), (None if tied else f32c(s_in)), f32c(norm)
         params = tuple(f32c(p) for p in params)
@@ -80,7 +80,15 @@
         fvec = torch.empty(M, dtype=torch.float32, device=s.device)
         hvec = torch.empty(M, dtype=torch.float32, device=s.device)
         nb = 4 * D * M * (2 if s_in is not None else 1) + (4 * b1 if norm is not None else 0) + 8 * M
-        call("mrg_gate_row_fwd", (ptr(s), ptr(s_in), ptr(norm), ptr(uvc), ptr(fvec), ptr(hvec), b0, b1, M, D, scale, st), nbytes=nb)
+        args = (ptr(s), ptr(s_in), ptr(norm), ptr(uvc), ptr(fvec), ptr(hvec), b0, b1, M, D, scale, st)
+        vec4 = D % 4 == 0 and all(t is None or t.data_ptr() % 16 == 0 for t in (s, s_in, uvc))
+        blocks = int(_lib.load().mrg_gate_row_colsum_blocks(b0, b1, M, D, int(vec4))) if sums is not None else 0
+        if blocks > 0:
+            part = _ws(blocks * 4 * D * 8, s)
+            call("mrg_gate_row_fwd", args + (ptr(part), blocks), nbytes=nb + part.numel(), symbol="mrg_gate_row_fwd_colsum")
+            sums += [_lib.ColSums(part, 0, blocks, 4 * D, M), _lib.ColSums(part, 2 * D * 8, blocks, 4 * D, M)]
+        else:
+            call("mrg_gate_row_fwd", args, nbytes=nb)
         ctx.save_for_backward(s, s_in, norm, uvc, hvec, *params)
         ctx.cfg = (b0, b1, scale, in_dim, tied)
         ctx.link = link
@@ -122,11 +130,13 @@
             for seg, (lo, hi) in enumerate(((0, b0), (b0, b1), (b1, M))):
                 if hi > lo:
                     torch.mul(dz[lo:hi, None], uvc[seg, :D][None, :], out=gs[lo:hi])
-        return (None, gs, gs_in, None, None, None, None, *gparams)
+        return (None, None, gs, gs_in, None, None, None, None, *gparams)
 
 
-def gate_comp_row_factor(s, s_in, norm, b0, b1, W_in, b_in, a_in, W_out, b_out, a_out, W_self, b_self, a_self):
+def gate_comp_row_factor(s, s_in, norm, b0, b1, W_in, b_in, a_in, W_out, b_out, a_out, W_self, b_self, a_self, for_epilogue=True):
     s = f32c(s)
     link = Link()
-    fvec = _GateRow.apply(link, s, s_in, norm, int(b0), int(b1), 1.0 / 3.0, W_in, b_in, a_in, W_out, b_out, a_out, W_self, b_self, a_self)
-    return Candidate("rowfactor", fvec, link=link, s=s, b0=int(b0), b1=int(b1))
+    sums = [] if (wants_stats(for_epilogue) and s.is_cuda) else None
+    fvec = _GateRow.apply(link, sums, s, s_in, norm, int(b0), int(b1), 1.0 / 3.0, W_in, b_in, a_in, W_out, b_out, a_out, W_self, b_self, a_self)
+    s_sums, f_sums = sums if sums else (None, None)
+    return Candidate("rowfactor", fvec, link=link, s=s, b0=int(b0), b1=int(b1), sums=f_sums, s_sums=s_sums)
diff --git a/mr-gnas_amd/functional/mixed.py b/mr-gnas_amd/functional/mixed.py
--- a/mr-gnas_amd/functional/mixed.py
+++ b/mr-gnas_amd/functional/mixed.py
@@ -11,8 +11,9 @@
 class _MixCfg:
 
     def __init__(self, bns, present, group=None, total_rows=None, has_addend=False, rowscale=None, identity=None, gated=None, act=0,
-                 valid_rows=None):
+                 valid_rows=None, given=None):
         self.bns, self.present, self.group, self.total_rows, self.has_addend = bns, present, group, total_rows, has_addend
+        self.given = given
         self.act = act
         self.valid_rows = valid_rows
         self.gated = gated
@@ -61,8 +62,21 @@
             rv = ptr_array([b.running_var if track else None for b in cfg.bns])
             mom = bn0.momentum if bn0.momentum is not None else 0.1
             if cfg.group is None:
-                call("mrg_mix_stats_coef", (ypa, ptr_array(gam), ptr_array(bet), rm, rv, K_, rows, total, D, bn0.eps, mom, ptr(coef), ptr(ws), gb, st),
-                     nbytes=4 * D * rows * nz_rd)
+                given, cfg.given = cfg.given, None
+                if given is not None and cfg.valid_rows is None and all(c is None or c.rows == rows for c in given):
+                    swept = set()
+                    for k, y in enumerate(ys):
+                        if y is not None and given[k] is None:
+                            swept.add(y.data_ptr())
+                            if cfg.gated is not None and k == cfg.gated.get("k"):
+                                swept.add(cfg.gated["s"].data_ptr())
+                    gb_stats = _lib.gated_branch(cfg.gated, act=cfg.act, given=given)
+                    nb_stats = 4 * D * rows * len(swept) + sum(c.n * 2 * D * 8 for c in given if c is not None)
+                else:
+                    gb_stats, nb_stats = gb, 4 * D * rows * nz_rd
+                call("mrg_mix_stats_coef", (ypa, ptr_array(gam), ptr_array(bet), rm, rv, K_, rows, total, D, bn0.eps, mom, ptr(coef), ptr(ws), gb_stats, st),
+                     nbytes=nb_stats)
+                del given
             else:
                 import torch.distributed as dist
                 if cfg.chain is not None and cfg.chain[0].sums is not None:
@@ -347,5 +361,14 @@
             gated.update(row_k=k, row_f=y, b0=rb0, b1=rb1, row_link=c.link if wants_grad else None)
         else:
             ys[k] = c.materialize()
-    cfg = _MixCfg(list(bns), present, group, total_rows, False, rowscale, identity, gated, _lib.ACTS[act], valid_rows)
+    given = None
+    if group is None and valid_rows is None and bns and (bns[0].training or not bns[0].track_running_stats):
+        given = [c.sums if c is not None else None for c in cands]
+        if identity is not None and cands[identity] is None and ys[identity] is not None:
+            for c in cands:
+                if c is not None and c.kind == "rowfactor" and c.s_sums is not None and _same_memory(c.s, ys[identity]):
+                    given[identity] = c.s_sums
+        if not any(c is not None for c in given):
+            given = None
+    cfg = _MixCfg(list(bns), present, group, total_rows, False, rowscale, identity, gated, _lib.ACTS[act], valid_rows, given)
     return PreparedEpilogue(cfg, [y for y in ys if y is not None], list(bns))
diff --git a/mr-gnas_amd/functional/switches.py b/mr-gnas_amd/functional/switches.py
--- a/mr-gnas_amd/functional/switches.py
+++ b/mr-gnas_amd/functional/switches.py
@@ -16,6 +16,7 @@
 GROUPED_SEGMENTS = os.environ.get("MRG_GROUPED_SEGMENTS", "1") == "1"
 DENSE_PAIR = os.environ.get("MRG_DENSE_PAIR", "1") == "1"
 GATED_RECOMPUTE = os.environ.get("MRG_GATED_RECOMPUTE", "1") == "1"
+PRODUCER_STATS = os.environ.get("MRG_PRODUCER_STATS", "1") == "1"
 COMPGCN_TAIL = os.environ.get("MRG_COMPGCN_TAIL", "1") == "1"
 SPARSE_AMAX_BWD = os.environ.get("MRG_SPARSE_AMAX_BWD", "1") == "1"
 CCORR_PATH = None
diff --git a/mr-gnas_amd/operations_lp.py b/mr-gnas_amd/operations_lp.py
--- a/mr-gnas_amd/operations_lp.py
+++ b/mr-gnas_amd/operations_lp.py
@@ -102,7 +102,7 @@
             W, a = getattr(self, "W_" + x), getattr(self, "a_" + x)
             p += [W.weight, W.bias, a.weight]
         if for_epilogue and K.switches.ROW_FACTOR and src_emb.is_cuda:
-            return K.gate_comp_row_factor(src_emb, src_emb_in, g.norm_flat(), b0, b1, *p)
+            return K.gate_comp_row_factor(src_emb, src_emb_in, g.norm_flat(), b0, b1, *p, for_epilogue=for_epilogue)
         return K.gate_comp(src_emb, src_emb_in, g.norm_flat(), b0, b1, *p)
 
 
```
